# Ced3-han/PepFlowww

Measured on AMD Instinct MI355X. Metric: residues x denoise-steps / s, higher is better.
Workload: dtype f32 (fp32 storage and accumulation; matrix products as 3 x f16 split MFMA, ~22-bit operands); 1 GPU; cfg4/GPU: B=64 x 128-residue synthetic pockets (112 ctx + 16 gen) per GPU; per_gpu_batch=64, residues=128, global_batch=64, parallelism=batch-shard x1, hipgraph=True, precision=fp32

## Files before the change

include/pepflow_hip.h:

```cpp
#ifndef PEPFLOW_HIP_H
#define PEPFLOW_HIP_H
#include <stdint.h>

#ifdef __cplusplus
extern "C" {
#endif

#define PF_ABI_VERSION 65
#define PF_ATT_VROWS 164
#define PF_ATT_VT_NST(L) (((L) + 31) >> 5)
#define PF_ATT_VT_HEAD(L) ((size_t)11 * PF_ATT_VT_NST(L) * 512)
#define PF_ATT_VT_OFF(c, j, L) ((((size_t)(((c) < 128 ? ((c) & 7) : 8 + (((c) - 128) >> 4)) * PF_ATT_VT_NST(L) + ((j) >> 5)) * 64 + (((j) >> 3) & 3) * 16 + \
                                  ((c) < 128 ? ((c) >> 3) : (((c) - 128) & 15))) * 8) + ((j) & 7))
#define PF_E_BADARG (-1)
#define PF_E_TOOLARGE (-2)

typedef void* pf_stream_t;

#define PF_C_S 128
#define PF_C_Z 64
#define PF_HEADS 8
#define PF_C_HID 128
#define PF_QK_PTS 8
#define PF_V_PTS 12
#define PF_IPA_PROJ 3744
#define PF_IPA_FEATS 1536
#define PF_ET_PRE 512

int pf_abi_version(void);

int pf_selftest_mfma(const float* a, const float* b, float* c, int K, pf_stream_t stream);
int pf_selftest_lanes(const float* in, float* out, pf_stream_t stream);

typedef struct {
    const float* x;  int ldx;
    const float* w;  int ldw;
    const float* bias;
    float* y;        int ldy;
    int M, N, K;
    int relu;
    const float* row_mask;
    int mask_pre, mask_post;
    const float* residual; int ldr;
    const float* ln_gamma; const float* ln_beta; float ln_eps;
    const void* w_f16;
    const float* gate; int ldg;
    const float* pt_rot; const float* pt_trans; float* pt_qp; float* pt_kp; float* pt_vp; int pt_col0;
    int single_pass;
    void* att_qk; void* att_vt; int att_L;
    const int* key_end; int key_L; int active_rows;
    float* k_frag;
} pf_linear_args;
int pf_linear_fwd(const pf_linear_args* a, pf_stream_t stream);
int pf_split_pack_f16(const float* w, int ldw, int N, int K, int transpose, void* out, pf_stream_t stream);
typedef struct { const float* w; int ldw, N, K, transpose; void* out; int first; int pad_; } pf_pack_desc;
int pf_split_pack_f16_batch(const pf_pack_desc* desc_dev, int ndesc, int total_items, int* range_flag, pf_stream_t stream);
int pf_split_pack_f16_checked(const float* w, int ldw, int N, int K, int transpose, void* out, int* range_flag, pf_stream_t stream);

typedef struct {
    const float* node_embed;
    const float* seq_table;
    const int64_t* seqs;
    const float* t;
    const float* time_freq;
    const float* ang_freq;
    const float* angles;
    float* out;
    int B, L;
} pf_embed_args;
int pf_embed_inputs_fwd(const pf_embed_args* a, pf_stream_t stream);
typedef struct {
    const float* node_embed; const float* seq_table; const int64_t* seqs; const float* t; const float* time_freq;
    const float* ang_freq; const float* angles;
    const void* w0_f16; const float* b0; const void* w2_f16; const float* b2;
    const float* mask;
    const float* rot;
    float* quat;
    float* s_out;
    int B, L;
    int single_pass;
} pf_input_mixer_args;
int pf_input_mixer_fwd(const pf_input_mixer_args* a, pf_stream_t stream);

typedef struct {
    const float* proj; int ldp;
    const float* rot;
    const float* trans;
    float* qp;
    float* kp;
    float* vp;
    int rows;
} pf_ipa_points_args;
int pf_ipa_points_fwd(const pf_ipa_points_args* a, pf_stream_t stream);

typedef struct {
    const float* proj; int ldp;
    const float* qp; const float* kp; const float* vp;
    const float* z;
    const float* rot; const float* trans;
    const float* mask;
    const float* w_b; const float* b_b;
    const float* w_dz; const float* b_dz;
    const float* head_w;
    float* feats;
    int B, L;
    const float* bias;
    float* p_out;
    int variant;
    const void* att_qk; const void* att_vt; int att_mode;
    int head_group;
    const int* key_end;
    int z_f16;
    const float* dz;
    int dz_f16;
    int fused_pair;
    const float* s_in; const void* proj_w_f16; const float* proj_bias;
    const float* k_frag;
    int k_from_s;
} pf_ipa_attn_args;
int pf_ipa_attn_fwd(const pf_ipa_attn_args* a, pf_stream_t stream);
int pf_ipa_proj_inside_ok(int L, int f16_mode);
int pf_pair_bias_fwd(const float* z, const float* w_b, const float* b_b, float* bias, int B, int L, pf_stream_t stream);

typedef struct {
    const float* qkv;
    const float* mask;
    float* out;
    int B, L;
} pf_seq_attn_args;
int pf_seq_attn_fwd(const pf_seq_attn_args* a, pf_stream_t stream);

typedef struct {
    const float* feats;
    const float* s_in;
    const float* mask;
    const void* w_out_f16; const float* b_out;
    const float* ln_g; const float* ln_b;
    const void* w_in_f16; const float* b_in;
    float* s_ipa;
    float* qkv;
    int rows;
    int single_pass;
    const int* key_end; int key_L;
    float* dump_a0;
    int o_premul;
} pf_node_head_args;
int pf_node_head_fwd(const pf_node_head_args* a, pf_stream_t stream);

typedef struct {
    const float* qkv;
    const float* resid;
    const float* mask;
    const void* w_o_f16; const float* b_o; const float* n1_g; const float* n1_b;
    const void* w_1_f16; const float* b_1; const void* w_2_f16; const float* b_2; const float* n2_g; const float* n2_b;
    const void* w_in_next_f16; const float* b_in_next; float* qkv_out; float* v_out;
    int last;
    const float* s_ipa;
    const void* w_post_f16; const float* b_post;
    const void* w_t1_f16; const float* b_t1; const void* w_t2_f16; const float* b_t2; const void* w_t3_f16; const float* b_t3;
    const float* nt_g; const float* nt_b;
    const void* w_bb_f16; const float* b_bb;
    float* s_out;
    const float* quat_in; const float* rot_in; const float* trans_in;
    float* quat_out; float* rot_out; float* trans_out;
    int has_et;
    const void* w_init_f16; const float* b_init; const void* w_pre_f16; const float* b_pre; float* pre;
    int B, L;
    const void* h_w[2][3]; const float* h_b[2][3];
    float* logits_out;
    float* ang_out;
    int single_pass;
    const int* key_end;
    float* dump[11];
    const int* row_on;
} pf_node_tfmr_args;
int pf_node_tfmr_fwd(const pf_node_tfmr_args* a, pf_stream_t stream);

int pf_rot_to_quat(const float* rot, float* quat, int n, pf_stream_t stream);

typedef struct {
    const float* quat_in;
    const float* rot_in;
    const float* trans_in;
    const float* upd; int ldu;
    const float* mask;
    float* quat_out; float* rot_out; float* trans_out;
    int n;
} pf_rigid_update_args;
int pf_rigid_update_fwd(const pf_rigid_update_args* a, pf_stream_t stream);

typedef struct {
    const float* z_in;
    float* z_out;
    const float* pre;
    const void* w1z_f16;
    const void* w2_f16;
    const float* b2;
    const void* wf_f16;
    const float* ln_g; const float* ln_b;
    const float* mask;
    int B, L;
    const void* w_stream;
    float* bias_out; const void* wb_frags; const float* bb;
    float* dump_h1; float* dump_h2; float* dump_y;
    int single_pass;
    const int* tile_list; const int* n_tiles;
    int z_in_f16, z_out_f16;
    float* dz_out;
    int dz_out_f16;
    const void* w_stream32; const void* wb_frags32;
    unsigned char* dump_m1; unsigned char* dump_m2;
    int z_in_frag, z_out_frag;
    const void* w_stream64;
} pf_edge_transition_args;
int pf_edge_transition_fwd(const pf_edge_transition_args* a, pf_stream_t stream);
int pf_edge_transition_tile_rows(int single_pass);
int pf_edge_transition_v4_tile_rows(void);

typedef struct {
    const int64_t* aa; const int64_t* res_nb; const int64_t* chain_nb;
    const float* pos;
    const float* mask_atoms;
    const float* gen_mask;
    const float* aa_table;
    const float* freq3;
    float* feat;
    float* rot1; float* trans1;
    float* mres; float* ctx;
    int B, L;
    int sample_structure, sample_sequence;
    int L0;
} pf_node_feat_args;
int pf_node_features_fwd(const pf_node_feat_args* a, pf_stream_t stream);

typedef struct {
    const int64_t* aa; const int64_t* res_nb; const int64_t* chain_nb;
    const float* pos; const float* mask_atoms;
    const float* ctx; const float* mres;
    const float* aapair_table;
    const float* relpos_table;
    const float* distcoef;
    const float* freq3;
    const float* w_d0; const float* b_d0; const float* w_d2; const float* b_d2;
    const float* w_o0; const float* b_o0; const float* w_o2; const float* b_o2; const float* w_o4; const float* b_o4;
    float* out;
    int B, L;
    int sample_structure, sample_sequence;
    float* dump_g; float* dump_d2; float* dump_h1; float* dump_cat; float* dump_o1; float* dump_o2;
    float* softplus_ws;
} pf_edge_feat_args;
int pf_edge_features_fwd(const pf_edge_feat_args* a, pf_stream_t stream);

typedef struct {
    const float* rot1; const float* trans1; const float* ang1; const int64_t* seq1;
    const float* gen_mask;
    const float* res_mask;
    float* rot_t; float* trans_t; float* ang_t; int64_t* seq_t; float* simplex_t;
    float* trans0; float* simplex0;
    const float* pred_rot; const float* pred_trans; const float* pred_ang_raw; const float* pred_logits;
    float* traj_rot; float* traj_trans; float* traj_ang; int64_t* traj_seq; float* traj_simplex;
    const float* ts; int num_steps;
    int* step;
    float* t_out;
    const float* expo; uint64_t seed; int64_t first_sample;
    int B, L;
    int sample_bb, sample_ang, sample_seq;
    const uint64_t* seed_dev;
    const int64_t* sample_ids;
} pf_sampler_args;
int pf_sampler_init(const pf_sampler_args* a, const float* rot0, const float* trans0_raw,
                    const float* ang0, const float* simplex0_raw, pf_stream_t stream);
int pf_sampler_step(const pf_sampler_args* a, pf_stream_t stream);
typedef struct {
    int partial;
    const float* start_rot;
    const float* start_trans;
    const float* start_ang;
    const int64_t* start_seq;
    const uint8_t* res_flags;
    const uint32_t* aa_allowed;
} pf_sampler_cond_args;
int pf_sampler_init_cond(const pf_sampler_args* a, const pf_sampler_cond_args* c, const float* rot0, const float* trans0_raw,
                         const float* ang0, const float* simplex0_raw, pf_stream_t stream);
int pf_sampler_step_cond(const pf_sampler_args* a, const pf_sampler_cond_args* c, pf_stream_t stream);

#define PF_GUIDE_MAX_PAIRS 64
#define PF_GUIDE_MAX_L 1024
#define PF_GUIDE_NPARAMS 16
#define PF_GUIDE_NTERMS 5
typedef struct {
    const float* pred_trans;
    const float* trans1;
    const float* gen_mask;
    const float* res_mask;
    const uint8_t* res_flags;
    const uint8_t* hotspots;
    const int* pair_idx;
    const float* pair_par;
    const float* params;
    const float* ts;
    const int* step;
    const float* t;
    float* guided_trans;
    float* energy;
    float* shift_max;
    float* grad;
    int* error;
    int B, L, num_steps, sample_bb;
} pf_guidance_args;
int pf_guidance_fwd(const pf_guidance_args* a, pf_stream_t stream);

int pf_so3_geodesic(const float* base, const float* target, const float* t, float* out, int n, pf_stream_t stream);
int pf_so3_log(const float* rot, float* rotvec, int n, pf_stream_t stream);
int pf_so3_exp(const float* rotvec, float* rot, int n, pf_stream_t stream);
int pf_torus_geodesic(const float* base, const float* target, const float* t, float* out, int n, pf_stream_t stream);

typedef struct {
    const float* rot1; const float* trans1; const float* ang1; const int64_t* seq1;
    const float* gen_mask; const float* res_mask;
    const float* t_raw; const float* rot0; const float* trans0_raw; const float* ang0; const float* simplex0_raw;
    const float* expo; uint64_t seed; int64_t first_sample;
    float* t; float* rot_t; float* trans_t; float* ang_t; int64_t* seq_t;
    const float* pred_rot; const float* pred_trans; const float* pred_ang_raw; const float* pred_logits;
    int64_t* pred_seq;
    float* per_sample;
    float* losses;
    int B, L;
// ... 479 lines not shown
```

pepflowww_amd/_capi.py:

```python
import ctypes as C
import os

import torch

_HERE = os.path.dirname(os.path.abspath(__file__))
LIB_PATH = os.environ.get("PF_LIB_PATH") or os.path.join(_HERE, "lib", "libpepflow_hip.so")
ABI_VERSION = 65

_fp = C.c_void_p
_i = C.c_int
GUIDE_MAX_PAIRS, GUIDE_MAX_L, GUIDE_NPARAMS, GUIDE_NTERMS = 64, 1024, 16, 5


class LinearArgs(C.Structure):
    _fields_ = [("x", _fp), ("ldx", _i), ("w", _fp), ("ldw", _i), ("bias", _fp), ("y", _fp), ("ldy", _i),
                ("M", _i), ("N", _i), ("K", _i), ("relu", _i), ("row_mask", _fp), ("mask_pre", _i),
                ("mask_post", _i), ("residual", _fp), ("ldr", _i), ("ln_gamma", _fp), ("ln_beta", _fp),
                ("ln_eps", C.c_float), ("w_f16", _fp), ("gate", _fp), ("ldg", _i),
                ("pt_rot", _fp), ("pt_trans", _fp), ("pt_qp", _fp), ("pt_kp", _fp), ("pt_vp", _fp), ("pt_col0", _i),
                ("single_pass", _i), ("att_qk", _fp), ("att_vt", _fp), ("att_L", _i), ("key_end", _fp), ("key_L", _i), ("active_rows", _i),
                ("k_frag", _fp)]


class EmbedArgs(C.Structure):
    _fields_ = [("node_embed", _fp), ("seq_table", _fp), ("seqs", _fp), ("t", _fp), ("time_freq", _fp),
                ("ang_freq", _fp), ("angles", _fp), ("out", _fp), ("B", _i), ("L", _i)]


class IpaPointsArgs(C.Structure):
    _fields_ = [("proj", _fp), ("ldp", _i), ("rot", _fp), ("trans", _fp), ("qp", _fp), ("kp", _fp), ("vp", _fp),
                ("rows", _i)]


class IpaAttnArgs(C.Structure):
    _fields_ = [("proj", _fp), ("ldp", _i), ("qp", _fp), ("kp", _fp), ("vp", _fp), ("z", _fp), ("rot", _fp),
                ("trans", _fp), ("mask", _fp), ("w_b", _fp), ("b_b", _fp), ("w_dz", _fp), ("b_dz", _fp),
                ("head_w", _fp), ("feats", _fp), ("B", _i), ("L", _i), ("bias", _fp), ("p_out", _fp),
                ("variant", _i), ("att_qk", _fp), ("att_vt", _fp), ("att_mode", _i), ("head_group", _i), ("key_end", _fp), ("z_f16", _i), ("dz", _fp), ("dz_f16", _i), ("fused_pair", _i),
                ("s_in", _fp), ("proj_w_f16", _fp), ("proj_bias", _fp), ("k_frag", _fp), ("k_from_s", _i)]


class InputMixerArgs(C.Structure):
    _fields_ = [("node_embed", _fp), ("seq_table", _fp), ("seqs", _fp), ("t", _fp), ("time_freq", _fp), ("ang_freq", _fp),
                ("angles", _fp), ("w0_f16", _fp), ("b0", _fp), ("w2_f16", _fp), ("b2", _fp), ("mask", _fp), ("rot", _fp),
                ("quat", _fp), ("s_out", _fp), ("B", _i), ("L", _i), ("single_pass", _i)]


class SeqAttnArgs(C.Structure):
    _fields_ = [("qkv", _fp), ("mask", _fp), ("out", _fp), ("B", _i), ("L", _i)]


class RigidUpdateArgs(C.Structure):
    _fields_ = [("quat_in", _fp), ("rot_in", _fp), ("trans_in", _fp), ("upd", _fp), ("ldu", _i), ("mask", _fp),
                ("quat_out", _fp), ("rot_out", _fp), ("trans_out", _fp), ("n", _i)]


class EdgeTransitionArgs(C.Structure):
    _fields_ = [("z_in", _fp), ("z_out", _fp), ("pre", _fp), ("w1z_f16", _fp), ("w2_f16", _fp), ("b2", _fp), ("wf_f16", _fp),
                ("ln_g", _fp), ("ln_b", _fp), ("mask", _fp), ("B", _i), ("L", _i), ("w_stream", _fp),
                ("bias_out", _fp), ("wb_frags", _fp), ("bb", _fp), ("dump_h1", _fp), ("dump_h2", _fp), ("dump_y", _fp),
                ("single_pass", _i), ("tile_list", _fp), ("n_tiles", _fp), ("z_in_f16", _i), ("z_out_f16", _i), ("dz_out", _fp), ("dz_out_f16", _i),
                ("w_stream32", _fp), ("wb_frags32", _fp), ("dump_m1", _fp), ("dump_m2", _fp), ("z_in_frag", _i), ("z_out_frag", _i), ("w_stream64", _fp)]


class SamplerArgs(C.Structure):
    _fields_ = [("rot1", _fp), ("trans1", _fp), ("ang1", _fp), ("seq1", _fp), ("gen_mask", _fp), ("res_mask", _fp),
                ("rot_t", _fp), ("trans_t", _fp), ("ang_t", _fp), ("seq_t", _fp), ("simplex_t", _fp),
                ("trans0", _fp), ("simplex0", _fp),
                ("pred_rot", _fp), ("pred_trans", _fp), ("pred_ang_raw", _fp), ("pred_logits", _fp),
                ("traj_rot", _fp), ("traj_trans", _fp), ("traj_ang", _fp), ("traj_seq", _fp), ("traj_simplex", _fp),
                ("ts", _fp), ("num_steps", _i), ("step", _fp), ("t_out", _fp),
                ("expo", _fp), ("seed", C.c_uint64), ("first_sample", C.c_int64),
                ("B", _i), ("L", _i), ("sample_bb", _i), ("sample_ang", _i), ("sample_seq", _i), ("seed_dev", _fp), ("sample_ids", _fp)]


class SamplerCondArgs(C.Structure):
    _fields_ = [("partial", _i), ("start_rot", _fp), ("start_trans", _fp), ("start_ang", _fp), ("start_seq", _fp),
                ("res_flags", _fp), ("aa_allowed", _fp)]


class GuidanceArgs(C.Structure):
    _fields_ = [("pred_trans", _fp), ("trans1", _fp), ("gen_mask", _fp), ("res_mask", _fp), ("res_flags", _fp), ("hotspots", _fp),
                ("pair_idx", _fp), ("pair_par", _fp), ("params", _fp), ("ts", _fp), ("step", _fp), ("t", _fp),
                ("guided_trans", _fp), ("energy", _fp), ("shift_max", _fp), ("grad", _fp), ("error", _fp),
                ("B", _i), ("L", _i), ("num_steps", _i), ("sample_bb", _i)]


class TrainArgs(C.Structure):
    _fields_ = [("rot1", _fp), ("trans1", _fp), ("ang1", _fp), ("seq1", _fp), ("gen_mask", _fp), ("res_mask", _fp),
                ("t_raw", _fp), ("rot0", _fp), ("trans0_raw", _fp), ("ang0", _fp), ("simplex0_raw", _fp),
                ("expo", _fp), ("seed", C.c_uint64), ("first_sample", C.c_int64),
                ("t", _fp), ("rot_t", _fp), ("trans_t", _fp), ("ang_t", _fp), ("seq_t", _fp),
                ("pred_rot", _fp), ("pred_trans", _fp), ("pred_ang_raw", _fp), ("pred_logits", _fp),
                ("pred_seq", _fp), ("per_sample", _fp), ("losses", _fp),
                ("B", _i), ("L", _i), ("sample_structure", _i), ("sample_sequence", _i), ("seed_dev", _fp)]


class TrainBwdArgs(C.Structure):
    _fields_ = [("w", C.c_float * 6), ("d_rot", _fp), ("d_trans", _fp), ("d_ang", _fp), ("d_logits", _fp), ("w_dev", _fp)]


class GemmArgs(C.Structure):
    _fields_ = [("A", _fp), ("sam", C.c_longlong), ("sak", C.c_longlong), ("B", _fp), ("sbk", C.c_longlong), ("sbn", C.c_longlong),
                ("C", _fp), ("ldc", _i), ("M", _i), ("N", _i), ("K", _i), ("accumulate", _i),
                ("bias", _fp), ("relu", _i), ("residual", _fp), ("alpha", C.c_float), ("batch1", _i), ("batch2", _i),
                ("bsA1", C.c_longlong), ("bsA2", C.c_longlong), ("bsB1", C.c_longlong), ("bsB2", C.c_longlong),
                ("bsC1", C.c_longlong), ("bsC2", C.c_longlong), ("ksplit", _i), ("rowsum_a", _fp), ("gate", _fp)]


class LayerNormBwdArgs(C.Structure):
    _fields_ = [("x", _fp), ("dy", _fp), ("gamma", _fp), ("dx", _fp), ("dgamma_rows", _fp), ("M", _i), ("N", _i),
                ("dgamma", _fp), ("dbeta", _fp), ("workspace", _fp), ("workspace_elems", C.c_longlong), ("row_scale", _fp)]


class RigidUpdateBwdArgs(C.Structure):
    _fields_ = [("quat_in", _fp), ("rot_in", _fp), ("upd", _fp), ("ldu", _i), ("mask", _fp),
                ("g_rot_out", _fp), ("g_quat_out", _fp), ("g_trans_out", _fp),
                ("g_upd", _fp), ("g_quat_in", _fp), ("g_trans_in", _fp), ("g_rot_in", _fp), ("rot_is_from_quat", _i), ("n", _i)]


class IpaBwdArgs(C.Structure):
    _fields_ = [("proj", _fp), ("ldp", _i), ("qp", _fp), ("kp", _fp), ("vp", _fp), ("z", _fp), ("rot", _fp), ("trans", _fp), ("mask", _fp),
                ("w_b", _fp), ("b_b", _fp), ("w_dz", _fp), ("b_dz", _fp), ("head_w", _fp), ("g_feats", _fp),
                ("P", _fp), ("gA", _fp), ("g_opt", _fp), ("g_frame_rows", _fp), ("g_gamma_rows", _fp),
                ("g_bias", _fp), ("g_pz", _fp), ("g_z", _fp), ("accumulate_gz", _i),
                ("g_qp", _fp), ("g_kp", _fp), ("g_vp", _fp), ("g_proj", _fp), ("B", _i), ("L", _i), ("g_bp", _fp)]


class FullAtomArgs(C.Structure):
    _fields_ = [("rot", _fp), ("trans", _fp), ("angles", _fp), ("aa", _fp), ("tab_rot", _fp), ("tab_trans", _fp), ("tab_group", _fp),
                ("tab_pos", _fp), ("tab_mask", _fp), ("frame_group", _i * 5), ("pos14", _fp), ("frames_rot", _fp), ("frames_trans", _fp),
                ("gen_mask", _fp), ("ctx_pos15", _fp), ("pos15_merged", _fp), ("mask15", _fp), ("rows", _i)]


class BackboneAtomsArgs(C.Structure):
    _fields_ = [("rot", _fp), ("trans", _fp), ("aa", _fp), ("chain_nb", _fp), ("res_nb", _fp), ("mask", _fp), ("tab_bb", _fp),
                ("tab_o", _fp), ("pos4", _fp), ("gen_mask", _fp), ("ctx_pos15", _fp), ("ctx_mask15", _fp), ("pos15_merged", _fp),
                ("mask15", _fp), ("B", _i), ("L", _i)]


class NodeFeatArgs(C.Structure):
    _fields_ = [("aa", _fp), ("res_nb", _fp), ("chain_nb", _fp), ("pos", _fp), ("mask_atoms", _fp), ("gen_mask", _fp),
                ("aa_table", _fp), ("freq3", _fp), ("feat", _fp), ("rot1", _fp), ("trans1", _fp), ("mres", _fp),
                ("ctx", _fp), ("B", _i), ("L", _i), ("sample_structure", _i), ("sample_sequence", _i), ("L0", _i)]


class EdgeFeatArgs(C.Structure):
    _fields_ = [("aa", _fp), ("res_nb", _fp), ("chain_nb", _fp), ("pos", _fp), ("mask_atoms", _fp), ("ctx", _fp),
                ("mres", _fp), ("aapair_table", _fp), ("relpos_table", _fp), ("distcoef", _fp), ("freq3", _fp),
                ("w_d0", _fp), ("b_d0", _fp), ("w_d2", _fp), ("b_d2", _fp), ("w_o0", _fp), ("b_o0", _fp),
                ("w_o2", _fp), ("b_o2", _fp), ("w_o4", _fp), ("b_o4", _fp), ("out", _fp), ("B", _i), ("L", _i),
                ("sample_structure", _i), ("sample_sequence", _i),
                ("dump_g", _fp), ("dump_d2", _fp), ("dump_h1", _fp), ("dump_cat", _fp), ("dump_o1", _fp), ("dump_o2", _fp),
                ("softplus_ws", _fp)]


class NodeHeadArgs(C.Structure):
    _fields_ = [("feats", _fp), ("s_in", _fp), ("mask", _fp), ("w_out_f16", _fp), ("b_out", _fp), ("ln_g", _fp),
                ("ln_b", _fp), ("w_in_f16", _fp), ("b_in", _fp), ("s_ipa", _fp), ("qkv", _fp), ("rows", _i), ("single_pass", _i), ("key_end", _fp), ("key_L", _i), ("dump_a0", _fp), ("o_premul", _i)]


class NodeTfmrArgs(C.Structure):
    _fields_ = [("qkv", _fp), ("resid", _fp), ("mask", _fp),
                ("w_o_f16", _fp), ("b_o", _fp), ("n1_g", _fp), ("n1_b", _fp), ("w_1_f16", _fp), ("b_1", _fp),
                ("w_2_f16", _fp), ("b_2", _fp), ("n2_g", _fp), ("n2_b", _fp),
                ("w_in_next_f16", _fp), ("b_in_next", _fp), ("qkv_out", _fp), ("v_out", _fp), ("last", _i),
                ("s_ipa", _fp), ("w_post_f16", _fp), ("b_post", _fp), ("w_t1_f16", _fp), ("b_t1", _fp), ("w_t2_f16", _fp),
                ("b_t2", _fp), ("w_t3_f16", _fp), ("b_t3", _fp), ("nt_g", _fp), ("nt_b", _fp), ("w_bb_f16", _fp),
                ("b_bb", _fp), ("s_out", _fp), ("quat_in", _fp), ("rot_in", _fp), ("trans_in", _fp),
                ("quat_out", _fp), ("rot_out", _fp), ("trans_out", _fp), ("has_et", _i),
                ("w_init_f16", _fp), ("b_init", _fp), ("w_pre_f16", _fp), ("b_pre", _fp), ("pre", _fp), ("B", _i), ("L", _i),
                ("h_w", (_fp * 3) * 2), ("h_b", (_fp * 3) * 2), ("logits_out", _fp), ("ang_out", _fp), ("single_pass", _i), ("key_end", _fp), ("dump", _fp * 11), ("row_on", _fp)]


class SuperposeArgs(C.Structure):
    _fields_ = [("x", _fp), ("y", _fp), ("mx", _fp), ("my", _fp), ("aa_x", _fp), ("aa_y", _fp), ("pairs", _fp),
                ("rmsd_plain", _fp), ("rmsd", _fp), ("count", _fp), ("ident", _fp), ("rot", _fp), ("trans", _fp), ("aligned", _fp),
                ("degenerate", _fp), ("Bx", _i), ("By", _i), ("N", _i), ("P", _i), ("allow_reflection", _i)]


class BindingSiteArgs(C.Structure):
    _fields_ = [("ctx_pos", _fp), ("ctx_atom_mask", _fp), ("n_atoms", _i), ("ca_atom", _i), ("res_mask", _fp), ("gen_mask", _fp),
                ("pep_sample", _fp), ("pep_native", _fp), ("cutoff", C.c_float), ("site_sample", _fp), ("site_native", _fp),
                ("bsr", _fp), ("B", _i), ("L", _i)]


class TmScoreArgs(C.Structure):
    _fields_ = [("x", _fp), ("y", _fp), ("mx", _fp), ("my", _fp), ("pairs", _fp), ("tm", _fp), ("count", _fp), ("lnorm", _fp),
                ("rot", _fp), ("trans", _fp), ("aligned", _fp), ("work", _fp), ("Bx", _i), ("By", _i), ("N", _i), ("P", _i)]


class DsspArgs(C.Structure):
    _fields_ = [("pos", _fp), ("mask", _fp), ("chain", _fp), ("aa", _fp), ("ss", _fp), ("hb_acc", _fp), ("hb_energy", _fp),
                ("B", _i), ("N", _i), ("n_atoms", _i), ("pro", _i)]


class TmAlignArgs(C.Structure):
    _fields_ = [("x", _fp), ("y", _fp), ("mx", _fp), ("my", _fp), ("pairs", _fp), ("tm", _fp), ("tm_x", _fp), ("rmsd", _fp),
                ("n_aligned", _fp), ("len_x", _fp), ("len_y", _fp), ("rot", _fp), ("trans", _fp), ("y2x", _fp), ("kept", _fp),
                ("aligned", _fp), ("Bx", _i), ("By", _i), ("N", _i), ("P", _i), ("max_len", _i)]


class ViolationsArgs(C.Structure):
    _fields_ = [("pos", _fp), ("atom_mask", _fp), ("aa", _fp), ("residue_index", _fp), ("query", _fp), ("group", _fp), ("radius", _fp),
                ("clash_atom_loss", _fp), ("clash_atom", _fp), ("clash_atom_pairs", _fp), ("clash_atom_loss_cross", _fp),
                ("clash_atom_cross", _fp), ("clash_mean_loss", _fp), ("bond_c_n_loss_mean", _fp), ("angle_ca_c_n_loss_mean", _fp),
                ("angle_c_n_ca_loss_mean", _fp), ("connection_loss", _fp), ("connection_violation", _fp), ("ca_ca_break", _fp),
                ("ca_ca_extreme", _fp), ("B", _i), ("N", _i), ("n_atoms", _i), ("pro", _i),
                ("violation_tolerance_factor", C.c_float), ("clash_overlap_tolerance", C.c_float)]


class SasaArgs(C.Structure):
    _fields_ = [("pos", _fp), ("atom_mask", _fp), ("aa", _fp), ("query", _fp), ("group", _fp), ("radius", _fp), ("points", _fp),
                ("work", _fp), ("count", _fp), ("sasa_atom", _fp), ("sasa_residue", _fp), ("sasa_total", _fp), ("count_own", _fp),
                ("sasa_atom_own", _fp), ("sasa_residue_own", _fp), ("sasa_total_own", _fp), ("B", _i), ("N", _i), ("n_atoms", _i),
                ("n_points", _i), ("probe_radius", C.c_float)]


class CavityArgs(C.Structure):
    _fields_ = [("pos", _fp), ("atom_mask", _fp), ("aa", _fp), ("radius", _fp), ("origin", _fp), ("work", _fp), ("occupied", _fp),
                ("buried", _fp), ("label", _fp), ("n_found", _fp), ("size", _fp), ("center", _fp), ("mean_buried", _fp),
                ("lining", _fp), ("status", _fp), ("B", _i), ("N", _i), ("n_atoms", _i), ("nx", _i), ("ny", _i), ("nz", _i),
                ("n_axis", _i), ("n_diag", _i), ("min_buried", _i), ("connectivity", _i), ("min_points", _i), ("max_cavities", _i),
                ("h", C.c_float), ("probe", C.c_float), ("r_lining", C.c_float)]


class TorsionsArgs(C.Structure):
    _fields_ = [("pos", _fp), ("atom_mask", _fp), ("aa", _fp), ("residue_index", _fp), ("chi_atoms", _fp), ("angles", _fp),
                ("defined", _fp), ("B", _i), ("N", _i), ("n_atoms", _i)]


class SidechainCompareArgs(C.Structure):
    _fields_ = [("pos_x", _fp), ("pos_y", _fp), ("mask_x", _fp), ("mask_y", _fp), ("aa_x", _fp), ("aa_y", _fp), ("angles_x", _fp),
                ("angles_y", _fp), ("defined_x", _fp), ("defined_y", _fp), ("pairs", _fp), ("periodic", _fp), ("swap", _fp),
                ("err_sum", _fp), ("err_count", _fp), ("within", _fp), ("res_with_chi", _fp), ("res_correct", _fp), ("sc_sq_sum", _fp),
                ("sc_atoms", _fp), ("sc_rmsd", _fp), ("err", _fp), ("sc_sq", _fp), ("sc_n", _fp), ("swapped", _fp),
                ("Bx", _i), ("By", _i), ("N", _i), ("P", _i), ("n_atoms_x", _i), ("n_atoms_y", _i), ("correct_tol", C.c_float)]


class LddtArgs(C.Structure):
    _fields_ = [("pos_x", _fp), ("pos_y", _fp), ("mask_x", _fp), ("mask_y", _fp), ("aa_x", _fp), ("aa_y", _fp), ("pairs", _fp),
                ("group", _fp), ("query", _fp), ("scored", _fp), ("kept", _fp), ("scored_cross", _fp), ("kept_cross", _fp),
                ("scored_atom", _fp), ("kept_atom", _fp), ("scored_atom_cross", _fp), ("kept_atom_cross", _fp),
                ("Bx", _i), ("By", _i), ("N", _i), ("P", _i), ("n_atoms_x", _i), ("n_atoms_y", _i), ("slot_mask", _i),
                ("exclude_same_residue", _i), ("cutoff", C.c_float)]


class ContactsArgs(C.Structure):
    _fields_ = [("pos_x", _fp), ("pos_y", _fp), ("mask_x", _fp), ("mask_y", _fp), ("pairs", _fp), ("group", _fp),
                ("contacts_x", _fp), ("contacts_y", _fp), ("contacts_shared", _fp), ("interface_x", _fp), ("interface_y", _fp),
                ("min_dist_x", _fp), ("min_dist_y", _fp), ("Bx", _i), ("By", _i), ("N", _i), ("P", _i), ("n_atoms_x", _i),
                ("n_atoms_y", _i), ("slot_mask", _i), ("contact_cutoff", C.c_float), ("interface_cutoff", C.c_float)]


class ClusterArgs(C.Structure):
    _fields_ = [("dist", _fp), ("index", _fp), ("offsets", _fp), ("score", _fp), ("work", _fp), ("label", _fp), ("cluster_size", _fp),
                ("representative", _fp), ("best", _fp), ("n_neighbours", _fp), ("n_clusters", _fp), ("B", _i), ("G", _i), ("n_max", _i),
                ("method", _i), ("cutoff", C.c_float)]


class PackArgs(C.Structure):
    _fields_ = [("pos", _fp), ("atom_mask", _fp), ("aa", _fp), ("residue_index", _fp), ("movable", _fp), ("radius", _fp), ("types", _fp),
                ("own_mask", _fp), ("tab_rot", _fp), ("tab_trans", _fp), ("tab_group", _fp), ("tab_pos", _fp), ("tab_mask", _fp),
                ("rot_chi", _fp), ("rot_count", _fp), ("rot_energy", _fp), ("work", _fp), ("pos_out", _fp), ("mask_out", _fp),
                ("packed", _fp), ("rotamer", _fp), ("chi", _fp), ("n_rotamers", _fp), ("energy_self_best", _fp), ("energy_residue", _fp),
                ("energy_trace", _fp), ("sweeps_run", _fp), ("changed", _fp), ("choice_trace", _fp),
                ("B", _i), ("N", _i), ("n_atoms", _i), ("max_rot", _i), ("sweeps", _i), ("pro", _i), ("cys", _i),
                ("cutoff", C.c_float), ("w_gauss1", C.c_float), ("w_gauss2", C.c_float), ("w_repulsion", C.c_float),
                ("w_hydrophobic", C.c_float), ("w_hbond", C.c_float)]


class InterfaceEnergyArgs(C.Structure):
    _fields_ = [("pos", _fp), ("atom_mask", _fp), ("aa", _fp), ("group", _fp), ("query", _fp), ("radius", _fp), ("types", _fp),
                ("work", _fp), ("terms_atom", _fp), ("terms_residue", _fp), ("energy_residue", _fp), ("pairs_atom", _fp),
                ("hbond_pairs_atom", _fp), ("hydrophobic_pairs_atom", _fp), ("B", _i), ("N", _i), ("n_atoms", _i),
                ("cutoff", C.c_float), ("w_gauss1", C.c_float), ("w_gauss2", C.c_float), ("w_repulsion", C.c_float),
                ("w_hydrophobic", C.c_float), ("w_hbond", C.c_float)]


class RelaxArgs(C.Structure):
    _fields_ = [("pos", _fp), ("ref_pos", _fp), ("atom_mask", _fp), ("aa", _fp), ("residue_index", _fp), ("movable", _fp),
                ("radius", _fp), ("pair_mask", _fp), ("work", _fp), ("gradient", _fp), ("terms_atom", _fp), ("energy_atom", _fp),
                ("terms", _fp), ("energy", _fp), ("x", _fp), ("g", _fp), ("y", _fp), ("alpha", _fp), ("frozen", _fp),
                ("terms_initial", _fp), ("energy_trace", _fp), ("accepted", _fp), ("step_size", _fp), ("grad_max", _fp),
                ("iterations", _fp), ("B", _i), ("N", _i), ("n_atoms", _i), ("pro", _i), ("steps", _i),
                ("k_rest", C.c_float), ("k_intra", C.c_float), ("k_bond", C.c_float), ("k_angle", C.c_float), ("k_clash", C.c_float),
                ("clash_overlap_tolerance", C.c_float), ("clash_margin", C.c_float), ("step0", C.c_float), ("gtol", C.c_float)]


class EtBwdArgs(C.Structure):
    _fields_ = [("g_y", _fp), ("h1", _fp), ("h2", _fp), ("wfT_f16", _fp), ("w2T_f16", _fp), ("w1T_f16", _fp),
                ("g_h2", _fp), ("g_h1", _fp), ("g_x", _fp), ("npairs", C.c_longlong), ("m1", _fp), ("m2", _fp)]


class OptimArgs(C.Structure):
    _fields_ = [("tensors", _fp), ("hyper", _fp), ("chunks", _fp), ("exp_avg", _fp), ("exp_avg_sq", _fp), ("steps", _fp), ("work", _fp),
                ("result", _fp), ("n_tensors", _i), ("n_groups", _i), ("n_chunks", _i)]


_SIGNATURES = {
    "pf_et_bwd_chain": ([C.POINTER(EtBwdArgs), _fp], _i),
    "pf_gemm_tn_cat": ([_fp, _i, _i, _fp, _fp, _fp, _i, _i, _fp, _i, _i, _fp, _i, _fp, C.c_longlong, _fp], _i),
    "pf_gemm_tn_sum2": ([_fp, _i, _i, _fp, _fp, _i, _i, _fp, _i, C.c_longlong, _i, _fp, _i, _fp, C.c_longlong, _fp], _i),
    "pf_et_pack_train": ([_fp, _fp, _fp, _fp, _fp, _fp, _fp, C.c_float, _fp, _fp, _fp], _i),
    "pf_abi_version": ([], _i),
    "pf_selftest_mfma": ([_fp, _fp, _fp, _i, _fp], _i),
    "pf_selftest_lanes": ([_fp, _fp, _fp], _i),
    "pf_linear_fwd": ([C.POINTER(LinearArgs), _fp], _i),
    "pf_embed_inputs_fwd": ([C.POINTER(EmbedArgs), _fp], _i),
    "pf_input_mixer_fwd": ([C.POINTER(InputMixerArgs), _fp], _i),
    "pf_ipa_points_fwd": ([C.POINTER(IpaPointsArgs), _fp], _i),
    "pf_ipa_attn_fwd": ([C.POINTER(IpaAttnArgs), _fp], _i),
    "pf_ipa_proj_inside_ok": ([_i, _i], _i),
    "pf_pair_bias_fwd": ([_fp, _fp, _fp, _fp, _i, _i, _fp], _i),
    "pf_seq_attn_fwd": ([C.POINTER(SeqAttnArgs), _fp], _i),
    "pf_node_head_fwd": ([C.POINTER(NodeHeadArgs), _fp], _i),
    "pf_node_tfmr_fwd": ([C.POINTER(NodeTfmrArgs), _fp], _i),
    "pf_rot_to_quat": ([_fp, _fp, _i, _fp], _i),
    "pf_rigid_update_fwd": ([C.POINTER(RigidUpdateArgs), _fp], _i),
    "pf_edge_transition_fwd": ([C.POINTER(EdgeTransitionArgs), _fp], _i),
    "pf_edge_transition_tile_rows": ([_i], _i),
    "pf_edge_transition_v4_tile_rows": ([], _i),
    "pf_node_features_fwd": ([C.POINTER(NodeFeatArgs), _fp], _i),
    "pf_edge_features_fwd": ([C.POINTER(EdgeFeatArgs), _fp], _i),
    "pf_sampler_init": ([C.POINTER(SamplerArgs), _fp, _fp, _fp, _fp, _fp], _i),
# ... 141 lines not shown
```

pepflowww_amd/csrc/common.h:

```cpp
#pragma once
#include <hip/hip_runtime.h>

static inline int pf_cu_count() {
    static int cache[64] = {0};
    int dev = 0, c = 256;
    if (hipGetDevice(&dev) != hipSuccess) return 256;
    if (dev >= 0 && dev < 64 && cache[dev] > 0) return cache[dev];
    if (hipDeviceGetAttribute(&c, hipDeviceAttributeMultiprocessorCount, dev) != hipSuccess || c <= 0) c = 256;
    if (dev >= 0 && dev < 64) cache[dev] = c;
    return c;
}
#include <stdint.h>

#define PF_WAVE 64

typedef float f32x4 __attribute__((ext_vector_type(4)));

__device__ __forceinline__ f32x4 mfma16(float a, float b, f32x4 c) {
    return __builtin_amdgcn_mfma_f32_16x16x4f32(a, b, c, 0, 0, 0);
}

__device__ __forceinline__ void lds_barrier() {
    asm volatile("s_waitcnt lgkmcnt(0)" ::: "memory");
    __builtin_amdgcn_s_barrier();
// ... 14 lines not shown
template <int OFF> __device__ __forceinline__ float lane_xor(float v) {
    if constexpr (OFF == 1) return lane_xor1(v);
    else if constexpr (OFF == 2) return lane_xor2(v);
    else if constexpr (OFF == 4) return lane_xor4(v);
    else return lane_xor8(v);
}
__device__ __forceinline__ float sum_xor16(float v) {
    auto r = __builtin_amdgcn_permlane16_swap(__float_as_uint(v), __float_as_uint(v), false, false);
    return __uint_as_float(r[0]) + __uint_as_float(r[1]);
}
__device__ __forceinline__ float sum_xor32(float v) {
    auto r = __builtin_amdgcn_permlane32_swap(__float_as_uint(v), __float_as_uint(v), false, false);
    return __uint_as_float(r[0]) + __uint_as_float(r[1]);
}
__device__ __forceinline__ float max_xor16(float v) {
    auto r = __builtin_amdgcn_permlane16_swap(__float_as_uint(v), __float_as_uint(v), false, false);
    return fmaxf(__uint_as_float(r[0]), __uint_as_float(r[1]));
}
__device__ __forceinline__ float max_xor32(float v) {
    auto r = __builtin_amdgcn_permlane32_swap(__float_as_uint(v), __float_as_uint(v), false, false);
    return fmaxf(__uint_as_float(r[0]), __uint_as_float(r[1]));
}
__device__ __forceinline__ bool pf_rows_all_masked(const int* __restrict__ key_end, int L, int m0, int n, int M) {
    if (!key_end) return false;
    const int mend = m0 + n < M ? m0 + n : M;
    int m = m0;
    while (m < mend) {
        const int b = m / L, i = m - b * L;
        if (i < key_end[b]) return false;
        m = (b + 1) * L;
    }
    return true;
}
__device__ __forceinline__ float row16_sum(float v) {
    v += lane_xor8(v); v += lane_xor4(v); v += lane_xor2(v); v += lane_xor1(v);
    return v;
}
__device__ __forceinline__ float row16_max(float v) {
    v = fmaxf(v, lane_xor8(v)); v = fmaxf(v, lane_xor4(v)); v = fmaxf(v, lane_xor2(v)); v = fmaxf(v, lane_xor1(v));
    return v;
}
__device__ __forceinline__ float wave_sum(float v) { return sum_xor32(sum_xor16(row16_sum(v))); }
__device__ __forceinline__ float wave_max(float v) { return max_xor32(max_xor16(row16_max(v))); }

__device__ __forceinline__ float keep_if(bool ok, float v) { return __uint_as_float(__float_as_uint(v) & (ok ? 0xffffffffu : 0u)); }
__device__ __forceinline__ float4 keep_if(bool ok, const float4& v) {
    const unsigned m = ok ? 0xffffffffu : 0u;
    return make_float4(__uint_as_float(__float_as_uint(v.x) & m), __uint_as_float(__float_as_uint(v.y) & m),
                       __uint_as_float(__float_as_uint(v.z) & m), __uint_as_float(__float_as_uint(v.w) & m));
}

template <int MT, int NT>
__device__ __forceinline__ void mfma_slice(const float4 (&a)[MT], const float4 (&b)[NT], f32x4 (&acc)[MT][NT]) {
#pragma unroll
    for (int mt = 0; mt < MT; ++mt)
#pragma unroll
        for (int nt = 0; nt < NT; ++nt) {
            acc[mt][nt] = mfma16(a[mt].x, b[nt].x, acc[mt][nt]);
            acc[mt][nt] = mfma16(a[mt].y, b[nt].y, acc[mt][nt]);
            acc[mt][nt] = mfma16(a[mt].z, b[nt].z, acc[mt][nt]);
            acc[mt][nt] = mfma16(a[mt].w, b[nt].w, acc[mt][nt]);
        }
}

template <int NT, int PF_DEPTH = 4>
struct BStream {
    const float* wrow[NT];
    bool wok[NT];
    float4 ring[PF_DEPTH][NT];
    int nslices;

    __device__ __forceinline__ void init(const float* __restrict__ W, int ldw, int n0, int n_valid, int K) {
        const int lane = threadIdx.x & 63;
        const int r = lane & 15, g = lane >> 4;
        nslices = K >> 4;
#pragma unroll
        for (int nt = 0; nt < NT; ++nt) {
            const int n = n0 + 16 * nt + r;
            wok[nt] = n < n_valid;
            wrow[nt] = W + (size_t)(wok[nt] ? n : 0) * ldw + 4 * g;
        }
    }
    __device__ __forceinline__ void load(int slot_static, int slice, float4 (&dst)[NT]) {
        (void)slot_static;
#pragma unroll
        for (int nt = 0; nt < NT; ++nt)
            dst[nt] = *reinterpret_cast<const float4*>(wrow[nt] + 16 * slice);
    }
    __device__ __forceinline__ void prefetch() {
#pragma unroll
        for (int d = 0; d < PF_DEPTH; ++d)
            if (d < nslices) load(d, d, ring[d]);
    }
};

template <int MT, int NT, int PF_DEPTH>
__device__ __forceinline__ void gemm_ldsA_stream(const float* __restrict__ A_lds, int lda, BStream<NT, PF_DEPTH>& bs,
                                                 f32x4 (&acc)[MT][NT], int slice0, int count) {
    const int lane = threadIdx.x & 63;
    const float* arow = A_lds + (lane & 15) * lda + 4 * (lane >> 4);
    const int ns = bs.nslices;
    for (int base = 0; base < count; base += PF_DEPTH) {
#pragma unroll
        for (int u = 0; u < PF_DEPTH; ++u) {
            if (base + u < count) {
                const int sl = slice0 + base + u;
                float4 a[MT];
#pragma unroll
                for (int mt = 0; mt < MT; ++mt)
                    a[mt] = *reinterpret_cast<const float4*>(arow + mt * 16 * lda + 16 * (base + u));
                mfma_slice<MT, NT>(a, bs.ring[u], acc);
                if (sl + PF_DEPTH < ns) bs.load(u, sl + PF_DEPTH, bs.ring[u]);
            }
        }
    }
}

template <int MT, int NT>
__device__ __forceinline__ void gemm_ldsA_glbB(const float* __restrict__ A_lds, int lda,
                                               const float* __restrict__ W, int ldw, int n0, int n_valid,
                                               int K, f32x4 (&acc)[MT][NT]) {
    BStream<NT> bs;
    bs.init(W, ldw, n0, n_valid, K);
    bs.prefetch();
    gemm_ldsA_stream<MT, NT, 4>(A_lds, lda, bs, acc, 0, bs.nslices);
}

typedef _Float16 half8 __attribute__((ext_vector_type(8)));
typedef _Float16 half4 __attribute__((ext_vector_type(4)));
__device__ __forceinline__ float exp_softmax(float x) { return __builtin_amdgcn_exp2f(x * 1.4426950408889634f); }
constexpr float PF_LO_SCALE = 2048.f, PF_LO_INV = 1.f / 2048.f;

__device__ __forceinline__ f32x4 mfma_h(half8 a, half8 b, f32x4 c) {
    return __builtin_amdgcn_mfma_f32_16x16x32_f16(a, b, c, 0, 0, 0);
}
constexpr float PF_F16_MAX = 65504.f;
#ifndef PF_SPLIT_SATURATE
#define PF_SPLIT_SATURATE 1
#endif
__device__ __forceinline__ void split4(const float (&v)[4], half4& hi, half4& lo) {
#pragma unroll
    for (int e = 0; e < 4; ++e) {
#if PF_SPLIT_SATURATE
        const float vc = fminf(fmaxf(v[e], -PF_F16_MAX), PF_F16_MAX) + v[e] * 0.f;
#else
        const float vc = v[e];
#endif
        const _Float16 h = (_Float16)vc;
        hi[e] = h;
        lo[e] = (_Float16)__builtin_fmaf((float)h, -PF_LO_SCALE, vc * PF_LO_SCALE);
    }
}
__device__ __forceinline__ float join(f32x4 m, f32x4 c, int e) { return m[e] + c[e] * PF_LO_INV; }

template <int WT, int D, bool SP = false>
struct WSplit {
    const _Float16* wh[WT];
    const _Float16* wl[WT];
    half8 rh[D][WT], rl[D][WT];
    int nsteps;
    __device__ __forceinline__ void init(const void* planes, int Npad, int K, int n0) {
        const int lane = threadIdx.x & 63;
        const _Float16* hi = reinterpret_cast<const _Float16*>(planes);
        const _Float16* lo = hi + (size_t)Npad * K;
        nsteps = K >> 5;
#pragma unroll
        for (int wt = 0; wt < WT; ++wt) {
            const size_t off = ((size_t)((n0 >> 4) + wt) * nsteps * 64 + lane) * 8;
            wh[wt] = hi + off;
            wl[wt] = lo + off;
        }
    }
    __device__ __forceinline__ void load(int step, half8 (&dh)[WT], half8 (&dl)[WT]) {
#pragma unroll
        for (int wt = 0; wt < WT; ++wt) {
            dh[wt] = *reinterpret_cast<const half8*>(wh[wt] + (size_t)step * 512);
            if constexpr (!SP) dl[wt] = *reinterpret_cast<const half8*>(wl[wt] + (size_t)step * 512);
        }
    }
    __device__ __forceinline__ void prefetch() {
#pragma unroll
        for (int d = 0; d < D; ++d)
            if (d < nsteps) load(d, rh[d], rl[d]);
    }
};

template <int WT, int D, bool SP>
__device__ __forceinline__ void gemm_split16(WSplit<WT, D, SP>& ws, const _Float16* Xh, const _Float16* Xl, int ldx,
                                             f32x4 (&am)[WT], f32x4 (&ac)[WT], int step0, int count) {
    const int lane = threadIdx.x & 63;
    const int off = (lane & 15) * ldx + 8 * (lane >> 4);
    for (int base = 0; base < count; base += D) {
#pragma unroll
        for (int u = 0; u < D; ++u) {
            if (base + u < count) {
                const int st = step0 + base + u;
                const half8 xh = *reinterpret_cast<const half8*>(Xh + off + 32 * (base + u));
                half8 xl;
                if constexpr (!SP) xl = *reinterpret_cast<const half8*>(Xl + off + 32 * (base + u));
#pragma unroll
                for (int wt = 0; wt < WT; ++wt) {
                    am[wt] = mfma_h(ws.rh[u][wt], xh, am[wt]);
                    if constexpr (!SP) {
                        ac[wt] = mfma_h(ws.rh[u][wt], xl, ac[wt]);
                        ac[wt] = mfma_h(ws.rl[u][wt], xh, ac[wt]);
                    }
                }
                if (st + D < ws.nsteps) ws.load(st + D, ws.rh[u], ws.rl[u]);
            }
        }
    }
}
template <int WT, int D, bool SP, int RT>
__device__ __forceinline__ void gemm_split16r(WSplit<WT, D, SP>& ws, const _Float16* Xh, const _Float16* Xl, int ldx,
                                              f32x4 (&am)[RT][WT], f32x4 (&ac)[RT][WT], int step0, int count) {
    const int lane = threadIdx.x & 63;
    const int off = (lane & 15) * ldx + 8 * (lane >> 4);
    for (int base = 0; base < count; base += D) {
#pragma unroll
        for (int u = 0; u < D; ++u) {
            if (base + u < count) {
                const int st = step0 + base + u;
#pragma unroll
                for (int rt = 0; rt < RT; ++rt) {
                    const half8 xh = *reinterpret_cast<const half8*>(Xh + rt * 16 * ldx + off + 32 * (base + u));
                    half8 xl;
                    if constexpr (!SP) xl = *reinterpret_cast<const half8*>(Xl + rt * 16 * ldx + off + 32 * (base + u));
#pragma unroll
                    for (int wt = 0; wt < WT; ++wt) {
                        am[rt][wt] = mfma_h(ws.rh[u][wt], xh, am[rt][wt]);
                        if constexpr (!SP) {
                            ac[rt][wt] = mfma_h(ws.rh[u][wt], xl, ac[rt][wt]);
                            ac[rt][wt] = mfma_h(ws.rl[u][wt], xh, ac[rt][wt]);
                        }
                    }
                }
                if (st + D < ws.nsteps) ws.load(st + D, ws.rh[u], ws.rl[u]);
            }
        }
    }
}
template <int WT> __device__ __forceinline__ void acc_zero1(f32x4 (&a)[WT], f32x4 (&b)[WT]) {
#pragma unroll
    for (int wt = 0; wt < WT; ++wt) { a[wt] = (f32x4){0.f, 0.f, 0.f, 0.f}; b[wt] = (f32x4){0.f, 0.f, 0.f, 0.f}; }
}

template <int WT>
struct WPre {
    half8 h[WT], l[WT];
    __device__ __forceinline__ void load(const void* planes, int N, int Kw, int n0) {
        const int lane = threadIdx.x & 63;
        const int wsteps = Kw >> 5;
        const _Float16* wh = reinterpret_cast<const _Float16*>(planes) + ((size_t)(n0 >> 4) * wsteps * 64 + lane) * 8;
        const _Float16* wl = wh + (size_t)N * Kw;
        const size_t tstride = (size_t)wsteps * 512;
#pragma unroll
        for (int wt = 0; wt < WT; ++wt) {
            h[wt] = *reinterpret_cast<const half8*>(wh + wt * tstride);
            l[wt] = *reinterpret_cast<const half8*>(wl + wt * tstride);
        }
    }
};

template <int WT, int PT, bool SP = false>
__device__ __forceinline__ void gemm_split_lowreg(const void* planes, int N, int Kw, int n0, int K,
                                                  const _Float16* Xh, const _Float16* Xl, int ldx,
                                                  f32x4 (&am)[WT][PT], f32x4 (&ac)[WT][PT]) {
    static_assert(PT % 2 == 0, "row tiles are fed in pairs");
    const int lane = threadIdx.x & 63, r = lane & 15, g = lane >> 4;
    const int wsteps = Kw >> 5, nst = K >> 5;
    const _Float16* wh = reinterpret_cast<const _Float16*>(planes) + ((size_t)(n0 >> 4) * wsteps * 64 + lane) * 8;
    const _Float16* wl = wh + (size_t)N * Kw;
    const size_t tstride = (size_t)wsteps * 512;
    const _Float16* xh = Xh + r * ldx + 8 * g;
    const _Float16* xl = Xl + r * ldx + 8 * g;
    for (int st = 0; st < nst; ++st) {
        half8 bh[WT], bl[WT];
#pragma unroll
        for (int wt = 0; wt < WT; ++wt) {
            bh[wt] = *reinterpret_cast<const half8*>(wh + wt * tstride + (size_t)st * 512);
            if constexpr (!SP) bl[wt] = *reinterpret_cast<const half8*>(wl + wt * tstride + (size_t)st * 512);
        }
#pragma unroll
        for (int p0 = 0; p0 < PT; p0 += 2) {
            half8 ah[2], al[2];
#pragma unroll
            for (int q = 0; q < 2; ++q) {
                ah[q] = *reinterpret_cast<const half8*>(xh + (p0 + q) * 16 * ldx + 32 * st);
                if constexpr (!SP) al[q] = *reinterpret_cast<const half8*>(xl + (p0 + q) * 16 * ldx + 32 * st);
            }
#pragma unroll
            for (int wt = 0; wt < WT; ++wt)
#pragma unroll
                for (int q = 0; q < 2; ++q) am[wt][p0 + q] = mfma_h(bh[wt], ah[q], am[wt][p0 + q]);
            if constexpr (!SP) {
#pragma unroll
                for (int wt = 0; wt < WT; ++wt)
#pragma unroll
                    for (int q = 0; q < 2; ++q) ac[wt][p0 + q] = mfma_h(bh[wt], al[q], ac[wt][p0 + q]);
#pragma unroll
                for (int wt = 0; wt < WT; ++wt)
#pragma unroll
                    for (int q = 0; q < 2; ++q) ac[wt][p0 + q] = mfma_h(bl[wt], ah[q], ac[wt][p0 + q]);
            }
        }
    }
// ... 88 lines not shown
```

pepflowww_amd/csrc/ipa_split.hip:

```cpp
#include <cstdlib>
#include <type_traits>
#include "common.h"
#include "../../include/pepflow_hip.h"

#ifdef PF_PROFILE
__device__ long long g_prof_ipas[64];
#define PROFS(i) do { if (blockIdx.x == gridDim.x / 2 + 3 && threadIdx.x == 64) g_prof_ipas[i] = clock64(); } while (0)
extern "C" int pf_debug_prof_ipas(long long* out, int n) {
    return (int)hipMemcpyFromSymbol(out, HIP_SYMBOL(g_prof_ipas), sizeof(long long) * n, 0, hipMemcpyDeviceToHost);
}
#else
#define PROFS(i)
#endif

namespace {

typedef float f32x2 __attribute__((ext_vector_type(2)));
constexpr int H = PF_HEADS, C = PF_C_HID, PQ = PF_QK_PTS, PV = PF_V_PTS;
constexpr int OFF_KV = 1024;
#ifndef PF_IPA_WMAX
#define PF_IPA_WMAX 8
#endif
constexpr int WMAX = PF_IPA_WMAX;
constexpr int KPS = 28;
constexpr int VPS = 36;

__device__ __forceinline__ float softplusf2(float x) { return x > 20.f ? x : log1pf(expf(x)); }

template <bool D16> struct DzVec { typedef float4 type; };
template <> struct DzVec<true> { typedef half4 type; };

template <int NB4, bool D16>
__device__ __forceinline__ void pair_dz_rows(const void* __restrict__ dzp, size_t rowb, int L, int i0, int Le, int kt,
                                             const float* __restrict__ Pw, int SLD, int ks, int cq, f32x2 (&acc)[32]) {
    typedef typename DzVec<D16>::type V4;
    typedef typename std::conditional<D16, _Float16, float>::type DT;
    constexpr int NT = 4 * NB4;
    const DT* base = reinterpret_cast<const DT*>(dzp) + rowb * (size_t)L * 16 + 4 * cq;
    int koff[NT];
    float on[NT];
#pragma unroll
    for (int u = 0; u < NT; ++u) {
        const int uu = min(u, kt - 1);
        koff[u] = min(16 * uu + ks, L - 1) * 16;
        on[u] = u < kt ? 1.f : 0.f;
    }
    auto load_row = [&](int qi, V4 (&buf)[NT]) {
        const DT* row = base + (size_t)min(i0 + qi, Le - 1) * L * 16;
#pragma unroll
        for (int u = 0; u < NT; ++u) buf[u] = *reinterpret_cast<const V4*>(row + koff[u]);
    };
    auto mac_row = [&](int qi, const V4 (&buf)[NT]) {
        const float* pr = Pw + qi * SLD;
#pragma unroll
        for (int u = 0; u < NT; ++u) {
            float pv;
            if (u <= 4 * (NB4 - 1)) pv = pr[16 * u];
            else pv = pr[16 * min(u, kt - 1)] * on[u];
            const f32x2 p2 = {pv, pv};
            f32x2 d0, d1;
            if constexpr (D16) { d0 = (f32x2){(float)buf[u][0], (float)buf[u][1]}; d1 = (f32x2){(float)buf[u][2], (float)buf[u][3]}; }
            else { d0 = (f32x2){buf[u].x, buf[u].y}; d1 = (f32x2){buf[u].z, buf[u].w}; }
            acc[2 * qi] = __builtin_elementwise_fma(d0, p2, acc[2 * qi]);
            acc[2 * qi + 1] = __builtin_elementwise_fma(d1, p2, acc[2 * qi + 1]);
        }
    };
    constexpr int D = NB4 == 1 ? 8 : NB4 == 2 ? 4 : 2;
    V4 buf[D][NT];
#pragma unroll
    for (int d = 0; d < D - 1; ++d) load_row(d, buf[d]);
#pragma unroll
    for (int qi = 0; qi < 16; ++qi) {
        load_row(min(qi + D - 1, 15), buf[(qi + D - 1) % D]);
        __builtin_amdgcn_sched_barrier(0);
        mac_row(qi, buf[qi % D]);
        __builtin_amdgcn_sched_barrier(0);
    }
}

template <bool D16>
__device__ __forceinline__ void pair_dz_phase(const pf_ipa_attn_args& a, size_t rowb, int h, int i0, int Le, int kt, const float* Pwave,
                                              int SLD, float inv, int lane) {
    const int ks = (lane & 3) | ((lane >> 4) << 2), cq = (lane >> 2) & 3;
    f32x2 acc[32];
#pragma unroll
    for (int k = 0; k < 32; ++k) acc[k] = (f32x2){0.f, 0.f};
    const float* Pw = Pwave + ks;
    const int nb4 = (kt + 3) >> 2;
    if (nb4 <= 1) pair_dz_rows<1, D16>(a.dz, rowb, a.L, i0, Le, kt, Pw, SLD, ks, cq, acc);
    else if (nb4 == 2) pair_dz_rows<2, D16>(a.dz, rowb, a.L, i0, Le, kt, Pw, SLD, ks, cq, acc);
    else if (nb4 == 3) pair_dz_rows<3, D16>(a.dz, rowb, a.L, i0, Le, kt, Pw, SLD, ks, cq, acc);
    else pair_dz_rows<4, D16>(a.dz, rowb, a.L, i0, Le, kt, Pw, SLD, ks, cq, acc);
    float v[64];
#pragma unroll
    for (int k = 0; k < 32; ++k) { v[2 * k] = acc[k][0]; v[2 * k + 1] = acc[k][1]; }
    float w[32], x[16], y[8], z4[4];
#pragma unroll
    for (int k = 0; k < 32; ++k) {
        auto rr = __builtin_amdgcn_permlane32_swap(__float_as_uint(v[k]), __float_as_uint(v[k + 32]), false, false);
        w[k] = __uint_as_float(rr[0]) + __uint_as_float(rr[1]);
    }
#pragma unroll
    for (int k = 0; k < 16; ++k) {
        auto rr = __builtin_amdgcn_permlane16_swap(__float_as_uint(w[k]), __float_as_uint(w[k + 16]), false, false);
        x[k] = __uint_as_float(rr[0]) + __uint_as_float(rr[1]);
    }
    {
        const bool hi = lane & 2;
#pragma unroll
        for (int k = 0; k < 8; ++k) {
            const float send = hi ? x[k] : x[k + 8], keep = hi ? x[k + 8] : x[k];
            y[k] = keep + lane_xor2(send);
        }
    }
    {
        const bool hi = lane & 1;
#pragma unroll
        for (int k = 0; k < 4; ++k) {
            const float send = hi ? y[k] : y[k + 4], keep = hi ? y[k + 4] : y[k];
            z4[k] = keep + lane_xor1(send);
        }
    }
    const int qi = ((lane >> 5) & 1) * 8 + ((lane >> 4) & 1) * 4 + (lane & 3);
    const float invq = __shfl(inv, qi);
    const float4 bd = *reinterpret_cast<const float4*>(a.b_dz + 4 * cq);
    const int i = min(i0 + qi, Le - 1);
    *reinterpret_cast<float4*>(a.feats + (rowb + i) * PF_IPA_FEATS + 1408 + h * 16 + 4 * cq) =
        make_float4(z4[0] * invq + bd.x, z4[1] * invq + bd.y, z4[2] * invq + bd.z, z4[3] * invq + bd.w);
}

template <int I, int N, class F> __device__ __forceinline__ void cfor_p(F&& f) {
    if constexpr (I < N) {
        f(std::integral_constant<int, I>{});
        cfor_p<I + 1, N>(f);
    }
}
constexpr int PJ_TILES = 31;
constexpr int PJ_NPAD = 3968;
constexpr int PJ_CT = 3;
constexpr int PJ_NCH = (PJ_TILES + PJ_CT - 1) / PJ_CT;
constexpr int PJ_CHUNK_B = PJ_CT * 8 * 1024;
constexpr int PJ_NB = 4;
constexpr int PJ_STAGE_B = PJ_NB * PJ_CHUNK_B;
__device__ __forceinline__ constexpr int pj_tile(int idx, int h) {
    return idx < 8 ? 8 * h + idx : idx < 24 ? 64 + 16 * h + (idx - 8) : idx < 26 ? 192 + 2 * h + (idx - 24) : 208 + 5 * h + (idx - 26);
}
__device__ __forceinline__ void pj_glds16(const void* sbase, unsigned voff, unsigned lds_addr) {
    const unsigned long long v = (unsigned long long)sbase;
    const unsigned lo = __builtin_amdgcn_readfirstlane((unsigned)v), hi = __builtin_amdgcn_readfirstlane((unsigned)(v >> 32));
    const void* sb = (const void*)(((unsigned long long)hi << 32) | lo);
    lds_addr = __builtin_amdgcn_readfirstlane(lds_addr);
    asm volatile("s_mov_b32 m0, %2\n\ts_nop 4\n\tglobal_load_lds_dwordx4 %0, %1" : : "v"(voff), "s"(sb), "s"(lds_addr) : "memory", "m0");
}
template <class V> __device__ __forceinline__ void pf_pin(V& v) { asm("" : "+v"(v)); }
template <int N> __device__ __forceinline__ void pj_wait_vm() { asm volatile("s_waitcnt vmcnt(%0)" : : "n"(N) : "memory"); }
__device__ __forceinline__ void pj_wait_vm_dyn(int n) {
    n = __builtin_amdgcn_readfirstlane(n);
    switch (n > 40 ? 40 : n) {
#define PJ_W(k) case k: pj_wait_vm<k>(); break;
        PJ_W(0) PJ_W(1) PJ_W(2) PJ_W(3) PJ_W(4) PJ_W(5) PJ_W(6) PJ_W(7) PJ_W(8) PJ_W(9) PJ_W(10) PJ_W(11) PJ_W(12) PJ_W(13) PJ_W(14)
        PJ_W(15) PJ_W(16) PJ_W(17) PJ_W(18) PJ_W(19) PJ_W(20) PJ_W(21) PJ_W(22) PJ_W(23) PJ_W(24) PJ_W(25) PJ_W(26) PJ_W(27) PJ_W(28)
        PJ_W(29) PJ_W(30) PJ_W(31) PJ_W(32) PJ_W(33) PJ_W(34) PJ_W(35) PJ_W(36) PJ_W(37) PJ_W(38) PJ_W(39) PJ_W(40)
#undef PJ_W
    }
}
__device__ __forceinline__ constexpr int pj_vt_row(int f) { return f < 64 ? 16 * (f & 3) + (f >> 2) : 64 + 16 * ((f - 64) & 3) + ((f - 64) >> 2); }
__device__ __forceinline__ int pj_vt_pos(int j) { return (j & ~31) + 8 * ((j >> 2) & 3) + 4 * ((j >> 4) & 1) + (j & 3); }
__host__ __device__ __forceinline__ constexpr int pj_vtl(int LP) { return ((LP + 31) & ~31) + 8; }
__host__ __device__ __forceinline__ constexpr int pj_vp_floats(int LP) {
    return LP * VPS > 48 * pj_vtl(LP) ? LP * VPS : 48 * pj_vtl(LP);
}
struct PjW { half8 h[4], l[4]; };
template <bool KF> __device__ __forceinline__ constexpr int pj_ntiles() { return KF ? PJ_TILES - 8 : PJ_TILES; }
template <bool KF> __device__ __forceinline__ constexpr int pj_nch() { return (pj_ntiles<KF>() + PJ_CT - 1) / PJ_CT; }
template <bool KF> __device__ __forceinline__ constexpr int pj_orig(int j) { return KF && j >= 8 ? j + 8 : j; }
__device__ __forceinline__ constexpr bool pj_q_tile(int idx) { return idx < 8 || idx == 24 || idx == 25; }
template <bool KS, bool KF = false>
__device__ __forceinline__ void proj_head(const pf_ipa_attn_args& a, size_t rowb, int iq, int h, int jrow, int LPe, bool wave_on, int role, int tile, float* KP,
                                          _Float16* VPT , int VTL, _Float16* VTH , int VTG,
                                          unsigned char* WS , float* QPW ,
                                          float* PB ,
                                          float4 (&qf)[8], float4 (&qp4)[6], int lane, int wave, int nw) {
    const int r = lane & 15, g = lane >> 4;
    PROFS(8);
    const unsigned char* whp = reinterpret_cast<const unsigned char*>(a.proj_w_f16);
    const unsigned char* wlp = whp + (size_t)PJ_NPAD * 128 * 2;
    const unsigned ws0 = (unsigned)(size_t)(__attribute__((address_space(3))) void*)WS;
    const unsigned l16 = lane * 16;
    const int ppw = (PJ_CT * 8 + nw - 1) / nw;
    constexpr int NT = pj_ntiles<KF>(), NCH = pj_nch<KF>();
    auto issue = [&](int c) __attribute__((always_inline)) {
        const int npc = min(PJ_CT, NT - PJ_CT * c) * 8;
        for (int k = 0; k < ppw; ++k) {
            const int pc = min(wave + k * nw, npc - 1);
            const int tl = pc >> 3, ks = (pc >> 1) & 3, pl = pc & 1;
            const int T16 = pj_tile(pj_orig<KF>(PJ_CT * c + tl), h);
            pj_glds16((pl ? wlp : whp) + (size_t)(T16 * 4 + ks) * 1024, l16, ws0 + (c % PJ_NB) * PJ_CHUNK_B + pc * 1024);
        }
    };
    for (int i = wave * 64 + lane; i < PJ_TILES * 16; i += nw * 64) PB[i] = a.proj_bias[16 * pj_tile(i >> 4, h) + (i & 15)];
    for (int i = wave * 64 + lane; i < 24 * VTL; i += nw * 64) reinterpret_cast<float2*>(VPT)[i] = make_float2(0.f, 0.f);
    PROFS(30);
    half8 xh[4], xl[4];
    float R[9], T[3];
    {
        const float* xrow = a.s_in + (rowb + iq) * 128 + 8 * g;
        float4 t[8];
#pragma unroll
        for (int ks = 0; ks < 4; ++ks) { t[2 * ks] = *reinterpret_cast<const float4*>(xrow + 32 * ks); t[2 * ks + 1] = *reinterpret_cast<const float4*>(xrow + 32 * ks + 4); }
        const float* Rg = a.rot + (rowb + iq) * 9;
        const float* Tg = a.trans + (rowb + iq) * 3;
#pragma unroll
        for (int k = 0; k < 9; ++k) R[k] = Rg[k];
#pragma unroll
        for (int k = 0; k < 3; ++k) T[k] = Tg[k];
#pragma unroll
        for (int ks = 0; ks < 4; ++ks) {
            const float v0[4] = {t[2 * ks].x, t[2 * ks].y, t[2 * ks].z, t[2 * ks].w}, v1[4] = {t[2 * ks + 1].x, t[2 * ks + 1].y, t[2 * ks + 1].z, t[2 * ks + 1].w};
            half4 h0, l0, h1, l1;
            split4(v0, h0, l0);
            split4(v1, h1, l1);
#pragma unroll
            for (int e = 0; e < 4; ++e) { xh[ks][e] = h0[e]; xh[ks][4 + e] = h1[e]; xl[ks][e] = l0[e]; xl[ks][4 + e] = l1[e]; }
        }
    }
    PROFS(31);
    if constexpr (KF) {
        _Float16* kfrag = VTH + (size_t)8 * (VTG >> 5) * 1024 + (size_t)tile * 4096 + lane * 8;
        if (wave_on && role != 1) {
            const float* krow = a.s_in + (rowb + iq) * 128 + 4 * g;
#pragma unroll
            for (int hb = 0; hb < 2; ++hb) {
                float4 kt[4];
#pragma unroll
                for (int u = 0; u < 4; ++u) kt[u] = *reinterpret_cast<const float4*>(krow + 16 * (4 * hb + u));
#pragma unroll
                for (int u = 0; u < 4; ++u) {
                    const int t8 = 4 * hb + u;
                    const float v[4] = {kt[u].x, kt[u].y, kt[u].z, kt[u].w};
                    if constexpr (KS) {
                        half4 hi, lo;
#pragma unroll
                        for (int e = 0; e < 4; ++e) hi[e] = (_Float16)v[e];
                        pf_pin(hi);
#pragma unroll
                        for (int e = 0; e < 4; ++e) lo[e] = (_Float16)(v[e] - (float)hi[e]);
                        _Float16* d = kfrag + (t8 >> 1) * 1024 + (t8 & 1) * 4;
                        *reinterpret_cast<half4*>(d) = hi;
                        *reinterpret_cast<half4*>(d + 512) = lo;
                    } else {
                        *reinterpret_cast<float4*>(reinterpret_cast<float*>(kfrag - lane * 8) + t8 * 256 + lane * 4) = kt[u];
                    }
                }
            }
        }
    }
    PROFS(32);
    asm volatile("" ::: "memory");
#pragma unroll
    for (int c = 0; c < PJ_NB - 1; ++c)
        if (c < NCH) issue(c);
    PROFS(33);
    _Float16* kfrag = VTH + (size_t)8 * (VTG >> 5) * 1024 + (size_t)tile * 4096 + lane * 8;
    float qpr[2][3] = {{0.f, 0.f, 0.f}, {0.f, 0.f, 0.f}};
    auto ldfrag = [&](int c, int tl, PjW& w) __attribute__((always_inline)) {
        const unsigned char* b = WS + (c % PJ_NB) * PJ_CHUNK_B + tl * 8192 + lane * 16;
#pragma unroll
        for (int ks = 0; ks < 4; ++ks) {
            w.h[ks] = *reinterpret_cast<const half8*>(b + ks * 2048);
            w.l[ks] = *reinterpret_cast<const half8*>(b + ks * 2048 + 1024);
        }
    };
    cfor_p<0, NCH>([&](auto ic) __attribute__((always_inline)) {
        constexpr int c = decltype(ic)::value;
        constexpr int NDY = (c + 1 < NCH) + (PJ_NB > 3 && c + 2 < NCH) + (PJ_NB > 4 && c + 3 < NCH);
        static_assert(PJ_NB == 2 || PJ_NB == 4, "wait accounting written for 2 or 4 staging buffers");
        PROFS(9 + 2 * c);
        pj_wait_vm_dyn(PJ_NB == 2 ? 0 : NDY * ppw);
        if constexpr (c == 0) asm volatile("s_waitcnt lgkmcnt(0)" ::: "memory");
        __builtin_amdgcn_s_barrier();
        PROFS(10 + 2 * c);
        asm volatile("" ::: "memory");
        if constexpr (c + PJ_NB - 1 < NCH) issue(c + PJ_NB - 1);
        if (wave_on) {
            PjW wa, wb;
            if (role == 0) ldfrag(c, 0, wa);
            cfor_p<0, PJ_CT>([&](auto it) __attribute__((always_inline)) {
                constexpr int tl = decltype(it)::value, jt = PJ_CT * c + tl, idx = pj_orig<KF>(jt);
                if constexpr (jt < NT) {
                  if (role == 0 || (role == 1) == pj_q_tile(idx)) {
                    PjW& w = (tl & 1) ? wb : wa;
                    if (role != 0) ldfrag(c, tl, w);
                    else if constexpr (tl + 1 < PJ_CT && jt + 1 < NT) ldfrag(c, tl + 1, (tl & 1) ? wa : wb);
                    constexpr bool VTILE = idx >= 16 && idx < 24;
                    f32x4 am = {0.f, 0.f, 0.f, 0.f}, ac = {0.f, 0.f, 0.f, 0.f};
#pragma unroll
                    for (int ks = 0; ks < 4; ++ks) {
                        if constexpr (VTILE) {
                            am = mfma_h(xh[ks], w.h[ks], am);
                            ac = mfma_h(xl[ks], w.h[ks], ac);
                            ac = mfma_h(xh[ks], w.l[ks], ac);
                        } else {
                            am = mfma_h(w.h[ks], xh[ks], am);
                            ac = mfma_h(w.h[ks], xl[ks], ac);
                            ac = mfma_h(w.l[ks], xh[ks], ac);
                        }
                    }
                    float v[4];
                    if constexpr (VTILE) {
                        const float b1 = PB[16 * idx + r];
#pragma unroll
                        for (int e = 0; e < 4; ++e) v[e] = (am[e] + ac[e] * PF_LO_INV) + b1;
                    } else {
                        const float4 b4 = *reinterpret_cast<const float4*>(PB + 16 * idx + 4 * g);
                        v[0] = (am[0] + ac[0] * PF_LO_INV) + b4.x; v[1] = (am[1] + ac[1] * PF_LO_INV) + b4.y;
                        v[2] = (am[2] + ac[2] * PF_LO_INV) + b4.z; v[3] = (am[3] + ac[3] * PF_LO_INV) + b4.w;
                    }
                    if constexpr (idx < 8) {
                        qf[idx] = make_float4(v[0], v[1], v[2], v[3]);
                    } else if constexpr (idx < 16) {
                        if constexpr (KS) {
                            half4 hi, lo;
#pragma unroll
                            for (int e = 0; e < 4; ++e) hi[e] = (_Float16)v[e];
                            pf_pin(hi);
#pragma unroll
                            for (int e = 0; e < 4; ++e) lo[e] = (_Float16)(v[e] - (float)hi[e]);
                            _Float16* d = kfrag + ((idx - 8) >> 1) * 1024 + ((idx - 8) & 1) * 4;
                            *reinterpret_cast<half4*>(d) = hi;
                            *reinterpret_cast<half4*>(d + 512) = lo;
                        } else {
                            *reinterpret_cast<float4*>(reinterpret_cast<float*>(kfrag - lane * 8) + (idx - 8) * 256 + lane * 4) = make_float4(v[0], v[1], v[2], v[3]);
                        }
                    } else if constexpr (VTILE) {
                        half4 hi, lo;
#pragma unroll
                        for (int e = 0; e < 4; ++e) hi[e] = (_Float16)v[e];
                        pf_pin(hi);
#pragma unroll
                        for (int e = 0; e < 4; ++e) lo[e] = (_Float16)(v[e] - (float)hi[e]);
                        const int f = 16 * (idx - 16) + r;
                        const int row = pj_vt_row(f), nst = VTG >> 5;
                        _Float16* d = VTH + ((size_t)((row >> 4) * nst + (tile >> 1)) * 2 * 64 + 16 * g + (row & 15)) * 8 + 4 * (tile & 1);
                        *reinterpret_cast<half4*>(d) = hi;
                        *reinterpret_cast<half4*>(d + 512) = lo;
                    } else {
                        const float ox = R[0] * v[0] + R[1] * v[1] + R[2] * v[2] + T[0];
                        const float oy = R[3] * v[0] + R[4] * v[1] + R[5] * v[2] + T[1];
                        const float oz = R[6] * v[0] + R[7] * v[1] + R[8] * v[2] + T[2];
                        if constexpr (idx < 26) {
                            qpr[idx - 24][0] = ox; qpr[idx - 24][1] = oy; qpr[idx - 24][2] = oz;
                        } else {
                            const int pp = 4 * (idx - 26) + g;
                            if (jrow < LPe) {
                                if (pp < 8) {
                                    float* o = KP + jrow * KPS + 3 * pp;
                                    o[0] = ox; o[1] = oy; o[2] = oz;
                                } else {
                                    _Float16* o = VPT + 3 * (pp - 8) * VTL + pj_vt_pos(jrow);
                                    const float c3[3] = {ox, oy, oz};
#pragma unroll
                                    for (int m = 0; m < 3; ++m) {
                                        const _Float16 hi = (_Float16)c3[m];
                                        o[m * VTL] = hi;
                                        o[(48 + m) * VTL] = (_Float16)(c3[m] - (float)hi);
                                    }
                                }
                            }
                        }
                    }
                  }
                }
            });
        }
    });
    if (wave_on) {
        asm volatile("s_waitcnt vmcnt(0) lgkmcnt(0)" ::: "memory");
        __builtin_amdgcn_wave_barrier();
        if (role == 2) return;
        float qv[24];
#pragma unroll
        for (int t2 = 0; t2 < 2; ++t2)
#pragma unroll
            for (int gs = 0; gs < 4; ++gs)
#pragma unroll
                for (int cc = 0; cc < 3; ++cc) qv[3 * (4 * t2 + gs) + cc] = __shfl(qpr[t2][cc], r + 16 * gs, 64);
#pragma unroll
        for (int q = 0; q < 6; ++q) qp4[q] = make_float4(qv[4 * q], qv[4 * q + 1], qv[4 * q + 2], qv[4 * q + 3]);
        (void)QPW;
    }
}

constexpr int KLS = 128 + 8;
constexpr int PJ16_CHUNK_B = PJ_CT * 4 * 1024;
constexpr int PJ16_STAGE_B = PJ_NB * PJ16_CHUNK_B;
template <bool KF = false>
__device__ __forceinline__ void proj_head16(const pf_ipa_attn_args& a, size_t rowb, int iq, int h, int jrow, bool wave_on, float* KP,
                                            _Float16* KL, _Float16* VT, int VTS, unsigned char* WS ,
                                            float* QPW , float* PB,
                                            half8 (&qh)[4], float4 (&qp4)[6], int lane, int wave, int nw) {
    const int r = lane & 15, g = lane >> 4;
    const unsigned char* whp = reinterpret_cast<const unsigned char*>(a.proj_w_f16);
    const unsigned ws0 = (unsigned)(size_t)(__attribute__((address_space(3))) void*)WS;
    const unsigned l16 = lane * 16;
    const int ppw = (PJ_CT * 4 + nw - 1) / nw;
    constexpr int NT = pj_ntiles<KF>(), NCH = pj_nch<KF>();
    auto issue = [&](int c) __attribute__((always_inline)) {
        const int npc = min(PJ_CT, NT - PJ_CT * c) * 4;
        for (int k = 0; k < ppw; ++k) {
            const int pc = min(wave + k * nw, npc - 1);
            const int T16 = pj_tile(pj_orig<KF>(PJ_CT * c + (pc >> 2)), h);
            pj_glds16(whp + (size_t)(T16 * 4 + (pc & 3)) * 1024, l16, ws0 + (c % PJ_NB) * PJ16_CHUNK_B + pc * 1024);
        }
    };
    for (int i = wave * 64 + lane; i < PJ_TILES * 16; i += nw * 64) PB[i] = a.proj_bias[16 * pj_tile(i >> 4, h) + (i & 15)];
    half8 xh[4];
    float R[9], T[3];
    {
        const float* xrow = a.s_in + (rowb + iq) * 128 + 8 * g;
        float4 t[8];
#pragma unroll
        for (int ks = 0; ks < 4; ++ks) { t[2 * ks] = *reinterpret_cast<const float4*>(xrow + 32 * ks); t[2 * ks + 1] = *reinterpret_cast<const float4*>(xrow + 32 * ks + 4); }
        const float* Rg = a.rot + (rowb + iq) * 9;
        const float* Tg = a.trans + (rowb + iq) * 3;
#pragma unroll
        for (int k = 0; k < 9; ++k) R[k] = Rg[k];
#pragma unroll
        for (int k = 0; k < 3; ++k) T[k] = Tg[k];
#pragma unroll
        for (int ks = 0; ks < 4; ++ks) {
            xh[ks][0] = (_Float16)t[2 * ks].x; xh[ks][1] = (_Float16)t[2 * ks].y; xh[ks][2] = (_Float16)t[2 * ks].z; xh[ks][3] = (_Float16)t[2 * ks].w;
            xh[ks][4] = (_Float16)t[2 * ks + 1].x; xh[ks][5] = (_Float16)t[2 * ks + 1].y; xh[ks][6] = (_Float16)t[2 * ks + 1].z; xh[ks][7] = (_Float16)t[2 * ks + 1].w;
        }
    }
    if constexpr (KF) {
        if (wave_on) {
#pragma unroll
            for (int ks = 0; ks < 4; ++ks) *reinterpret_cast<half8*>(KL + jrow * KLS + 32 * ks + 8 * g) = xh[ks];
        }
    }
    asm volatile("" ::: "memory");
#pragma unroll
    for (int c = 0; c < PJ_NB - 1; ++c)
        if (c < NCH) issue(c);
    _Float16* QL = reinterpret_cast<_Float16*>(QPW);
    float qpr[2][3] = {{0.f, 0.f, 0.f}, {0.f, 0.f, 0.f}};
    auto ldfrag = [&](int c, int tl, half8 (&w)[4]) __attribute__((always_inline)) {
        const unsigned char* b = WS + (c % PJ_NB) * PJ16_CHUNK_B + tl * 4096 + lane * 16;
#pragma unroll
        for (int ks = 0; ks < 4; ++ks) w[ks] = *reinterpret_cast<const half8*>(b + ks * 1024);
    };
    cfor_p<0, NCH>([&](auto ic) __attribute__((always_inline)) {
        constexpr int c = decltype(ic)::value;
        constexpr int NDY = (c + 1 < NCH) + (PJ_NB > 3 && c + 2 < NCH);
        static_assert(PJ_NB == 4, "wait accounting written for 4 staging buffers");
        pj_wait_vm_dyn(NDY * ppw);
        if constexpr (c == 0) asm volatile("s_waitcnt lgkmcnt(0)" ::: "memory");
        __builtin_amdgcn_s_barrier();
        asm volatile("" ::: "memory");
        if constexpr (c + PJ_NB - 1 < NCH) issue(c + PJ_NB - 1);
        if (wave_on) {
            half8 wa[4], wb[4];
            ldfrag(c, 0, wa);
            cfor_p<0, PJ_CT>([&](auto it) __attribute__((always_inline)) {
                constexpr int tl = decltype(it)::value, jt = PJ_CT * c + tl, idx = pj_orig<KF>(jt);
                if constexpr (jt < NT) {
                    half8 (&w)[4] = (tl & 1) ? wb : wa;
                    if constexpr (tl + 1 < PJ_CT && jt + 1 < NT) ldfrag(c, tl + 1, (tl & 1) ? wa : wb);
                    f32x4 am = {0.f, 0.f, 0.f, 0.f};
                    if constexpr (idx >= 16 && idx < 24) {
#pragma unroll
                        for (int ks = 0; ks < 4; ++ks) am = mfma_h(xh[ks], w[ks], am);
                        const float bn = PB[16 * idx + r];
                        half4 hv;
                        hv[0] = (_Float16)(am[0] + bn); hv[1] = (_Float16)(am[1] + bn); hv[2] = (_Float16)(am[2] + bn); hv[3] = (_Float16)(am[3] + bn);
                        *reinterpret_cast<half4*>(VT + (16 * (idx - 16) + r) * VTS + (jrow - r) + 4 * g) = hv;
                    } else {
#pragma unroll
                        for (int ks = 0; ks < 4; ++ks) am = mfma_h(w[ks], xh[ks], am);
                        const float4 b4 = *reinterpret_cast<const float4*>(PB + 16 * idx + 4 * g);
                        float v[4];
                        v[0] = am[0] + b4.x; v[1] = am[1] + b4.y; v[2] = am[2] + b4.z; v[3] = am[3] + b4.w;
                        if constexpr (idx < 16) {
                            half4 hv;
                            hv[0] = (_Float16)v[0]; hv[1] = (_Float16)v[1]; hv[2] = (_Float16)v[2]; hv[3] = (_Float16)v[3];
                            if constexpr (idx < 8) {
                                *reinterpret_cast<half4*>(QL + r * 40 + 16 * (idx & 1) + 4 * g) = hv;
                                if constexpr (idx & 1) {
                                    asm volatile("s_waitcnt lgkmcnt(0)" ::: "memory");
                                    __builtin_amdgcn_wave_barrier();
                                    qh[idx >> 1] = *reinterpret_cast<const half8*>(QL + r * 40 + 8 * g);
                                    asm volatile("s_waitcnt lgkmcnt(0)" ::: "memory");
                                    __builtin_amdgcn_wave_barrier();
                                }
                            } else {
                                *reinterpret_cast<half4*>(KL + jrow * KLS + 16 * (idx - 8) + 4 * g) = hv;
                            }
                        } else {
                            const float ox = R[0] * v[0] + R[1] * v[1] + R[2] * v[2] + T[0];
                            const float oy = R[3] * v[0] + R[4] * v[1] + R[5] * v[2] + T[1];
                            const float oz = R[6] * v[0] + R[7] * v[1] + R[8] * v[2] + T[2];
                            if constexpr (idx < 26) {
                                qpr[idx - 24][0] = ox; qpr[idx - 24][1] = oy; qpr[idx - 24][2] = oz;
                            } else {
                                const int pp = 4 * (idx - 26) + g;
                                if (pp < 8) {
                                    float* o = KP + jrow * KPS + 3 * pp;
                                    o[0] = ox; o[1] = oy; o[2] = oz;
                                } else {
                                    _Float16* o = VT + (128 + 3 * (pp - 8)) * VTS + jrow;
                                    o[0] = (_Float16)ox; o[VTS] = (_Float16)oy; o[2 * VTS] = (_Float16)oz;
                                }
                            }
                        }
                    }
                }
            });
        }
    });
    if (wave_on) {
        asm volatile("s_waitcnt lgkmcnt(0)" ::: "memory");
        __builtin_amdgcn_wave_barrier();
        float qv[24];
#pragma unroll
        for (int t2 = 0; t2 < 2; ++t2)
#pragma unroll
            for (int gs = 0; gs < 4; ++gs)
#pragma unroll
                for (int cc = 0; cc < 3; ++cc) qv[3 * (4 * t2 + gs) + cc] = __shfl(qpr[t2][cc], r + 16 * gs, 64);
#pragma unroll
        for (int q = 0; q < 6; ++q) qp4[q] = make_float4(qv[4 * q], qv[4 * q + 1], qv[4 * q + 2], qv[4 * q + 3]);
    }
}

template <bool VEC4, bool FUSE = false, bool PROJ = false, bool KFRAG = false, bool KF = false, bool HELP = true>
__global__ __launch_bounds__(512) void ipa_scores_kernel(pf_ipa_attn_args a, int nrb, int rows_per_block, int LP, int SLD) {
    extern __shared__ __attribute__((aligned(16))) float smem[];
    constexpr bool KSPLIT = PROJ && !FUSE;
    const int L = a.L;
    float* KP = smem;
    float* MJ = KP + LP * KPS;
    float* VP = MJ + LP;
    float* SW = VP + (PROJ ? pj_vp_floats(LP) : LP * VPS);

    const int tid = threadIdx.x, wave = tid >> 6, lane = tid & 63;
    const int r = lane & 15, g = lane >> 4;
    const int lid = xcd_remap(blockIdx.x, gridDim.x);
    const int rb = lid % nrb;
    const int h = (lid / nrb) % H;
    const int b = lid / (nrb * H);
    const size_t rowb = (size_t)b * L;
    const int ntq = rows_per_block >> 4;
    const bool helper = PROJ && HELP && wave >= ntq;
    const int i0 = rb * rows_per_block + (helper ? wave - ntq : wave) * 16;
    const int Le = a.key_end ? min(__builtin_amdgcn_readfirstlane(a.key_end[b]), L) : L;
    const int kt = (Le + 15) >> 4, ktf = Le >> 4;
    const bool wave_on = i0 < Le;
    if (rb * rows_per_block >= Le) return;
    const int LPe = 16 * kt;
    PROFS(0);

    const int iq = max(min(i0 + r, Le - 1), 0);
    float4 qf[8];
    float4 qp4[6];
    if constexpr (!PROJ) {
        const float* qrow = a.proj + (rowb + iq) * a.ldp + h * C + 4 * g;
#pragma unroll
        for (int s = 0; s < 8; ++s) qf[s] = *reinterpret_cast<const float4*>(qrow + 16 * s);
#pragma unroll
        for (int q = 0; q < 6; ++q) qp4[q] = *reinterpret_cast<const float4*>(a.qp + (rowb + iq) * 192 + h * 24 + 4 * q);
    }
    const float mi = a.mask[rowb + iq];
    const float gamma = softplusf2(a.head_w[h]) * 0.09622504486493763f;
    const float* kbase = a.proj + rowb * a.ldp + OFF_KV + h * 2 * C + 4 * g;
    const char* kfr_u = nullptr;
    if constexpr (PROJ) {
        const int VTG = (L + 31) & ~31;
        kfr_u = reinterpret_cast<const char*>(a.att_vt) + (((size_t)b * H + h) * 512 * VTG + (size_t)8 * (VTG >> 5) * 1024) * sizeof(_Float16);
    }
    auto loadk = [&](int t, float4 (&kf)[8]) {
        if constexpr (KSPLIT) {
            const char* kt_u = kfr_u + (size_t)t * 8192;
#pragma unroll
            for (int s = 0; s < 4; ++s) {
                kf[s] = *reinterpret_cast<const float4*>(kt_u + s * 2048 + (unsigned)lane * 16u);
                kf[4 + s] = *reinterpret_cast<const float4*>(kt_u + s * 2048 + 1024 + (unsigned)lane * 16u);
            }
        } else if constexpr (PROJ) {
            const char* kt_u = kfr_u + (size_t)t * 8192;
#pragma unroll
            for (int s = 0; s < 8; ++s) kf[s] = *reinterpret_cast<const float4*>(kt_u + s * 1024 + (unsigned)lane * 16u);
        } else if constexpr (KFRAG) {
            const float* kt_f = a.k_frag + ((((size_t)b * H + h) * (L >> 4) + t) * 8) * 256 + lane * 4;
#pragma unroll
            for (int s = 0; s < 8; ++s) kf[s] = *reinterpret_cast<const float4*>(kt_f + s * 256);
        } else {
            const float* krow = kbase + (size_t)min(16 * t + r, Le - 1) * a.ldp;
#pragma unroll
            for (int s = 0; s < 8; ++s) kf[s] = *reinterpret_cast<const float4*>(krow + 16 * s);
        }
    };
    float4 kf[8], kn[8];
    half8 qh[4], ql[4];
    if constexpr (!PROJ) { if (wave_on) loadk(0, kf); }

    if constexpr (PROJ) {
        for (int j = tid; j < LPe; j += blockDim.x) MJ[j] = j < L ? a.mask[rowb + min(j, L - 1)] : 0.f;
        unsigned char* WS = reinterpret_cast<unsigned char*>(SW);
        float* QPW = reinterpret_cast<float*>(WS + PJ_STAGE_B) + (helper ? 0 : wave) * 16 * 24;
        float* PB = reinterpret_cast<float*>(WS + PJ_STAGE_B) + ntq * 16 * 24;
        const int role = HELP ? ((int)(blockDim.x >> 6) > ntq ? (helper ? 2 : 1) : 0) : 0;
        const int VTG = (L + 31) & ~31;
        _Float16* VTH = reinterpret_cast<_Float16*>(const_cast<void*>(a.att_vt)) + ((size_t)b * H + h) * 512 * VTG;
        proj_head<KSPLIT, KF>(a, rowb, iq, h, i0 + r, LPe, wave_on, role, helper ? wave - ntq : wave, KP, reinterpret_cast<_Float16*>(VP), pj_vtl(LP), VTH, VTG, WS, QPW,
                  PB, qf, qp4, lane, wave, (int)(blockDim.x >> 6));
        __syncthreads();
        if (!wave_on || helper) return;
        loadk(0, kf);
#pragma unroll
        for (int s = 0; KSPLIT && s < 4; ++s) {
            const float v[8] = {qf[2 * s].x, qf[2 * s].y, qf[2 * s].z, qf[2 * s].w, qf[2 * s + 1].x, qf[2 * s + 1].y, qf[2 * s + 1].z, qf[2 * s + 1].w};
#pragma unroll
            for (int j = 0; j < 8; ++j) qh[s][j] = (_Float16)v[j];
            pf_pin(qh[s]);
#pragma unroll
            for (int j = 0; j < 8; ++j) ql[s][j] = (_Float16)(v[j] - (float)qh[s][j]);
        }
    } else {
    {
        const int nth = blockDim.x;
        constexpr int KB = 2, VB = 3;
        float4 k4[KB], v4[VB];
        float mj0 = 0.f;
#pragma unroll
        for (int u = 0; u < KB; ++u) {
            const int idx = min(tid + u * nth, LPe * 6 - 1), j = idx / 6, q = idx - j * 6;
            k4[u] = *reinterpret_cast<const float4*>(a.kp + (rowb + min(j, L - 1)) * 192 + h * 24 + 4 * q);
        }
        mj0 = a.mask[rowb + min(tid, L - 1)];
        mj0 = tid < L ? mj0 : 0.f;
#pragma unroll
        for (int u = 0; u < VB; ++u) {
            const int idx = min(tid + u * nth, LPe * 9 - 1), j = idx / 9, q = idx - j * 9;
            v4[u] = *reinterpret_cast<const float4*>(a.vp + (rowb + min(j, L - 1)) * 288 + h * 36 + 4 * q);
        }
        asm volatile("" : "+v"(k4[0].x), "+v"(k4[0].y), "+v"(k4[0].z), "+v"(k4[0].w), "+v"(k4[1].x), "+v"(k4[1].y), "+v"(k4[1].z), "+v"(k4[1].w), "+v"(mj0));
        asm volatile("" : "+v"(v4[0].x), "+v"(v4[0].y), "+v"(v4[0].z), "+v"(v4[0].w), "+v"(v4[1].x), "+v"(v4[1].y), "+v"(v4[1].z), "+v"(v4[1].w),
                          "+v"(v4[2].x), "+v"(v4[2].y), "+v"(v4[2].z), "+v"(v4[2].w));
#pragma unroll
        for (int u = 0; u < KB; ++u) {
            const int idx = tid + u * nth, j = idx / 6, q = idx - j * 6;
            if (idx < LPe * 6) *reinterpret_cast<float4*>(KP + j * KPS + 4 * q) = k4[u];
        }
        if (tid < LPe) MJ[tid] = mj0;
#pragma unroll
        for (int u = 0; u < VB; ++u) {
            const int idx = tid + u * nth, j = idx / 9, q = idx - j * 9;
            if (idx < LPe * 9) *reinterpret_cast<float4*>(VP + j * VPS + 4 * q) = v4[u];
        }
        for (int idx = tid + KB * nth; idx < LPe * 6; idx += nth) {
            const int j = idx / 6, q = idx - j * 6;
            const float4 v = *reinterpret_cast<const float4*>(a.kp + (rowb + min(j, L - 1)) * 192 + h * 24 + 4 * q);
            *reinterpret_cast<float4*>(KP + j * KPS + 4 * q) = v;
        }
        for (int j = tid + nth; j < LPe; j += nth) MJ[j] = j < L ? a.mask[rowb + j] : 0.f;
        for (int idx = tid + VB * nth; idx < LPe * 9; idx += nth) {
            const int j = idx / 9, q = idx - j * 9;
            *reinterpret_cast<float4*>(VP + j * VPS + 4 * q) = *reinterpret_cast<const float4*>(a.vp + (rowb + min(j, L - 1)) * 288 + h * 36 + 4 * q);
        }
    }
    __syncthreads();
    if (!wave_on) return;
    }
    PROFS(1);

    const float scale_qk = 0.051031036307982884f;
    const float* brow = a.bias + (((size_t)b * H + h) * L + iq) * L;
    float* srow = SW + (size_t)wave * 16 * SLD + r * SLD + 4 * g;
    float mx = -3.0e38f;
    auto qk_tile = [&](int t, const float4 (&kf)[8], auto tail) {
        constexpr bool TAIL = decltype(tail)::value;
        const int jb = 16 * t + 4 * g;
        float bj[4];
        if constexpr (VEC4 && !TAIL) {
            const float4 bv = *reinterpret_cast<const float4*>(brow + jb);
            bj[0] = bv.x; bj[1] = bv.y; bj[2] = bv.z; bj[3] = bv.w;
        } else {
#pragma unroll
            for (int e = 0; e < 4; ++e) bj[e] = brow[TAIL ? min(jb + e, L - 1) : jb + e];
        }
        f32x4 acc = {0.f, 0.f, 0.f, 0.f}, acc2 = {0.f, 0.f, 0.f, 0.f};
        if constexpr (KSPLIT) {
#pragma unroll
            for (int s = 0; s < 4; ++s) {
                const half8 kh = __builtin_bit_cast(half8, kf[s]), kl = __builtin_bit_cast(half8, kf[4 + s]);
                acc = mfma_h(kh, qh[s], acc);
                acc2 = mfma_h(kh, ql[s], acc2);
                acc2 = mfma_h(kl, qh[s], acc2);
            }
        } else {
#pragma unroll
            for (int s = 0; s < 8; s += 2) {
                acc = mfma16(kf[s].x, qf[s].x, acc);   acc2 = mfma16(kf[s + 1].x, qf[s + 1].x, acc2);
                acc = mfma16(kf[s].y, qf[s].y, acc);   acc2 = mfma16(kf[s + 1].y, qf[s + 1].y, acc2);
                acc = mfma16(kf[s].z, qf[s].z, acc);   acc2 = mfma16(kf[s + 1].z, qf[s + 1].z, acc2);
                acc = mfma16(kf[s].w, qf[s].w, acc);   acc2 = mfma16(kf[s + 1].w, qf[s + 1].w, acc2);
            }
        }
        acc += acc2;
        float sv[4];
#pragma unroll
        for (int e = 0; e < 4; ++e) {
            const int j = jb + e;
            const float* kp = KP + j * KPS;
            f32x2 d2 = {0.f, 0.f};
#pragma unroll
            for (int q = 0; q < 6; ++q) {
                const float4 kq = *reinterpret_cast<const float4*>(kp + 4 * q);
                const f32x2 da = (f32x2){qp4[q].x, qp4[q].y} - (f32x2){kq.x, kq.y};
                const f32x2 db = (f32x2){qp4[q].z, qp4[q].w} - (f32x2){kq.z, kq.w};
                d2 = __builtin_elementwise_fma(da, da, d2);
                d2 = __builtin_elementwise_fma(db, db, d2);
            }
            float v = acc[e] * scale_qk + bj[e];
            v = v + (-0.5f) * (gamma * (d2[0] + d2[1]));
            v = v + 1e5f * (mi * MJ[j] - 1.f);
            if constexpr (TAIL) v = j < Le ? v : -3.0e38f;
            sv[e] = v;
            mx = fmaxf(mx, v);
// ... 599 lines not shown
#pragma unroll
        for (int k = 0; k < NP; ++k) {
            const int idx = lane + 64 * k, hh = idx / (LPU / 4), j = 4 * (idx % (LPU / 4));
            if (2 * LPU % 64 == 0 || idx < 2 * LPU) {
                const float4 v = pv[k];
                float* d = PL + hh * LDP + ((j >> 2) & 3);
                const int u = j >> 4;
                d[pdz_slot(u, 0)] = j < Le ? v.x : 0.f;
                d[pdz_slot(u, 1)] = j + 1 < Le ? v.y : 0.f;
                d[pdz_slot(u, 2)] = j + 2 < Le ? v.z : 0.f;
                d[pdz_slot(u, 3)] = j + 3 < Le ? v.w : 0.f;
            }
        }
    } else {
        for (int idx = lane; idx < LPU * 8; idx += 64) {
            const int hh = idx / LPU, j = idx - hh * LPU;
            PL[hh * LDP + pdz_slot(j >> 4, j & 3) + ((j >> 2) & 3)] = j < Le ? ld_boff<float>(prow, 4u * (unsigned)(hh * L * L + j)) : 0.f;
        }
    }
    asm volatile("s_waitcnt lgkmcnt(0)" ::: "memory");
    __builtin_amdgcn_wave_barrier();
    f32x4 acc[4];
#pragma unroll
    for (int t = 0; t < 4; ++t) acc[t] = (f32x4){0.f, 0.f, 0.f, 0.f};
    const float* pl = PL + (r & 7) * LDP;
#pragma unroll
    for (int u = 0; u < NU; ++u) {
        const float4 pa = *reinterpret_cast<const float4*>(pl + pdz_slot(u, g));
        if constexpr (D16) {
#pragma unroll
            for (int t = 0; t < 4; ++t) bv[u][t] = (float)bv16[u][t];
        }
        acc[0] = mfma16(pa.x, bv[u][0], acc[0]);
        acc[1] = mfma16(pa.y, bv[u][1], acc[1]);
        acc[2] = mfma16(pa.z, bv[u][2], acc[2]);
        acc[3] = mfma16(pa.w, bv[u][3], acc[3]);
    }
    if (g < 2) {
        float* f = a.feats + (size_t)row * PF_IPA_FEATS + 1408;
#pragma unroll
        for (int e = 0; e < 4; ++e) f[(unsigned)((4 * g + e) * 16 + r)] = ((acc[0][e] + acc[1][e]) + (acc[2][e] + acc[3][e])) + bdz;
    }
}

template <int NG, int NU, bool D16, bool V4>
__device__ __forceinline__ void pair_dz_pick(const pf_ipa_attn_args& a, float* PL, long row, long b, long i, int Le, int nge, int lane) {
    if constexpr (NU <= 2) pair_dz_row<NG, NU, D16, V4>(a, PL, row, b, i, Le, lane);
    else {
        if (nge > NU - 2) pair_dz_row<NG, NU, D16, V4>(a, PL, row, b, i, Le, lane);
        else pair_dz_pick<NG, NU - 2, D16, V4>(a, PL, row, b, i, Le, nge, lane);
    }
}

template <int NG, bool D16 = false>
__global__ __launch_bounds__(256, NG <= 8 ? 8 : NG <= 11 ? 5 : 4) void ipa_pair_dz_kernel(pf_ipa_attn_args a) {
    extern __shared__ __attribute__((aligned(16))) float smem[];
    const int tid = threadIdx.x, wave = __builtin_amdgcn_readfirstlane(tid >> 6), lane = tid & 63;
    const int L = a.L;
    const long row = (long)blockIdx.x * 4 + wave;
    if (row >= (long)a.B * L) return;
    const long b = (unsigned)row / (unsigned)L, i = row - b * L;
    const int Le = a.key_end ? min(__builtin_amdgcn_readfirstlane(a.key_end[b]), L) : L;
    if (i >= Le) return;
    float* PL = smem + wave * 8 * (16 * NG + 8);
    if ((L & 3) == 0) pair_dz_pick<NG, NG, D16, true>(a, PL, row, b, i, Le, (Le + 15) >> 4, lane);
    else pair_dz_pick<NG, NG, D16, false>(a, PL, row, b, i, Le, (Le + 15) >> 4, lane);
}

template <int NG>
__global__ __launch_bounds__(256) void ipa_pair_dz16_kernel(pf_ipa_attn_args a) {
    constexpr int LPZ = 16 * NG;
    extern __shared__ __attribute__((aligned(16))) float smem[];
    const int tid = threadIdx.x, wave = tid >> 6, lane = tid & 63;
    const int ks = (lane & 3) | ((lane >> 4) << 2), q = (lane >> 2) & 3;
    const int L = a.L;
    const long row = (long)blockIdx.x * 4 + wave;
    if (row >= (long)a.B * L) return;
    const long b = row / L, i = row - b * L;
    const int Le = a.key_end ? min(__builtin_amdgcn_readfirstlane(a.key_end[b]), L) : L;
    if (i >= Le) return;
    const int nge = (Le + 15) >> 4;
    float* PL = smem + wave * 8 * LPZ;
    const _Float16* drow = reinterpret_cast<const _Float16*>(a.dz) + (size_t)row * L * 16 + 4 * q;
    half4 d[NG];
#pragma unroll
    for (int u = 0; u < NG; ++u)
        if (u < nge) d[u] = *reinterpret_cast<const half4*>(drow + (size_t)min(16 * u + ks, L - 1) * 16);
    if ((L & 3) == 0) {
        for (int idx = lane; idx < LPZ * 2; idx += 64) {
            const int hh = idx / (LPZ / 4), j = 4 * (idx - hh * (LPZ / 4));
            float4 v = make_float4(0.f, 0.f, 0.f, 0.f);
            if (j < Le) {
                v = *reinterpret_cast<const float4*>(a.p_out + ((b * H + hh) * L + i) * L + j);
                if (j + 1 >= Le) v.y = 0.f;
                if (j + 2 >= Le) v.z = 0.f;
                if (j + 3 >= Le) v.w = 0.f;
            }
            *reinterpret_cast<float4*>(PL + hh * LPZ + j) = v;
        }
    } else {
        for (int idx = lane; idx < LPZ * 8; idx += 64) {
            const int hh = idx / LPZ, j = idx - hh * LPZ;
            PL[idx] = j < Le ? a.p_out[((b * H + hh) * L + i) * L + j] : 0.f;
        }
    }
    asm volatile("s_waitcnt lgkmcnt(0)" ::: "memory");
    __builtin_amdgcn_wave_barrier();
    float v[32];
#pragma unroll
    for (int k = 0; k < 32; ++k) v[k] = 0.f;
#pragma unroll
    for (int u = 0; u < NG; ++u) {
        if (u < nge) {
            const float d0 = (float)d[u][0], d1 = (float)d[u][1], d2 = (float)d[u][2], d3 = (float)d[u][3];
#pragma unroll
            for (int h = 0; h < 8; ++h) {
                const float ph = PL[h * LPZ + 16 * u + ks];
                v[4 * h] += ph * d0; v[4 * h + 1] += ph * d1; v[4 * h + 2] += ph * d2; v[4 * h + 3] += ph * d3;
            }
        }
    }
    float w[16], x[8], y[4], z2[2];
    {
        const bool hi = lane & 1;
#pragma unroll
        for (int k = 0; k < 16; ++k) {
            const float send = hi ? v[k] : v[k + 16], keep = hi ? v[k + 16] : v[k];
            w[k] = keep + lane_xor1(send);
        }
    }
    {
        const bool hi = lane & 2;
#pragma unroll
        for (int k = 0; k < 8; ++k) {
            const float send = hi ? w[k] : w[k + 8], keep = hi ? w[k + 8] : w[k];
            x[k] = keep + lane_xor2(send);
        }
    }
#pragma unroll
    for (int k = 0; k < 4; ++k) {
        auto rr = __builtin_amdgcn_permlane16_swap(__float_as_uint(x[k]), __float_as_uint(x[k + 4]), false, false);
        y[k] = __uint_as_float(rr[0]) + __uint_as_float(rr[1]);
    }
#pragma unroll
    for (int k = 0; k < 2; ++k) {
        auto rr = __builtin_amdgcn_permlane32_swap(__float_as_uint(y[k]), __float_as_uint(y[k + 2]), false, false);
        z2[k] = __uint_as_float(rr[0]) + __uint_as_float(rr[1]);
    }
    const int h = ((lane & 1) << 2) | (lane & 2) | ((lane >> 4) & 1), c = 4 * q + 2 * (lane >> 5);
    const float2 bd = *reinterpret_cast<const float2*>(a.b_dz + c);
    *reinterpret_cast<float2*>(a.feats + (size_t)row * PF_IPA_FEATS + 1408 + h * 16 + c) = make_float2(z2[0] + bd.x, z2[1] + bd.y);
}

}

extern "C" int pf_ipa_proj_inside_ok(int L, int f16_mode) {
    if (L < 1) return 0;
    const int LP = (L + 15) & ~15, SLD = LP + 4 < 36 ? 36 : LP + 4, tiles = LP >> 4;
    if (f16_mode) {
        if ((L & 15) != 0 || tiles > WMAX) return 0;
        const int L32 = (L + 31) & ~31, SLD16 = L32 + 4 < 36 ? 36 : L32 + 4;
        const size_t fixed16 = ((size_t)L * KPS + L) * sizeof(float);
        const size_t swb = (size_t)tiles * 16 * SLD16 * sizeof(float), stg = (size_t)PJ16_STAGE_B + (size_t)tiles * 1536 + (size_t)PJ_TILES * 64;
        const size_t lds16 = fixed16 + (swb > stg ? swb : stg) + ((size_t)L * KLS + (size_t)PF_ATT_VROWS * (L32 + 8)) * sizeof(_Float16);
        return lds16 <= 160 * 1024;
    }
    if ((L & 3) != 0) return 0;
    const size_t fixed = ((size_t)LP * KPS + LP + (size_t)pj_vp_floats(LP)) * sizeof(float), per_wave = (size_t)16 * SLD * sizeof(float);
    if (fixed + per_wave > 160 * 1024) return 0;
    int wmax = (int)((160 * 1024 - fixed) / per_wave);
    wmax = wmax > WMAX ? WMAX : wmax;
    if (tiles > WMAX && tiles % WMAX != 0 && wmax > 4) wmax = 4;
    if (wmax < 1) return 0;
    const int nrb = (tiles + wmax - 1) / wmax, wpb = (tiles + nrb - 1) / nrb;
    if (nrb != 1) return 0;
    const size_t lds = fixed + wpb * per_wave;
    const size_t need = fixed + (size_t)PJ_STAGE_B + (size_t)wpb * 16 * 24 * sizeof(float) + (size_t)PJ_TILES * 16 * sizeof(float);
    return (lds > need ? lds : need) <= 160 * 1024;
}

int pf_ipa_split_launch(const pf_ipa_attn_args* a, hipStream_t s) {
    const int L = a->L;
    int rc = 0;
    const bool pj16 = a->s_in && a->att_mode == 2 && (L & 15) == 0;
    if (a->k_from_s && !a->s_in) return PF_E_BADARG;
    if (a->att_mode == 1) return PF_E_BADARG;
    const bool planes = ((a->att_qk && a->att_vt) || pj16) && a->att_mode == 2 && (L & 15) == 0;
    const bool fuse = a->fused_pair && a->dz && (planes ? a->dz_f16 != 0 : a->dz_f16 == 0);
    if (!fuse && !a->p_out) return PF_E_BADARG;
    {
        const int LP = (L + 15) & ~15, SLD = LP + 4 < 36 ? 36 : LP + 4;
        const int tiles = LP >> 4;
        const bool pj = a->s_in != nullptr && !pj16;
        const size_t fixed = ((size_t)LP * KPS + LP + (size_t)(pj ? pj_vp_floats(LP) : LP * VPS)) * sizeof(float), per_wave = (size_t)16 * SLD * sizeof(float);
        int wmax = (int)((160 * 1024 - fixed) / per_wave);
        wmax = wmax > WMAX ? WMAX : wmax;
        if (tiles > WMAX && tiles % WMAX != 0 && wmax > 4) wmax = 4;
        if (wmax < 1) return PF_E_TOOLARGE;
        const int nrb = (tiles + wmax - 1) / wmax;
        const int wpb = (tiles + nrb - 1) / nrb;
        const size_t lds = fixed + wpb * per_wave;
        static PfOncePerDevice attr_set;
        if (attr_set.first()) {
            (void)hipFuncSetAttribute((const void*)ipa_scores_kernel<true>, hipFuncAttributeMaxDynamicSharedMemorySize, 160 * 1024);
            (void)hipFuncSetAttribute((const void*)ipa_scores_kernel<false>, hipFuncAttributeMaxDynamicSharedMemorySize, 160 * 1024);
            (void)hipFuncSetAttribute((const void*)ipa_scores_kernel<true, true>, hipFuncAttributeMaxDynamicSharedMemorySize, 160 * 1024);
            (void)hipFuncSetAttribute((const void*)ipa_scores_kernel<false, true>, hipFuncAttributeMaxDynamicSharedMemorySize, 160 * 1024);
            (void)hipFuncSetAttribute((const void*)ipa_scores_kernel<true, false, false, true>, hipFuncAttributeMaxDynamicSharedMemorySize, 160 * 1024);
            (void)hipFuncSetAttribute((const void*)ipa_scores_kernel<true, true, false, true>, hipFuncAttributeMaxDynamicSharedMemorySize, 160 * 1024);
        }
        if (pj16) {
            if (tiles > WMAX || !a->proj_w_f16 || !a->proj_bias || !fuse) return PF_E_BADARG;
            const int L32 = (L + 31) & ~31, SLD16 = L32 + 4 < 36 ? 36 : L32 + 4;
            const size_t fixed16 = ((size_t)L * KPS + L) * sizeof(float);
            const size_t swb = (size_t)tiles * 16 * SLD16 * sizeof(float), stg = (size_t)PJ16_STAGE_B + (size_t)tiles * 1536 + (size_t)PJ_TILES * 64;
            const size_t lds16 = fixed16 + (swb > stg ? swb : stg) + ((size_t)L * KLS + (size_t)PF_ATT_VROWS * (L32 + 8)) * sizeof(_Float16);
            if (lds16 > 160 * 1024) return PF_E_TOOLARGE;
            static PfOncePerDevice attr_pj16;
            if (attr_pj16.first()) {
                (void)hipFuncSetAttribute((const void*)ipa_scores16_kernel<true, true>, hipFuncAttributeMaxDynamicSharedMemorySize, 160 * 1024);
                (void)hipFuncSetAttribute((const void*)ipa_scores16_kernel<true, true, true>, hipFuncAttributeMaxDynamicSharedMemorySize, 160 * 1024);
            }
            if (a->k_from_s) hipLaunchKernelGGL((ipa_scores16_kernel<true, true, true>), dim3((unsigned)(a->B * H)), dim3(64 * tiles), lds16, s, *a, 1, 16 * tiles, SLD16);
            else hipLaunchKernelGGL((ipa_scores16_kernel<true, true>), dim3((unsigned)(a->B * H)), dim3(64 * tiles), lds16, s, *a, 1, 16 * tiles, SLD16);
            PF_CHECK_LAUNCH();
            return 0;
        }
        if (a->k_frag && (a->s_in || planes || (L & 15) != 0)) return PF_E_BADARG;
        if (pj && (planes || nrb != 1 || (L & 3) != 0 || !a->proj_w_f16 || !a->proj_bias || !a->proj || !a->att_vt || a->ldp < OFF_KV + 2 * H * C)) return PF_E_BADARG;
        if (pj) {
            static PfOncePerDevice attr_pj;
            if (attr_pj.first()) {
                (void)hipFuncSetAttribute((const void*)ipa_scores_kernel<true, false, true, false, false, true>, hipFuncAttributeMaxDynamicSharedMemorySize, 160 * 1024);
                (void)hipFuncSetAttribute((const void*)ipa_scores_kernel<true, true, true, false, false, true>, hipFuncAttributeMaxDynamicSharedMemorySize, 160 * 1024);
                (void)hipFuncSetAttribute((const void*)ipa_scores_kernel<true, false, true, false, true, true>, hipFuncAttributeMaxDynamicSharedMemorySize, 160 * 1024);
                (void)hipFuncSetAttribute((const void*)ipa_scores_kernel<true, true, true, false, true, true>, hipFuncAttributeMaxDynamicSharedMemorySize, 160 * 1024);
                (void)hipFuncSetAttribute((const void*)ipa_scores_kernel<true, false, true, false, false, false>, hipFuncAttributeMaxDynamicSharedMemorySize, 160 * 1024);
                (void)hipFuncSetAttribute((const void*)ipa_scores_kernel<true, true, true, false, false, false>, hipFuncAttributeMaxDynamicSharedMemorySize, 160 * 1024);
                (void)hipFuncSetAttribute((const void*)ipa_scores_kernel<true, false, true, false, true, false>, hipFuncAttributeMaxDynamicSharedMemorySize, 160 * 1024);
                (void)hipFuncSetAttribute((const void*)ipa_scores_kernel<true, true, true, false, true, false>, hipFuncAttributeMaxDynamicSharedMemorySize, 160 * 1024);
            }
            const size_t need = fixed + (size_t)PJ_STAGE_B + (size_t)wpb * 16 * 24 * sizeof(float) + (size_t)PJ_TILES * 16 * sizeof(float);
            const size_t ldsp = lds > need ? lds : need;
            if (ldsp > 160 * 1024) return PF_E_TOOLARGE;
            const int nwv = wpb <= 4 ? 2 * wpb : wpb;
#define PF_SCORES_PJ(FUSEv, KFv) do { \
                if (nwv != wpb) hipLaunchKernelGGL((ipa_scores_kernel<true, FUSEv, true, false, KFv, true>), dim3((unsigned)(a->B * H * nrb)), dim3(64 * nwv), ldsp, s, *a, nrb, 16 * wpb, LP, SLD); \
                else hipLaunchKernelGGL((ipa_scores_kernel<true, FUSEv, true, false, KFv, false>), dim3((unsigned)(a->B * H * nrb)), dim3(64 * nwv), ldsp, s, *a, nrb, 16 * wpb, LP, SLD); } while (0)
            if (a->k_from_s) {
                if (fuse) PF_SCORES_PJ(true, true);
                else PF_SCORES_PJ(false, true);
            } else if (fuse) PF_SCORES_PJ(true, false);
            else PF_SCORES_PJ(false, false);
#undef PF_SCORES_PJ
        } else if (planes) {
            const int L32 = (L + 31) & ~31, SLD16 = L32 + 4 < 36 ? 36 : L32 + 4;
            const size_t fixed16 = ((size_t)L * KPS + L) * sizeof(float), pw16 = (size_t)16 * SLD16 * sizeof(float);
            int wm = (int)((160 * 1024 - fixed16) / pw16);
            wm = wm > WMAX ? WMAX : wm;
            if (tiles > WMAX && tiles % WMAX != 0 && wm > 4) wm = 4;
            if (tiles <= 4 && wm > 2) wm = 2;
            if (wm < 1) return PF_E_TOOLARGE;
            const int nrb16 = (tiles + wm - 1) / wm, wpb16 = (tiles + nrb16 - 1) / nrb16;
            const size_t lds16 = fixed16 + wpb16 * pw16;
            static PfOncePerDevice attr16;
            if (attr16.first()) {
                (void)hipFuncSetAttribute((const void*)ipa_scores16_kernel<false>, hipFuncAttributeMaxDynamicSharedMemorySize, 160 * 1024);
                (void)hipFuncSetAttribute((const void*)ipa_scores16_kernel<true>, hipFuncAttributeMaxDynamicSharedMemorySize, 160 * 1024);
            }
            const dim3 g16((unsigned)(a->B * H * nrb16)), b16(64 * wpb16);
            if (fuse) hipLaunchKernelGGL((ipa_scores16_kernel<true>), g16, b16, lds16, s, *a, nrb16, 16 * wpb16, SLD16);
            else hipLaunchKernelGGL(ipa_scores16_kernel<false>, g16, b16, lds16, s, *a, nrb16, 16 * wpb16, SLD16);
        } else if (a->k_frag) {
            if (fuse) hipLaunchKernelGGL((ipa_scores_kernel<true, true, false, true>), dim3((unsigned)(a->B * H * nrb)), dim3(64 * wpb), lds, s, *a, nrb, 16 * wpb, LP, SLD);
            else hipLaunchKernelGGL((ipa_scores_kernel<true, false, false, true>), dim3((unsigned)(a->B * H * nrb)), dim3(64 * wpb), lds, s, *a, nrb, 16 * wpb, LP, SLD);
        } else if (fuse) {
            if ((L & 3) == 0) hipLaunchKernelGGL((ipa_scores_kernel<true, true>), dim3((unsigned)(a->B * H * nrb)), dim3(64 * wpb), lds, s, *a, nrb, 16 * wpb, LP, SLD);
            else hipLaunchKernelGGL((ipa_scores_kernel<false, true>), dim3((unsigned)(a->B * H * nrb)), dim3(64 * wpb), lds, s, *a, nrb, 16 * wpb, LP, SLD);
        } else if ((L & 3) == 0)
            hipLaunchKernelGGL(ipa_scores_kernel<true>, dim3((unsigned)(a->B * H * nrb)), dim3(64 * wpb), lds, s, *a, nrb, 16 * wpb, LP, SLD);
        else
            hipLaunchKernelGGL(ipa_scores_kernel<false>, dim3((unsigned)(a->B * H * nrb)), dim3(64 * wpb), lds, s, *a, nrb, 16 * wpb, LP, SLD);
        PF_CHECK_LAUNCH();
    }
    if (rc) return rc;
    if (fuse) return 0;
    const int ng = (L + 15) / 16;
    const size_t lds = ((size_t)8 * 16 * ng + ZW * 8 * 64 + 4 * 64 * 4) * sizeof(float);
    const long rows = (long)a->B * L;
    if (ng > 16 || rows > 0x7fffffffL) return PF_E_TOOLARGE;
    if (a->dz) {
        const dim3 gridd((unsigned)((rows + 3) / 4));
        const size_t ldsd = (size_t)4 * 8 * (a->dz_f16 ? 16 * ng : 16 * ng + 8) * sizeof(float);
        switch (ng) {
#define PF_PAIRDZ_CASE(N) case N: if (a->dz_f16) hipLaunchKernelGGL(ipa_pair_dz16_kernel<N>, gridd, dim3(256), ldsd, s, *a); else hipLaunchKernelGGL((ipa_pair_dz_kernel<N, false>), gridd, dim3(256), ldsd, s, *a); break;
            PF_PAIRDZ_CASE(1) PF_PAIRDZ_CASE(2) PF_PAIRDZ_CASE(3) PF_PAIRDZ_CASE(4) PF_PAIRDZ_CASE(5) PF_PAIRDZ_CASE(6) PF_PAIRDZ_CASE(7)
            PF_PAIRDZ_CASE(8) PF_PAIRDZ_CASE(9) PF_PAIRDZ_CASE(10) PF_PAIRDZ_CASE(11) PF_PAIRDZ_CASE(12) PF_PAIRDZ_CASE(13)
            PF_PAIRDZ_CASE(14) PF_PAIRDZ_CASE(15) PF_PAIRDZ_CASE(16)
#undef PF_PAIRDZ_CASE
        }
        PF_CHECK_LAUNCH();
        return 0;
    }
    const dim3 grid((unsigned)rows), blk(64 * ZW);
    switch (ng) {
#define PF_PAIR_CASE(N) case N: if (a->z_f16) hipLaunchKernelGGL((ipa_pair_kernel<N, true>), grid, blk, lds, s, *a); else hipLaunchKernelGGL(ipa_pair_kernel<N>, grid, blk, lds, s, *a); break;
        PF_PAIR_CASE(1) PF_PAIR_CASE(2) PF_PAIR_CASE(3) PF_PAIR_CASE(4) PF_PAIR_CASE(5) PF_PAIR_CASE(6) PF_PAIR_CASE(7) PF_PAIR_CASE(8)
        PF_PAIR_CASE(9) PF_PAIR_CASE(10) PF_PAIR_CASE(11) PF_PAIR_CASE(12) PF_PAIR_CASE(13) PF_PAIR_CASE(14) PF_PAIR_CASE(15) PF_PAIR_CASE(16)
#undef PF_PAIR_CASE
    }
    PF_CHECK_LAUNCH();
    return 0;
}
```

pepflowww_amd/csrc/node_track.hip:

```cpp
#include "common.h"
#include "rigid_dev.h"
#include "../../include/pepflow_hip.h"

#ifdef PF_PROFILE
__device__ long long g_prof[64];
#ifndef PF_PROF_LAST
#define PF_PROF_LAST 1
#endif
#define PROF(i) do { if (LAST == (PF_PROF_LAST != 0) && blockIdx.x == 0 && threadIdx.x == 0) g_prof[i] = clock64(); } while (0)
extern "C" int pf_debug_prof(long long* out, int n) {
    return (int)hipMemcpyFromSymbol(out, HIP_SYMBOL(g_prof), sizeof(long long) * n, 0, hipMemcpyDeviceToHost);
}
#else
#define PROF(i)
#endif

namespace {

constexpr int TR = 16;
constexpr int LDX = 132;
constexpr int LDP = 136;
constexpr int NTHR = 512;
#ifndef PF_NT_MINW
#define PF_NT_MINW 2
#endif

struct Planes { _Float16* h; _Float16* l; };

struct LnParams { float g[8], b[8]; };
__device__ __forceinline__ void ln_load(LnParams& p, const float* __restrict__ g, const float* __restrict__ b) {
    const int sub = threadIdx.x & 15;
    const float4 g0 = *reinterpret_cast<const float4*>(g + 8 * sub), g1 = *reinterpret_cast<const float4*>(g + 8 * sub + 4);
    const float4 b0 = *reinterpret_cast<const float4*>(b + 8 * sub), b1 = *reinterpret_cast<const float4*>(b + 8 * sub + 4);
    p.g[0] = g0.x; p.g[1] = g0.y; p.g[2] = g0.z; p.g[3] = g0.w; p.g[4] = g1.x; p.g[5] = g1.y; p.g[6] = g1.z; p.g[7] = g1.w;
    p.b[0] = b0.x; p.b[1] = b0.y; p.b[2] = b0.z; p.b[3] = b0.w; p.b[4] = b1.x; p.b[5] = b1.y; p.b[6] = b1.z; p.b[7] = b1.w;
}
template <int ROWS = 16>
__device__ __forceinline__ void ln_tile(float* T, const LnParams& p, float mk, Planes out, int m0, int M, float* gout) {
    const int tid = threadIdx.x;
    if (tid < 16 * ROWS) {
        const int row = tid >> 4, sub = tid & 15, m = m0 + row;
        float v[8];
        {
            const float4 a = *reinterpret_cast<const float4*>(T + row * LDX + 8 * sub);
            const float4 b = *reinterpret_cast<const float4*>(T + row * LDX + 8 * sub + 4);
            v[0] = a.x; v[1] = a.y; v[2] = a.z; v[3] = a.w; v[4] = b.x; v[5] = b.y; v[6] = b.z; v[7] = b.w;
        }
        float s = ((v[0] + v[1]) + (v[2] + v[3])) + ((v[4] + v[5]) + (v[6] + v[7]));
        s = row16_sum(s);
        const float mean = s / 128.f;
        float q = 0.f;
#pragma unroll
        for (int c = 0; c < 8; ++c) { const float d = v[c] - mean; q += d * d; }
        q = row16_sum(q);
        const float rstd = rsqrtf(q / 128.f + 1e-5f);
        float y[8];
#pragma unroll
        for (int c = 0; c < 8; ++c) y[c] = ((v[c] - mean) * rstd * p.g[c] + p.b[c]) * mk;
        *reinterpret_cast<float4*>(T + row * LDX + 8 * sub) = make_float4(y[0], y[1], y[2], y[3]);
        *reinterpret_cast<float4*>(T + row * LDX + 8 * sub + 4) = make_float4(y[4], y[5], y[6], y[7]);
        half4 h0, l0, h1, l1;
        const float y0[4] = {y[0], y[1], y[2], y[3]}, y1[4] = {y[4], y[5], y[6], y[7]};
        split4(y0, h0, l0);
        split4(y1, h1, l1);
        *reinterpret_cast<half4*>(out.h + row * LDP + 8 * sub) = h0;
        *reinterpret_cast<half4*>(out.h + row * LDP + 8 * sub + 4) = h1;
        *reinterpret_cast<half4*>(out.l + row * LDP + 8 * sub) = l0;
        *reinterpret_cast<half4*>(out.l + row * LDP + 8 * sub + 4) = l1;
        if (gout && m < M) {
            *reinterpret_cast<float4*>(gout + (size_t)m * 128 + 8 * sub) = make_float4(y[0], y[1], y[2], y[3]);
            *reinterpret_cast<float4*>(gout + (size_t)m * 128 + 8 * sub + 4) = make_float4(y[4], y[5], y[6], y[7]);
        }
    }
}

__device__ __forceinline__ float4 sel4(bool ok, const float4& v) {
    const float f = ok ? 1.f : 0.f;
    return make_float4(v.x * f, v.y * f, v.z * f, v.w * f);
}

__device__ __forceinline__ void put_planes(Planes p, int r, int n, const float (&v)[4]) {
    half4 hi, lo;
    split4(v, hi, lo);
    *reinterpret_cast<half4*>(p.h + r * LDP + n) = hi;
    *reinterpret_cast<half4*>(p.l + r * LDP + n) = lo;
}

template <bool SP, bool DUMP = false, bool PM = false>
__global__ __launch_bounds__(NTHR, PF_NT_MINW) void node_head_kernel(pf_node_head_args a) {
    extern __shared__ __attribute__((aligned(16))) unsigned char smem_raw[];
    constexpr int CK = 256, LDC = CK + 8;
    _Float16* Ch = reinterpret_cast<_Float16*>(smem_raw);
    float* X = reinterpret_cast<float*>(smem_raw + 2 * 2 * TR * LDC * sizeof(_Float16));
    Planes Xa = {reinterpret_cast<_Float16*>(X + TR * LDX), reinterpret_cast<_Float16*>(X + TR * LDX) + TR * LDP};
    const int tid = threadIdx.x, wave = tid >> 6, lane = tid & 63;
    const int r = lane & 15, g = lane >> 4;
    const int m0 = blockIdx.x * TR, M = a.rows;
    if (pf_rows_all_masked(a.key_end, a.key_L, m0, TR, M)) return;
    const int n = wave * 16 + 4 * g;

    constexpr int C0 = PM ? 4 : 0;
    WSplit<1, 8, SP> ws;
    ws.init(a.w_out_f16, 128, PF_IPA_FEATS - C0 * 256, wave * 16);
    ws.prefetch();
    LnParams lnp;
    ln_load(lnp, a.ln_g, a.ln_b);
    const float4 bias_out = *reinterpret_cast<const float4*>(a.b_out + n);
    float4 bias_in[3];
#pragma unroll
    for (int wt = 0; wt < 3; ++wt) bias_in[wt] = *reinterpret_cast<const float4*>(a.b_in + wave * 48 + wt * 16 + 4 * g);
    const int mr = m0 + r;
    const int mrc = mr < M ? mr : M - 1;
    const float rmask_ld = a.mask[mrc];
    const float4 rres_ld = *reinterpret_cast<const float4*>(a.s_in + (size_t)mrc * 128 + n);
    const int srow = tid >> 5, sc4 = tid & 31;
    const bool sok = m0 + srow < M;
    const float* src = a.feats + (size_t)(sok ? m0 + srow : 0) * PF_IPA_FEATS + 4 * sc4;
    constexpr int NCH = PF_IPA_FEATS / CK;
    float4 st[NCH][2];
#pragma unroll
    for (int c = 0; c < NCH; ++c)
#pragma unroll
        for (int hlf = 0; hlf < 2; ++hlf)
            st[c][hlf] = *reinterpret_cast<const float4*>(src + c * CK + hlf * 128);
    auto commit = [&](int c) {
        _Float16* bh = Ch + (c & 1) * 2 * TR * LDC;
        _Float16* bl = bh + TR * LDC;
#pragma unroll
        for (int hlf = 0; hlf < 2; ++hlf) {
            const float4 sv = sel4(sok, st[c][hlf]);
            const float v[4] = {sv.x, sv.y, sv.z, sv.w};
            half4 hi, lo;
            split4(v, hi, lo);
            *reinterpret_cast<half4*>(bh + srow * LDC + hlf * 128 + 4 * sc4) = hi;
            *reinterpret_cast<half4*>(bl + srow * LDC + hlf * 128 + 4 * sc4) = lo;
        }
    };
    if constexpr (PM) {
        auto add4 = [](const float4& p, const float4& q) { return make_float4(p.x + q.x, p.y + q.y, p.z + q.z, p.w + q.w); };
        float4 ev = sel4(sok, st[0][0]), od = sel4(sok, st[0][1]);
#pragma unroll
        for (int c = 1; c < 4; ++c) { ev = add4(ev, sel4(sok, st[c][0])); od = add4(od, sel4(sok, st[c][1])); }
        *reinterpret_cast<float4*>(X + srow * LDX + 4 * sc4) = add4(ev, od);
    }
    commit(C0);
    __syncthreads();
    f32x4 am[1], ac[1];
    acc_zero1<1>(am, ac);
#pragma unroll
    for (int c = C0; c < NCH; ++c) {
        const _Float16* bh = Ch + (c & 1) * 2 * TR * LDC;
        gemm_split16(ws, bh, bh + TR * LDC, LDC, am, ac, (c - C0) * 8, 8);
        if (c + 1 < NCH) commit(c + 1);
        __syncthreads();
    }
    WSplit<3, 4, SP> wq;
    wq.init(a.w_in_f16, 384, 128, wave * 48);
    wq.prefetch();
    {
        const float rmask = rmask_ld * (mr < M ? 1.f : 0.f);
        const float4 rres = sel4(mr < M, rres_ld);
        float4 hs = make_float4(0.f, 0.f, 0.f, 0.f);
        if constexpr (PM) hs = *reinterpret_cast<const float4*>(X + r * LDX + n);
        auto lin = [&](int e, float h) { const float j = join(am[0], ac[0], e); if constexpr (PM) return j + h; else return j; };
        float4 y;
        y.x = (lin(0, hs.x) + bias_out.x) * rmask + rres.x;
        y.y = (lin(1, hs.y) + bias_out.y) * rmask + rres.y;
        y.z = (lin(2, hs.z) + bias_out.z) * rmask + rres.z;
        y.w = (lin(3, hs.w) + bias_out.w) * rmask + rres.w;
        *reinterpret_cast<float4*>(X + r * LDX + n) = y;
        if constexpr (DUMP) { if (mr < M) *reinterpret_cast<float4*>(a.dump_a0 + (size_t)mr * 128 + n) = y; }
    }
    __syncthreads();
    ln_tile(X, lnp, 1.f, Xa, m0, M, a.s_ipa);
    __syncthreads();
    f32x4 qm[3], qc[3];
    acc_zero1<3>(qm, qc);
    gemm_split16(wq, Xa.h, Xa.l, LDP, qm, qc, 0, 4);
    if (mr < M) {
#pragma unroll
        for (int wt = 0; wt < 3; ++wt) {
            float4 y;
            y.x = join(qm[wt], qc[wt], 0) + bias_in[wt].x; y.y = join(qm[wt], qc[wt], 1) + bias_in[wt].y;
            y.z = join(qm[wt], qc[wt], 2) + bias_in[wt].z; y.w = join(qm[wt], qc[wt], 3) + bias_in[wt].w;
            *reinterpret_cast<float4*>(a.qkv + (size_t)mr * 384 + wave * 48 + wt * 16 + 4 * g) = y;
        }
    }
}

constexpr int TR2 = 32;
template <bool SP, bool PM = false>
__global__ __launch_bounds__(NTHR, PF_NT_MINW) void node_head32_kernel(pf_node_head_args a) {
    extern __shared__ __attribute__((aligned(16))) unsigned char smem_raw[];
    constexpr int CK = 256, LDC = CK + 8;
    _Float16* Ch = reinterpret_cast<_Float16*>(smem_raw);
    float* X = reinterpret_cast<float*>(smem_raw + 2 * 2 * TR2 * LDC * sizeof(_Float16));
    Planes Xa = {reinterpret_cast<_Float16*>(X + TR2 * LDX), reinterpret_cast<_Float16*>(X + TR2 * LDX) + TR2 * LDP};
    const int tid = threadIdx.x, wave = tid >> 6, lane = tid & 63;
    const int r = lane & 15, g = lane >> 4;
    int m0 = blockIdx.x * TR2, M = a.rows;
    if (a.key_end) {
        const int tps = (a.key_L + TR2 - 1) / TR2, b = blockIdx.x / tps, i0 = (blockIdx.x - b * tps) * TR2;
        if (i0 >= a.key_end[b]) return;
        m0 = b * a.key_L + i0;
        M = (b + 1) * a.key_L;
    }
    const int n = wave * 16 + 4 * g;

    constexpr int C0 = PM ? 4 : 0;
    WSplit<1, 8, SP> ws;
    ws.init(a.w_out_f16, 128, PF_IPA_FEATS - C0 * 256, wave * 16);
    ws.prefetch();
    LnParams lnp;
    ln_load(lnp, a.ln_g, a.ln_b);
    const float4 bias_out = *reinterpret_cast<const float4*>(a.b_out + n);
    float4 bias_in[3];
#pragma unroll
    for (int wt = 0; wt < 3; ++wt) bias_in[wt] = *reinterpret_cast<const float4*>(a.b_in + wave * 48 + wt * 16 + 4 * g);
    float rmask_ld[2];
    float4 rres_ld[2];
#pragma unroll
    for (int rt = 0; rt < 2; ++rt) {
        const int mr = m0 + rt * 16 + r;
        const int mrc = mr < M ? mr : M - 1;
// ... 342 lines not shown
    auto joined = [&](int rt, const float4& bias, float (&v)[4]) {
        v[0] = join(am[rt][0], ac[rt][0], 0) + bias.x; v[1] = join(am[rt][0], ac[rt][0], 1) + bias.y;
        v[2] = join(am[rt][0], ac[rt][0], 2) + bias.z; v[3] = join(am[rt][0], ac[rt][0], 3) + bias.w;
    };
    auto relu4 = [](float (&v)[4]) {
#pragma unroll
        for (int e = 0; e < 4; ++e) v[e] = fmaxf(v[e], 0.f);
    };
    zero();
    gemm_split16r<1, 4, SP, RT>(ws, Xa.h, Xa.l, LDP, am, ac, 0, 4);
    ws.init(a.w_1_f16, 128, 128, wave * 16);
    ws.prefetch();
#pragma unroll
    for (int rt = 0; rt < RT; ++rt) {
        const float4 rres = sel4(mr[rt] < M, rres_ld[rt]);
        float v[4];
        joined(rt, bias_o, v);
        *reinterpret_cast<float4*>(T1 + (16 * rt + r) * LDX + n) = make_float4(v[0] + rres.x, v[1] + rres.y, v[2] + rres.z, v[3] + rres.w);
        dump4(a.dump[1], rt, v[0] + rres.x, v[1] + rres.y, v[2] + rres.z, v[3] + rres.w);
    }
    __syncthreads();
    ln_tile<TR>(T1, ln1, 1.f, Xb, m0, M, DUMP ? a.dump[2] : nullptr);
    __syncthreads();
    PROF(5);
    zero();
    gemm_split16r<1, 4, SP, RT>(ws, Xb.h, Xb.l, LDP, am, ac, 0, 4);
    ws.init(a.w_2_f16, 128, 128, wave * 16);
    ws.prefetch();
#pragma unroll
    for (int rt = 0; rt < RT; ++rt) {
        float v[4];
        joined(rt, bias_1, v);
        relu4(v);
        put_planes(Xa, 16 * rt + r, n, v);
        dump4(a.dump[3], rt, v[0], v[1], v[2], v[3]);
    }
    __syncthreads();
    PROF(6);
    zero();
    gemm_split16r<1, 4, SP, RT>(ws, Xa.h, Xa.l, LDP, am, ac, 0, 4);
    auto lin2_to_t0 = [&]() {
#pragma unroll
        for (int rt = 0; rt < RT; ++rt) {
            const float4 u = *reinterpret_cast<const float4*>(T1 + (16 * rt + r) * LDX + n);
            float v[4];
            joined(rt, bias_2, v);
            *reinterpret_cast<float4*>(T0 + (16 * rt + r) * LDX + n) = make_float4(v[0] + u.x, v[1] + u.y, v[2] + u.z, v[3] + u.w);
            dump4(a.dump[4], rt, v[0] + u.x, v[1] + u.y, v[2] + u.z, v[3] + u.w);
        }
    };
    if constexpr (!LAST) {
        WSplit<3, 4, SP> wq;
        wq.init(a.w_in_next_f16, 384, 128, wave * 48);
        wq.prefetch();
        lin2_to_t0();
        __syncthreads();
        ln_tile<TR>(T0, ln2, 1.f, Xb, m0, M, a.v_out);
        __syncthreads();
        PROF(7);
        f32x4 qm[RT][3], qc[RT][3];
#pragma unroll
        for (int rt = 0; rt < RT; ++rt) acc_zero1<3>(qm[rt], qc[rt]);
        gemm_split16r<3, 4, SP, RT>(wq, Xb.h, Xb.l, LDP, qm, qc, 0, 4);
#pragma unroll
        for (int rt = 0; rt < RT; ++rt) {
            if (mr[rt] < M) {
#pragma unroll
                for (int wt = 0; wt < 3; ++wt) {
                    float4 y;
                    y.x = join(qm[rt][wt], qc[rt][wt], 0) + bias_in[wt].x; y.y = join(qm[rt][wt], qc[rt][wt], 1) + bias_in[wt].y;
                    y.z = join(qm[rt][wt], qc[rt][wt], 2) + bias_in[wt].z; y.w = join(qm[rt][wt], qc[rt][wt], 3) + bias_in[wt].w;
                    *reinterpret_cast<float4*>(a.qkv_out + (size_t)mr[rt] * 384 + wave * 48 + wt * 16 + 4 * g) = y;
                }
            }
        }
        PROF(8);
    } else {
        ws.init(a.w_post_f16, 128, 128, wave * 16);
        ws.prefetch();
        lin2_to_t0();
        float4 fq = make_float4(1.f, 0.f, 0.f, 0.f);
        float fR[9], fx[3], fmask = 0.f;
        if (tid < TR && m0 + tid < M) {
            const int m = m0 + tid;
            fq = *reinterpret_cast<const float4*>(a.quat_in + (size_t)m * 4);
#pragma unroll
            for (int k = 0; k < 9; ++k) fR[k] = a.rot_in[(size_t)m * 9 + k];
#pragma unroll
            for (int k = 0; k < 3; ++k) fx[k] = a.trans_in[(size_t)m * 3 + k];
            fmask = a.mask[m];
        }
        __syncthreads();
        ln_tile<TR>(T0, ln2, 1.f, Xb, m0, M, DUMP ? a.dump[5] : nullptr);
        __syncthreads();
        PROF(7);
        zero();
        gemm_split16r<1, 4, SP, RT>(ws, Xb.h, Xb.l, LDP, am, ac, 0, 4);
        ws.init(a.w_t1_f16, 128, 128, wave * 16);
        ws.prefetch();
#pragma unroll
        for (int rt = 0; rt < RT; ++rt) {
            const float4 rsipa = sel4(mr[rt] < M, rsipa_ld[rt]);
            float v[4];
            joined(rt, bias_post, v);
            v[0] += rsipa.x; v[1] += rsipa.y; v[2] += rsipa.z; v[3] += rsipa.w;
            *reinterpret_cast<float4*>(T1 + (16 * rt + r) * LDX + n) = make_float4(v[0], v[1], v[2], v[3]);
            put_planes(Xa, 16 * rt + r, n, v);
            dump4(a.dump[6], rt, v[0], v[1], v[2], v[3]);
        }
        __syncthreads();
        PROF(8);
        zero();
        gemm_split16r<1, 4, SP, RT>(ws, Xa.h, Xa.l, LDP, am, ac, 0, 4);
        ws.init(a.w_t2_f16, 128, 128, wave * 16);
        ws.prefetch();
#pragma unroll
        for (int rt = 0; rt < RT; ++rt) {
            float v[4];
            joined(rt, bias_t1, v);
            relu4(v);
            put_planes(Xb, 16 * rt + r, n, v);
            dump4(a.dump[7], rt, v[0], v[1], v[2], v[3]);
        }
        __syncthreads();
        zero();
        gemm_split16r<1, 4, SP, RT>(ws, Xb.h, Xb.l, LDP, am, ac, 0, 4);
        ws.init(a.w_t3_f16, 128, 128, wave * 16);
        ws.prefetch();
#pragma unroll
        for (int rt = 0; rt < RT; ++rt) {
            float v[4];
            joined(rt, bias_t2, v);
            relu4(v);
            put_planes(Xa, 16 * rt + r, n, v);
            dump4(a.dump[8], rt, v[0], v[1], v[2], v[3]);
        }
        __syncthreads();
        zero();
        gemm_split16r<1, 4, SP, RT>(ws, Xa.h, Xa.l, LDP, am, ac, 0, 4);
        const bool do_bb = wave == 0, do_init = a.has_et && wave >= 4;
        if (do_bb) { ws.init(a.w_bb_f16, 16, 128, 0); ws.prefetch(); }
        else if (do_init) { ws.init(a.w_init_f16, 64, 128, (wave - 4) * 16); ws.prefetch(); }
        WSplit<4, 2, SP> wp;
        if (a.has_et) { wp.init(a.w_pre_f16, PF_ET_PRE, 64, wave * 64); wp.prefetch(); }
#pragma unroll
        for (int rt = 0; rt < RT; ++rt) {
            const float4 s0 = *reinterpret_cast<const float4*>(T1 + (16 * rt + r) * LDX + n);
            float v[4];
            joined(rt, bias_t3, v);
            *reinterpret_cast<float4*>(T0 + (16 * rt + r) * LDX + n) = make_float4(v[0] + s0.x, v[1] + s0.y, v[2] + s0.z, v[3] + s0.w);
            dump4(a.dump[9], rt, v[0] + s0.x, v[1] + s0.y, v[2] + s0.z, v[3] + s0.w);
        }
        __syncthreads();
        ln_tile<TR>(T0, ln3, lnmask_ld * (lnrow < M ? 1.f : 0.f), Xb, m0, M, a.s_out);
        __syncthreads();
        PROF(9);
        if (do_bb || do_init) {
            zero();
            gemm_split16r<1, 4, SP, RT>(ws, Xb.h, Xb.l, LDP, am, ac, 0, 4);
#pragma unroll
            for (int rt = 0; rt < RT; ++rt) {
                float v[4];
                if (do_bb) {
                    joined(rt, bias_bb, v);
                    if (g < 2) *reinterpret_cast<float4*>(U + (16 * rt + r) * 8 + 4 * g) = make_float4(v[0], v[1], v[2], v[3]);
                    if constexpr (DUMP) { if (g < 2 && mr[rt] < M) *reinterpret_cast<float4*>(a.dump[10] + (size_t)mr[rt] * 8 + 4 * g) = make_float4(v[0], v[1], v[2], v[3]); }
                } else {
                    joined(rt, bias_init, v);
                    put_planes(Xa, 16 * rt + r, (wave - 4) * 16 + 4 * g, v);
                }
            }
        }
        __syncthreads();
        if (tid < TR && m0 + tid < M) {
            const int m = m0 + tid;
            float Ro[9], xo[3];
            float4 qo;
            rigid_update_dev(fq, fR, fx, U + tid * 8, fmask, qo, Ro, xo);
            *reinterpret_cast<float4*>(a.quat_out + (size_t)m * 4) = qo;
#pragma unroll
            for (int k = 0; k < 3; ++k) a.trans_out[(size_t)m * 3 + k] = xo[k];
#pragma unroll
            for (int k = 0; k < 9; ++k) a.rot_out[(size_t)m * 9 + k] = Ro[k];
        }
        PROF(10);
        if (a.has_et) {
            f32x4 pm[RT][4], pc[RT][4];
#pragma unroll
            for (int rt = 0; rt < RT; ++rt) acc_zero1<4>(pm[rt], pc[rt]);
            PROF(12);
            gemm_split16r<4, 2, SP, RT>(wp, Xa.h, Xa.l, LDP, pm, pc, 0, 2);
            PROF(13);
#pragma unroll
            for (int rt = 0; rt < RT; ++rt) {
                if (mr[rt] < M) {
#pragma unroll
                    for (int wt = 0; wt < 4; ++wt) {
                        float4 y;
                        y.x = join(pm[rt][wt], pc[rt][wt], 0) + bias_pre[wt].x; y.y = join(pm[rt][wt], pc[rt][wt], 1) + bias_pre[wt].y;
                        y.z = join(pm[rt][wt], pc[rt][wt], 2) + bias_pre[wt].z; y.w = join(pm[rt][wt], pc[rt][wt], 3) + bias_pre[wt].w;
                        *reinterpret_cast<float4*>(a.pre + (size_t)mr[rt] * PF_ET_PRE + wave * 64 + wt * 16 + 4 * g) = y;
                    }
                }
            }
        } else if (a.logits_out) {
            __syncthreads();
            Planes Xc = {reinterpret_cast<_Float16*>(T0), reinterpret_cast<_Float16*>(T0) + TR * LDP};
#pragma unroll
            for (int net = 0; net < 2; ++net) {
                const int nout = net ? 5 : 20, ntile = net ? 1 : 2;
                ws.init(a.h_w[net][0], 128, 128, wave * 16);
                ws.prefetch();
                const float4 hb0 = *reinterpret_cast<const float4*>(a.h_b[net][0] + n), hb1 = *reinterpret_cast<const float4*>(a.h_b[net][1] + n);
                zero();
                gemm_split16r<1, 4, SP, RT>(ws, Xb.h, Xb.l, LDP, am, ac, 0, 4);
                ws.init(a.h_w[net][1], 128, 128, wave * 16);
                ws.prefetch();
#pragma unroll
                for (int rt = 0; rt < RT; ++rt) {
                    float v[4];
                    joined(rt, hb0, v);
                    relu4(v);
                    put_planes(Xa, 16 * rt + r, n, v);
                }
                __syncthreads();
                zero();
                gemm_split16r<1, 4, SP, RT>(ws, Xa.h, Xa.l, LDP, am, ac, 0, 4);
                if (wave < ntile) { ws.init(a.h_w[net][2], 16 * ntile, 128, wave * 16); ws.prefetch(); }
#pragma unroll
                for (int rt = 0; rt < RT; ++rt) {
                    float v[4];
                    joined(rt, hb1, v);
                    relu4(v);
                    put_planes(Xc, 16 * rt + r, n, v);
                }
                __syncthreads();
                if (wave < ntile) {
                    const float4 hb2 = *reinterpret_cast<const float4*>(a.h_b[net][2] + n);
                    zero();
                    gemm_split16r<1, 4, SP, RT>(ws, Xc.h, Xc.l, LDP, am, ac, 0, 4);
#pragma unroll
                    for (int rt = 0; rt < RT; ++rt) {
                        if (mr[rt] < M) {
                            float* op = (net ? a.ang_out : a.logits_out) + (size_t)mr[rt] * nout;
                            float v[4];
                            joined(rt, hb2, v);
#pragma unroll
                            for (int e = 0; e < 4; ++e)
                                if (n + e < nout) op[n + e] = v[e];
                        }
                    }
                }
                __syncthreads();
            }
        }
        PROF(11);
    }
}

constexpr int LDF = 640 + 8;
template <bool SP>
__global__ __launch_bounds__(NTHR) void input_mixer_kernel(pf_input_mixer_args a) {
    extern __shared__ __attribute__((aligned(16))) unsigned char smem_raw[];
    Planes Xf = {reinterpret_cast<_Float16*>(smem_raw), reinterpret_cast<_Float16*>(smem_raw) + TR * LDF};
    Planes Xa = {Xf.l + TR * LDF, Xf.l + TR * LDF + TR * LDP};
    const int tid = threadIdx.x, wave = tid >> 6, lane = tid & 63;
    const int r = lane & 15, g = lane >> 4;
    const int m0 = blockIdx.x * TR, M = a.B * a.L;
    const int n = wave * 16 + 4 * g;
    WSplit<1, 8, SP> w0;
    w0.init(a.w0_f16, 128, 640, wave * 16);
    w0.prefetch();
    const float4 b0 = *reinterpret_cast<const float4*>(a.b0 + n);
    const float4 b2 = *reinterpret_cast<const float4*>(a.b2 + n);
    const int mr = m0 + r, mrc = mr < M ? mr : M - 1;
    const float rmask = a.mask[mrc] * (mr < M ? 1.f : 0.f);
    __shared__ float TC[2][128];
    const int b_first = m0 / a.L, b_last = min(m0 + TR - 1, M - 1) / a.L;
    const bool tc_shared = b_last - b_first < 2;
    if (tc_shared && tid < 128 * (b_last - b_first + 1)) {
        const int bi = tid >> 7, k = tid & 127;
        const float tt = a.t[b_first + bi] * 2056.f;
        TC[bi][k] = k < 64 ? sinf(tt * a.time_freq[k]) : cosf(tt * a.time_freq[k - 64]);
    }
    __syncthreads();
    for (int idx = tid; idx < TR * 160; idx += NTHR) {
        const int row = idx / 160, c4 = idx - row * 160;
        const int m = min(m0 + row, M - 1);
        const int b = m / a.L;
        float v[4];
        if (c4 < 32) {
            const float4 t = *reinterpret_cast<const float4*>(a.node_embed + (size_t)m * 128 + 4 * c4);
            v[0] = t.x; v[1] = t.y; v[2] = t.z; v[3] = t.w;
        } else if (c4 < 64) {
            long long sq = a.seqs[m];
            sq = sq < 0 ? 0 : (sq > 21 ? 21 : sq);
            const float4 t = *reinterpret_cast<const float4*>(a.seq_table + sq * 128 + 4 * (c4 - 32));
            v[0] = t.x; v[1] = t.y; v[2] = t.z; v[3] = t.w;
        } else {
            const float tt = a.t[b] * 2056.f;
#pragma unroll
            for (int e = 0; e < 4; ++e) {
                const int c = 4 * c4 + e;
                float x;
                if (c < 384 && tc_shared) x = TC[b - b_first][c - 256];
                else if (c < 320) x = sinf(tt * a.time_freq[c - 256]);
                else if (c < 384) x = cosf(tt * a.time_freq[c - 320]);
                else if (c < 629) {
                    const int q = c - 384, d = q / 49, k = q - d * 49;
                    const float ang = a.angles[(size_t)m * 5 + d];
                    if (k == 0) x = ang;
                    else if (k < 25) x = sinf(ang * a.ang_freq[k - 1]);
                    else x = cosf(ang * a.ang_freq[k - 25]);
                } else x = 0.f;
                v[e] = x;
            }
        }
        half4 hi, lo;
        split4(v, hi, lo);
        *reinterpret_cast<half4*>(Xf.h + row * LDF + 4 * c4) = hi;
        *reinterpret_cast<half4*>(Xf.l + row * LDF + 4 * c4) = lo;
    }
    if (tid < TR && m0 + tid < M) {
        float R[9], q[4];
#pragma unroll
        for (int k = 0; k < 9; ++k) R[k] = a.rot[(size_t)(m0 + tid) * 9 + k];
        rot_to_quat_dev(R, q);
        *reinterpret_cast<float4*>(a.quat + (size_t)(m0 + tid) * 4) = make_float4(q[0], q[1], q[2], q[3]);
    }
    __syncthreads();
    f32x4 am[1], ac[1];
    acc_zero1<1>(am, ac);
    gemm_split16(w0, Xf.h, Xf.l, LDF, am, ac, 0, 20);
    WSplit<1, 4, SP> w2;
    w2.init(a.w2_f16, 128, 128, wave * 16);
    w2.prefetch();
    {
        const float v[4] = {fmaxf(join(am[0], ac[0], 0) + b0.x, 0.f), fmaxf(join(am[0], ac[0], 1) + b0.y, 0.f),
                            fmaxf(join(am[0], ac[0], 2) + b0.z, 0.f), fmaxf(join(am[0], ac[0], 3) + b0.w, 0.f)};
        put_planes(Xa, r, n, v);
    }
    __syncthreads();
    acc_zero1<1>(am, ac);
    gemm_split16(w2, Xa.h, Xa.l, LDP, am, ac, 0, 4);
    if (mr < M) {
        float4 y;
        y.x = (join(am[0], ac[0], 0) + b2.x) * rmask; y.y = (join(am[0], ac[0], 1) + b2.y) * rmask;
        y.z = (join(am[0], ac[0], 2) + b2.z) * rmask; y.w = (join(am[0], ac[0], 3) + b2.w) * rmask;
        *reinterpret_cast<float4*>(a.s_out + (size_t)mr * 128 + n) = y;
    }
}

}

extern "C" int pf_input_mixer_fwd(const pf_input_mixer_args* a, pf_stream_t stream) {
    if (!a || !a->node_embed || !a->seq_table || !a->seqs || !a->t || !a->time_freq || !a->ang_freq || !a->angles || !a->w0_f16 ||
        !a->b0 || !a->w2_f16 || !a->b2 || !a->mask || !a->rot || !a->quat || !a->s_out || a->B <= 0 || a->L <= 0)
        return PF_E_BADARG;
    const int rows = a->B * a->L;
    const size_t lds = (size_t)2 * TR * LDF * sizeof(_Float16) + (size_t)2 * TR * LDP * sizeof(_Float16);
    if (a->single_pass) hipLaunchKernelGGL(input_mixer_kernel<true>, dim3((unsigned)((rows + TR - 1) / TR)), dim3(NTHR), lds, (hipStream_t)stream, *a);
    else hipLaunchKernelGGL(input_mixer_kernel<false>, dim3((unsigned)((rows + TR - 1) / TR)), dim3(NTHR), lds, (hipStream_t)stream, *a);
    PF_CHECK_LAUNCH();
    return 0;
}

extern "C" int pf_node_head_fwd(const pf_node_head_args* a, pf_stream_t stream) {
    if (!a || !a->feats || !a->s_in || !a->mask || !a->w_out_f16 || !a->b_out || !a->ln_g || !a->ln_b || !a->w_in_f16 ||
        !a->b_in || !a->s_ipa || !a->qkv || a->rows <= 0)
        return PF_E_BADARG;
    const size_t lds = (size_t)2 * 2 * TR * 264 * sizeof(_Float16) + (size_t)TR * LDX * sizeof(float) +
                       (size_t)2 * TR * LDP * sizeof(_Float16);
    if (a->rows >= pf_cu_count() * TR2 && !a->dump_a0) {
        const size_t lds2 = (size_t)2 * 2 * TR2 * 264 * sizeof(_Float16) + (size_t)TR2 * LDX * sizeof(float) + (size_t)2 * TR2 * LDP * sizeof(_Float16);
        static PfOncePerDevice attr_set;
        if (attr_set.first()) {
            (void)hipFuncSetAttribute((const void*)node_head32_kernel<true>, hipFuncAttributeMaxDynamicSharedMemorySize, 160 * 1024);
            (void)hipFuncSetAttribute((const void*)node_head32_kernel<false>, hipFuncAttributeMaxDynamicSharedMemorySize, 160 * 1024);
            (void)hipFuncSetAttribute((const void*)node_head32_kernel<true, true>, hipFuncAttributeMaxDynamicSharedMemorySize, 160 * 1024);
            (void)hipFuncSetAttribute((const void*)node_head32_kernel<false, true>, hipFuncAttributeMaxDynamicSharedMemorySize, 160 * 1024);
        }
        const bool per_sample = a->key_end && a->key_L > 0 && a->rows % a->key_L == 0;
        pf_node_head_args aa = *a;
        if (!per_sample) aa.key_end = nullptr;
        const dim3 grid(per_sample ? (unsigned)((a->rows / a->key_L) * ((a->key_L + TR2 - 1) / TR2)) : (unsigned)((a->rows + TR2 - 1) / TR2));
        a = &aa;
        if (a->o_premul) {
            if (a->single_pass) hipLaunchKernelGGL((node_head32_kernel<true, true>), grid, dim3(NTHR), lds2, (hipStream_t)stream, *a);
            else hipLaunchKernelGGL((node_head32_kernel<false, true>), grid, dim3(NTHR), lds2, (hipStream_t)stream, *a);
        } else if (a->single_pass) hipLaunchKernelGGL(node_head32_kernel<true>, grid, dim3(NTHR), lds2, (hipStream_t)stream, *a);
        else hipLaunchKernelGGL(node_head32_kernel<false>, grid, dim3(NTHR), lds2, (hipStream_t)stream, *a);
        PF_CHECK_LAUNCH();
        return 0;
    }
    if (a->dump_a0) {
        if (a->single_pass || a->o_premul) return PF_E_BADARG;
        hipLaunchKernelGGL((node_head_kernel<false, true>), dim3((unsigned)((a->rows + TR - 1) / TR)), dim3(NTHR), lds, (hipStream_t)stream, *a);
        PF_CHECK_LAUNCH();
        return 0;
    }
    if (a->o_premul) {
        if (a->single_pass) hipLaunchKernelGGL((node_head_kernel<true, false, true>), dim3((unsigned)((a->rows + TR - 1) / TR)), dim3(NTHR), lds, (hipStream_t)stream, *a);
        else hipLaunchKernelGGL((node_head_kernel<false, false, true>), dim3((unsigned)((a->rows + TR - 1) / TR)), dim3(NTHR), lds, (hipStream_t)stream, *a);
    } else if (a->single_pass) hipLaunchKernelGGL(node_head_kernel<true>, dim3((unsigned)((a->rows + TR - 1) / TR)), dim3(NTHR), lds, (hipStream_t)stream, *a);
    else hipLaunchKernelGGL(node_head_kernel<false>, dim3((unsigned)((a->rows + TR - 1) / TR)), dim3(NTHR), lds, (hipStream_t)stream, *a);
    PF_CHECK_LAUNCH();
    return 0;
}

extern "C" int pf_node_tfmr_fwd(const pf_node_tfmr_args* a, pf_stream_t stream) {
    if (!a || !a->qkv || !a->resid || !a->mask || !a->w_o_f16 || !a->b_o || !a->n1_g || !a->n1_b || !a->w_1_f16 || !a->b_1 ||
        !a->w_2_f16 || !a->b_2 || !a->n2_g || !a->n2_b || a->B <= 0 || a->L <= 0)
        return PF_E_BADARG;
    if (!a->last && (!a->w_in_next_f16 || !a->b_in_next || !a->qkv_out || !a->v_out)) return PF_E_BADARG;
    if (a->last && (!a->s_ipa || !a->w_post_f16 || !a->b_post || !a->w_t1_f16 || !a->b_t1 || !a->w_t2_f16 || !a->b_t2 ||
                    !a->w_t3_f16 || !a->b_t3 || !a->nt_g || !a->nt_b || !a->w_bb_f16 || !a->b_bb || !a->s_out || !a->quat_in ||
                    !a->rot_in || !a->trans_in || !a->quat_out || !a->rot_out || !a->trans_out))
        return PF_E_BADARG;
    if (a->last && a->has_et && (!a->w_init_f16 || !a->b_init || !a->w_pre_f16 || !a->b_pre || !a->pre)) return PF_E_BADARG;
    if (a->last && !a->has_et && a->logits_out) {
        if (!a->ang_out) return PF_E_BADARG;
        for (int net = 0; net < 2; ++net)
            for (int l = 0; l < 3; ++l)
                if (!a->h_w[net][l] || !a->h_b[net][l]) return PF_E_BADARG;
    }
    const int LP = (a->L + 15) / 16 * 16;
    const int LDS_S = LP + 4;
    const int tiles16 = (a->L + 15) / 16;
    auto lds_of = [&](int rt) {
        const int tr = 16 * rt;
        return ((size_t)2 * tr * LDX + tr * 8 + (size_t)tr * 4 * LDS_S) * sizeof(float) + (size_t)4 * tr * LDP * sizeof(_Float16);
    };
    const int RTn = ((long)a->B * tiles16 > pf_cu_count() && a->L > 16 && !a->dump[0] && lds_of(2) <= (size_t)160 * 1024) ? 2 : 1;
    const int TRn = 16 * RTn;
    const size_t lds = lds_of(RTn);
    if (lds > 160 * 1024) return PF_E_TOOLARGE;
    const int tiles = (a->L + TRn - 1) / TRn;
    const dim3 grid((unsigned)(a->B * tiles));
    const int variant = (RTn == 2 ? 4 : 0) + (a->last ? 2 : 0) + (a->single_pass ? 1 : 0);
    static PfOncePerDevice attr_set[8];
#define PF_NT_CASE(V, LASTV, SPV, RTV)                                                                                           \
    case V:                                                                                                                      \
        if (attr_set[V].first()) {                                                                                                      \
            (void)hipFuncSetAttribute((const void*)node_tfmr_kernel<LASTV, SPV, RTV>, hipFuncAttributeMaxDynamicSharedMemorySize, \
                                      160 * 1024);                                                                               \
        }                                                                                                                        \
        hipLaunchKernelGGL((node_tfmr_kernel<LASTV, SPV, RTV>), grid, dim3(NTHR), lds, (hipStream_t)stream, *a, LP, LDS_S);      \
        break;
    if (a->dump[0]) {
        for (int k = 0; k < (a->last ? 11 : 5); ++k)
            if (!a->dump[k]) return PF_E_BADARG;
        if (a->single_pass || RTn != 1) return PF_E_BADARG;
        static PfOncePerDevice dattr[2];
        if (a->last) {
            if (dattr[1].first()) { (void)hipFuncSetAttribute((const void*)node_tfmr_kernel<true, false, 1, true>, hipFuncAttributeMaxDynamicSharedMemorySize, 160 * 1024); }
            hipLaunchKernelGGL((node_tfmr_kernel<true, false, 1, true>), grid, dim3(NTHR), lds, (hipStream_t)stream, *a, LP, LDS_S);
        } else {
            if (dattr[0].first()) { (void)hipFuncSetAttribute((const void*)node_tfmr_kernel<false, false, 1, true>, hipFuncAttributeMaxDynamicSharedMemorySize, 160 * 1024); }
            hipLaunchKernelGGL((node_tfmr_kernel<false, false, 1, true>), grid, dim3(NTHR), lds, (hipStream_t)stream, *a, LP, LDS_S);
        }
        PF_CHECK_LAUNCH();
        return 0;
    }
    switch (variant) {
        PF_NT_CASE(0, false, false, 1) PF_NT_CASE(1, false, true, 1) PF_NT_CASE(2, true, false, 1) PF_NT_CASE(3, true, true, 1)
        PF_NT_CASE(4, false, false, 2) PF_NT_CASE(5, false, true, 2) PF_NT_CASE(6, true, false, 2) PF_NT_CASE(7, true, true, 2)
    }
#undef PF_NT_CASE
    PF_CHECK_LAUNCH();
    return 0;
}
```

pepflowww_amd/engine.py:

```python
import ctypes as C
import math
from collections import OrderedDict

import torch

from . import _capi

N_BLOCKS = 6


def _f32(t):
    return t.detach().to(torch.float32).contiguous()


LO_SCALE = 2048.0


F16_MAX = 65504.0


_DEFERRED = None


def _range_error(name):
# ... 365 lines not shown
        g = lambda k: _f32(sd["ga_encoder." + k]).to(device)
        self.t = {}
        t = self.t
        w0 = g("res_feat_mixer.0.weight")
        t["mix0.w"] = torch.nn.functional.pad(w0, (0, 640 - w0.shape[1])).contiguous()
        t["mix0.b"] = g("res_feat_mixer.0.bias")
        t["mix2.w"], t["mix2.b"] = g("res_feat_mixer.2.weight"), g("res_feat_mixer.2.bias")
        t["mix0.w16"], t["mix2.w16"] = split_f16(t["mix0.w"]), split_f16(t["mix2.w"])
        t["seq_table"] = g("current_seq_embedder.weight")
        t["ang_freq"] = g("angles_embedder.freq_bands")
        half = 64
        freq = torch.exp(torch.arange(half, dtype=torch.float32) * -(math.log(2056) / (half - 1)))
        t["time_freq"] = freq.to(device)
        for net in ("seq_net", "angle_net"):
            for i in (0, 2, 4):
                t[f"{net}.{i}.w"], t[f"{net}.{i}.b"] = g(f"{net}.{i}.weight"), g(f"{net}.{i}.bias")
                t[f"{net}.{i}.w16"] = split_f16(t[f"{net}.{i}.w"])
                if i == 4:
                    t[f"{net}.{i}.b"] = torch.nn.functional.pad(t[f"{net}.{i}.b"], (0, 32 - t[f"{net}.{i}.b"].numel())).contiguous()
        for net in ("seq_net", "angle_net"):
            h = torch.relu(t[f"{net}.0.b"])
            h = torch.relu(t[f"{net}.2.w"] @ h + t[f"{net}.2.b"])
            t[f"{net}.const"] = (t[f"{net}.4.w"] @ h + g(f"{net}.4.bias")).contiguous()
        for b in range(N_BLOCKS):
            p = f"trunk.ipa_{b}."
            t[f"{b}.proj.w"] = torch.cat([g(p + "linear_q.weight"), g(p + "linear_kv.weight"),
                                          g(p + "linear_q_points.weight"), g(p + "linear_kv_points.weight")], 0).contiguous()
            t[f"{b}.proj.b"] = torch.cat([g(p + "linear_q.bias"), g(p + "linear_kv.bias"),
                                          g(p + "linear_q_points.bias"), g(p + "linear_kv_points.bias")], 0).contiguous()
            t[f"{b}.proj.w16"] = split_f16(t[f"{b}.proj.w"])
            t[f"{b}.projp.w16"], t[f"{b}.projp.b"] = pack_ipa_projection(t[f"{b}.proj.w"], t[f"{b}.proj.b"])
            for nm in ("linear_b", "down_z", "linear_out"):
                t[f"{b}.{nm}.w"], t[f"{b}.{nm}.b"] = g(p + nm + ".weight"), g(p + nm + ".bias")
            t[f"{b}.linear_out.w16"] = split_f16(t[f"{b}.linear_out.w"])
            t[f"{b}.projm.w"], t[f"{b}.projm.b"] = fold_linear_out_into_values(t[f"{b}.proj.w"], t[f"{b}.proj.b"], t[f"{b}.linear_out.w"])
            t[f"{b}.projpm.w16"], t[f"{b}.projpm.b"] = pack_ipa_projection(t[f"{b}.projm.w"], t[f"{b}.projm.b"])
            t[f"{b}.linear_out.w16m"] = split_f16(t[f"{b}.linear_out.w"][:, 1024:].contiguous())
            wk_, bk_ = fold_keys_into_queries(t[f"{b}.projm.w"], t[f"{b}.projm.b"])
            t[f"{b}.projpmk.w16"], t[f"{b}.projpmk.b"] = pack_ipa_projection(wk_, bk_)
            wk_, bk_ = fold_keys_into_queries(t[f"{b}.proj.w"], t[f"{b}.proj.b"])
            t[f"{b}.projpk.w16"], t[f"{b}.projpk.b"] = pack_ipa_projection(wk_, bk_)
            t[f"{b}.head_w"] = g(p + "head_weights")
            t[f"{b}.ipa_ln.w"], t[f"{b}.ipa_ln.b"] = g(f"trunk.ipa_ln_{b}.weight"), g(f"trunk.ipa_ln_{b}.bias")
            for l in range(2):
                q = f"trunk.seq_tfmr_{b}.layers.{l}."
                t[f"{b}.{l}.in.w"], t[f"{b}.{l}.in.b"] = g(q + "self_attn.in_proj_weight"), g(q + "self_attn.in_proj_bias")
                t[f"{b}.{l}.out.w"], t[f"{b}.{l}.out.b"] = g(q + "self_attn.out_proj.weight"), g(q + "self_attn.out_proj.bias")
                for nm in ("linear1", "linear2", "norm1", "norm2"):
                    t[f"{b}.{l}.{nm}.w"], t[f"{b}.{l}.{nm}.b"] = g(q + nm + ".weight"), g(q + nm + ".bias")
                for nm in ("in", "out", "linear1", "linear2"):
                    t[f"{b}.{l}.{nm}.w16"] = split_f16(t[f"{b}.{l}.{nm}.w"])
            t[f"{b}.post.w"], t[f"{b}.post.b"] = g(f"trunk.post_tfmr_{b}.weight"), g(f"trunk.post_tfmr_{b}.bias")
            t[f"{b}.post.w16"] = split_f16(t[f"{b}.post.w"])
            q = f"trunk.node_transition_{b}."
            for nm in ("linear_1", "linear_2", "linear_3", "ln"):
                t[f"{b}.nt.{nm}.w"], t[f"{b}.nt.{nm}.b"] = g(q + nm + ".weight"), g(q + nm + ".bias")
            for nm in ("linear_1", "linear_2", "linear_3"):
                t[f"{b}.nt.{nm}.w16"] = split_f16(t[f"{b}.nt.{nm}.w"])
            t[f"{b}.bb.w"], t[f"{b}.bb.b"] = g(f"trunk.bb_update_{b}.linear.weight"), g(f"trunk.bb_update_{b}.linear.bias")
            t[f"{b}.bb.w16"] = split_f16(t[f"{b}.bb.w"])
            t[f"{b}.bb.b8"] = torch.nn.functional.pad(t[f"{b}.bb.b"], (0, 2)).contiguous()
            if b < N_BLOCKS - 1:
                q = f"trunk.edge_transition_{b}."
                t[f"{b}.et.init.w"], t[f"{b}.et.init.b"] = g(q + "initial_embed.weight"), g(q + "initial_embed.bias")
                w1, b1 = g(q + "trunk.0.weight"), g(q + "trunk.0.bias")
                wf, bf = g(q + "final_layer.weight"), g(q + "final_layer.bias")
                t[f"{b}.et.b2"] = g(q + "trunk.2.bias")
                t[f"{b}.et.stream"] = pack_et_stream(w1[:, :64], g(q + "trunk.2.weight"), wf)
                t[f"{b}.et.streamf"] = pack_et_stream(w1[:, :64], g(q + "trunk.2.weight"), wf, z_frag=True)
                t[f"{b}.et.wbfrags"] = pack_bias_frags(g(f"trunk.ipa_{b + 1}.linear_b.weight"), g(f"trunk.ipa_{b + 1}.down_z.weight"))
                t[f"{b}.et.stream32"] = pack_et_stream32(w1[:, :64], g(q + "trunk.2.weight"), wf)
                t[f"{b}.et.stream32f"] = pack_et_stream32(w1[:, :64], g(q + "trunk.2.weight"), wf, z_frag=True)
                t[f"{b}.et.stream64f"] = pack_et_stream64(w1[:, :64], g(q + "trunk.2.weight"), wf)
                t[f"{b}.et.stream64h"] = pack_et_stream64(w1[:, :64], g(q + "trunk.2.weight"), wf, f16=True)
                t[f"{b}.et.wbfrags32"] = pack_bias_frags32(g(f"trunk.ipa_{b + 1}.linear_b.weight"), g(f"trunk.ipa_{b + 1}.down_z.weight"))
                t[f"{b}.et.pre.w"] = torch.cat([w1[:, 64:128], w1[:, 128:192], wf[:, 64:128], wf[:, 128:192]], 0).contiguous()
                t[f"{b}.et.pre.b"] = torch.cat([torch.zeros_like(b1), b1, torch.zeros_like(bf), bf], 0).contiguous()
                t[f"{b}.et.ln.w"], t[f"{b}.et.ln.b"] = g(q + "layer_norm.weight"), g(q + "layer_norm.bias")
                t[f"{b}.et.init.w16"], t[f"{b}.et.pre.w16"] = split_f16(t[f"{b}.et.init.w"]), split_f16(t[f"{b}.et.pre.w"])

    def __getitem__(self, k):
        return self.t[k]


class DenoiseEngine:
    OPTIONS = ("fused_proj", "fused_pair", "et_v4", "et_v5", "et_zfrag", "k_frag", "et_last_store", "o_premul", "k_fold")
    K_FOLD = True
    O_PREMUL = True

    def __init__(self, weights, B, L, device, precision="fp32", owner=None, options=None):
        assert precision in ("fp32", "f16"), precision
        self.precision = precision
        opt = dict(options or {})
        assert set(opt) <= set(self.OPTIONS), sorted(set(opt) - set(self.OPTIONS))
        self.options = opt
        self._owner = owner
        self.lib = _capi.load()
        self.w = weights
        self.B, self.L, self.device = B, L, device
        rows = B * L
        self.rows = rows
        e = lambda *s, dt=torch.float32: torch.zeros(*s, dtype=dt, device=device)
        self.t = e(B)
        self.rot_t, self.trans_t, self.ang_t = e(rows, 9), e(rows, 3), e(rows, 5)
        self.seq_t = e(rows, dt=torch.int64)
        self.node_embed = e(rows, 128)
        self.edge_embed = None
        self.mask = e(rows)
        self.feat = e(rows, 640)
        self.s, self.u, self.v, self.ta, self.tb = (e(rows, 128) for _ in range(5))
        self.proj = e(rows, 3744)
        self.qp, self.kp, self.vp = e(rows, 192), e(rows, 192), e(rows, 288)
        self.feats = e(rows, 1536)
        self.qkv, self.qkv2 = e(rows, 384), e(rows, 384)
        self.upd = e(rows, 8)
        self.quat, self.rot, self.trans = e(rows, 4), e(rows, 9), e(rows, 3)
        self.n64, self.pre = e(rows, 64), e(rows, 512)
        self.z16 = precision == "f16" and (L % 16 == 0) and (64 <= L <= 256)
        self.zbuf = e(B, L, L, 64, dt=torch.float16 if self.z16 else torch.float32)
        self.edge16 = e(B, L, L, 64, dt=torch.float16) if self.z16 else None
        self.pair_bias = e(B, 8, L, L)
        self.pair_bias0 = e(B, 8, L, L)
        dzt = torch.float16 if self.z16 else torch.float32
        self.pair_dz = e(B, L, L, 16, dt=dzt) if 64 <= L <= 256 else None
        self.pair_dz0 = e(B, L, L, 16, dt=dzt) if 64 <= L <= 256 else None
        self._dz0_f32 = e(B, L, L, 16) if (self.z16 and self.pair_dz0 is not None) else None
        self.fused_pair = self.pair_dz is not None and opt.get("fused_pair", self.z16 or L <= 64)
        self.attn_p = None if self.fused_pair else e(B, 8, L, L)
        self.et_v4 = opt.get("et_v4", precision == "fp32")
        self.et_rows = int(self.lib.pf_edge_transition_v4_tile_rows()) if self.et_v4 else int(self.lib.pf_edge_transition_tile_rows(int(precision == "f16")))
        zf_ok = L % 16 == 0 and self.pair_dz is not None and opt.get("et_zfrag", True)
        self.z_frag = zf_ok and ((self.et_v4 and not self.z16) or (self.z16 and not self.et_v4 and self.et_rows == 16))
        self.et_v5h = bool(self.z_frag and self.z16 and 32 <= L <= 4096 and opt.get("et_v5", True))
        self.edge_frag = e(B, L, L, 64, dt=torch.float16 if self.z16 else torch.float32) if self.z_frag else None
        self.et_v5 = bool(self.et_v4 and self.z_frag and not self.z16 and 32 <= L <= 4096 and opt.get("et_v5", True))
        self.et_nib, self.et_njb = (L + self.et_rows - 1) // self.et_rows, (L + 15) // 16
        self.et_tiles = e(B * self.et_nib * self.et_njb, dt=torch.int32)
        self.et_ntiles = e(1, dt=torch.int32)
        self.key_end = e(B, dt=torch.int32)
        self.att_planes = precision == "f16" and (L % 16 == 0) and (64 <= L <= 256)
        can_pj = 64 <= L <= 128 and ((precision == "fp32" and L % 4 == 0 and not self.att_planes) or
                                     (precision == "f16" and self.att_planes and self.fused_pair))
        can_pj = bool(can_pj and self.lib.pf_ipa_proj_inside_ok(L, int(precision == "f16")))
        self.fused_proj = can_pj and opt.get("fused_proj", True)
        self.o_premul = bool(opt.get("o_premul", self.O_PREMUL and precision == "fp32"))
        self.k_fold = bool(self.fused_proj and opt.get("k_fold", self.K_FOLD and precision == "fp32"))
        self.att_qk = self.att_vt = None
        if self.att_planes and not self.fused_proj:
            self.att_qk = torch.zeros(rows * 2048, dtype=torch.float16, device=device)
            self.att_vt = torch.zeros(B * 8 * 11 * ((L + 31) // 32) * 512, dtype=torch.float16, device=device)
        self.att_vt32 = None
        if self.fused_proj and not self.att_planes:
            self.att_vt32 = torch.zeros(B * 8 * 512 * ((L + 31) // 32 * 32), dtype=torch.float16, device=device)
        self.k_frag = None
        if (not self.fused_proj and precision == "fp32" and L % 16 == 0 and self.pair_dz is not None and
                opt.get("k_frag", True)):
            self.k_frag = e(rows, 1024)
        self.logits, self.ang_raw = e(rows, 20), e(rows, 5)
        self.row_on = torch.ones(max(1, rows // 16), dtype=torch.int32, device=device) if L % 16 == 0 else None
        self._keep = []
        self.plan = None
        self.plan_version = 0
        self.active_rows = rows
        self._edge_in = None
        self._samplers = OrderedDict()
        self._warm = False
        self._side = None

    def edge_buffer(self):
        if self._edge_in is None:
            self._edge_in = torch.zeros(self.B, self.L, self.L, 64, dtype=torch.float32, device=self.device)
        return self._edge_in

    SAMPLER_CACHE = 2

    def sampler(self, num_steps, flags=(True, True, True), cond=False, guide=False):
        from .sampler import DeviceSampler
        key = (int(num_steps), tuple(bool(f) for f in flags)) + ((True,) if cond else ()) + (("guide",) if guide else ())
        smp = self._samplers.get(key)
        if smp is None:
            try:
                smp = DeviceSampler(self, num_steps, flags, cond=cond, guide=guide)
            except torch.cuda.OutOfMemoryError:
                self._samplers.clear()
                if self._owner is not None:
                    self._owner._make_room(self)
                torch.cuda.empty_cache()
                smp = DeviceSampler(self, num_steps, flags, cond=cond, guide=guide)
            self._samplers[key] = smp
            while len(self._samplers) > self.SAMPLER_CACHE:
                self._samplers.popitem(last=False)
        else:
            self._samplers.move_to_end(key)
        return smp

    RANGE_WARN = 0.5 * F16_MAX

    def operand_range(self):
        bufs = {"node_state": self.s, "pair_tensor": self.zbuf, "et_residue_terms": self.pre, "ipa_features": self.feats,
                "ipa_projection": self.proj}
        vals = torch.stack([torch.nan_to_num(b.detach().abs().amax().float(), nan=float("inf")) if b.numel() else torch.zeros((), device=self.device)
                            for b in bufs.values()]).tolist()
        rep = dict(zip(bufs, vals))
        rep["limit"] = F16_MAX
        rep["ok"] = all(v <= self.RANGE_WARN for v in vals)
        return rep

    def nbytes(self):
        seen, total = set(), 0
        holders = [self] + list(self._samplers.values())
        for h in holders:
            for v in vars(h).values():
                if torch.is_tensor(v) and v.device.type != "cpu":
                    st = v.untyped_storage()
                    if st.data_ptr() not in seen:
                        seen.add(st.data_ptr())
                        total += st.nbytes()
        return total

    def _linear(self, x, w, b, y, N, K, relu=False, mask_pre=False, mask_post=False, residual=None, ln=None, w16=None):
        a = _capi.LinearArgs()
        a.x, a.ldx = x.data_ptr(), x.shape[1]
        a.w, a.ldw = w.data_ptr(), w.shape[1]
        if w16 is not None:
            a.w_f16 = w16.data_ptr()
        a.bias = b.data_ptr() if b is not None else None
        a.y, a.ldy = y.data_ptr(), y.shape[1]
        a.M, a.N, a.K = self.rows, N, K
        a.relu = int(relu)
        a.row_mask = self.mask.data_ptr() if (mask_pre or mask_post) else None
        a.mask_pre, a.mask_post = int(mask_pre), int(mask_post)
        if residual is not None:
            a.residual, a.ldr = residual.data_ptr(), residual.shape[1]
        if ln is not None:
            a.ln_gamma, a.ln_beta, a.ln_eps = ln[0].data_ptr(), ln[1].data_ptr(), 1e-5
        self._keep.append(a)
        return (self.lib.pf_linear_fwd, C.byref(a), "pf_linear_fwd")

    def bind_context(self, node_embed, edge_embed, res_mask):
        B, L = self.B, self.L
        self.want_rows(None)
        self.node_embed.copy_(node_embed.reshape(B * L, 128))
        self.mask.copy_(res_mask.reshape(B * L).to(torch.float32))
        self._refresh_work_lists(res_mask.reshape(B, L))
        ee = edge_embed
        if ee.dtype != torch.float32 or not ee.is_contiguous():
            ee = ee.to(torch.float32).contiguous()
        _capi.dptr(ee, name="edge_embed")
        rebuild = self.plan is None or self.edge_embed is None or self.edge_embed.data_ptr() != ee.data_ptr()
        self.edge_embed = ee
        if self.z16:
            self.edge16.copy_(ee.reshape(B, L, L, 64))
        if self.z_frag:
            if self.et_v5h:
                z16_to_frag64(self.edge16, out=self.edge_frag)
            elif self.z16:
                z16_to_frag(self.edge16, out=self.edge_frag)
            else:
                z_to_frag(ee.reshape(B, L, L, 64), out=self.edge_frag)
        _capi.check(self.lib.pf_pair_bias_fwd(ee.data_ptr(), self.w["0.linear_b.w"].data_ptr(), self.w["0.linear_b.b"].data_ptr(),
                                              self.pair_bias0.data_ptr(), B, L, _capi.stream_ptr()), "pf_pair_bias_fwd")
        if self.pair_dz0 is not None:
            la = _capi.LinearArgs()
            la.x, la.ldx, la.w, la.ldw = ee.data_ptr(), 64, self.w["0.down_z.w"].data_ptr(), 64
            y = self._dz0_f32 if self.z16 else self.pair_dz0
            la.y, la.ldy, la.M, la.N, la.K = y.data_ptr(), 16, B * L * L, 16, 64
            _capi.check(self.lib.pf_linear_fwd(C.byref(la), _capi.stream_ptr()), "pf_linear_fwd (down_z of edge_embed)")
            if self.z16:
                self.pair_dz0.copy_(y)
        if rebuild:
            self._build_plan()

    def _refresh_work_lists(self, mask):
        B, L, R, nib, njb = self.B, self.L, self.et_rows, self.et_nib, self.et_njb
        m = mask.to(torch.bool)
        rows = torch.nn.functional.pad(m, (0, nib * R - L)).view(B, nib, R).any(-1)
        cols = torch.nn.functional.pad(m, (0, njb * 16 - L)).view(B, njb, 16).any(-1)
        active = (rows[:, :, None] & cols[:, None, :]).reshape(-1)
        order = torch.sort((~active).to(torch.int8), stable=True).indices
        self.et_tiles.copy_(order.to(torch.int32))
        self.et_ntiles.copy_(active.sum().to(torch.int32).reshape(1))
        self.key_end.copy_((m.to(torch.int32) * torch.arange(1, L + 1, device=m.device, dtype=torch.int32)).amax(-1))
        ke_sum, m_sum = torch.stack([self.key_end.sum().to(torch.int64), m.sum().to(torch.int64)]).tolist()
        self.active_rows = int(ke_sum)
        for la in getattr(self, "_proj_args", []):
            la.active_rows = self.active_rows
        for ta in getattr(self, "_tfmr_args", []):
            ta.key_end = self.key_end.data_ptr() if self.active_rows < B * L else None
        self.padded = int(m_sum) < B * L
        if self.padded:
            self.zbuf.zero_()
            self.pair_bias.zero_()
            if self.pair_dz is not None:
                self.pair_dz.zero_()

    def _build_plan(self):
        w, lib = self.w, self.lib
        self._keep = []
        self._proj_args = []
        self._tfmr_args = []
        plan = []
        B, L, rows = self.B, self.L, self.rows
        lin = self._linear

        ma = _capi.InputMixerArgs()
        ma.node_embed, ma.seq_table, ma.seqs = self.node_embed.data_ptr(), w["seq_table"].data_ptr(), self.seq_t.data_ptr()
        ma.t, ma.time_freq, ma.ang_freq, ma.angles = self.t.data_ptr(), w["time_freq"].data_ptr(), w["ang_freq"].data_ptr(), self.ang_t.data_ptr()
        ma.w0_f16, ma.b0, ma.w2_f16, ma.b2 = w["mix0.w16"].data_ptr(), w["mix0.b"].data_ptr(), w["mix2.w16"].data_ptr(), w["mix2.b"].data_ptr()
        ma.mask, ma.rot, ma.quat, ma.s_out, ma.B, ma.L = self.mask.data_ptr(), self.rot_t.data_ptr(), self.quat.data_ptr(), self.s.data_ptr(), B, L
        ma.single_pass = int(self.precision == "f16")
        self._keep.append(ma)
        plan.append((lib.pf_input_mixer_fwd, C.byref(ma), "pf_input_mixer_fwd"))

        def emit_proj(b, lane):
            rot = self.rot_t if b == 0 else self.rot
            trans = self.trans_t if b == 0 else self.trans
            pk = "projpm" if self.o_premul else "projp"
            e = lin(self.s, w[f"{b}.projm.w" if self.o_premul else f"{b}.proj.w"], w[f"{b}.{pk}.b"], self.proj, 3968, 128, w16=w[f"{b}.{pk}.w16"])
            la = self._keep[-1]
            la.single_pass = int(self.precision == "f16")
            la.pt_rot, la.pt_trans, la.pt_col0 = rot.data_ptr(), trans.data_ptr(), 3072
            la.pt_qp, la.pt_kp, la.pt_vp = self.qp.data_ptr(), self.kp.data_ptr(), self.vp.data_ptr()
            la.key_end, la.key_L, la.active_rows = self.key_end.data_ptr(), L, self.active_rows
            self._proj_args.append(la)
            if self.att_qk is not None:
                la.att_qk, la.att_vt, la.att_L = self.att_qk.data_ptr(), self.att_vt.data_ptr(), L
            if self.k_frag is not None:
                la.k_frag, la.att_L = self.k_frag.data_ptr(), L
            plan.append(e + (lane,))

        if not self.fused_proj:
            emit_proj(0, 0)
        for b in range(N_BLOCKS):
            rot = self.rot_t if b == 0 else self.rot
            trans = self.trans_t if b == 0 else self.trans
            z_in = (self.edge16 if self.z16 else self.edge_embed) if b == 0 else self.zbuf
            ia = _capi.IpaAttnArgs()
            ia.proj, ia.ldp = self.proj.data_ptr(), 3744
            ia.qp, ia.kp, ia.vp = self.qp.data_ptr(), self.kp.data_ptr(), self.vp.data_ptr()
            ia.z, ia.rot, ia.trans, ia.mask = z_in.data_ptr(), rot.data_ptr(), trans.data_ptr(), self.mask.data_ptr()
            ia.w_b, ia.b_b = w[f"{b}.linear_b.w"].data_ptr(), w[f"{b}.linear_b.b"].data_ptr()
            ia.w_dz, ia.b_dz = w[f"{b}.down_z.w"].data_ptr(), w[f"{b}.down_z.b"].data_ptr()
            ia.head_w, ia.feats, ia.B, ia.L = w[f"{b}.head_w"].data_ptr(), self.feats.data_ptr(), B, L
            ia.bias = (self.pair_bias if b > 0 else self.pair_bias0).data_ptr()
            ia.p_out = None if self.fused_pair else self.attn_p.data_ptr()
            ia.fused_pair = int(self.fused_pair)
            ia.key_end = self.key_end.data_ptr()
            ia.z_f16 = int(self.z16)
            if self.pair_dz is not None:
                ia.dz = (self.pair_dz if b > 0 else self.pair_dz0).data_ptr()
                ia.dz_f16 = int(self.z16)
            if self.att_planes:
                ia.att_mode = 2
                if self.att_qk is not None:
                    ia.att_qk, ia.att_vt = self.att_qk.data_ptr(), self.att_vt.data_ptr()
            if self.k_frag is not None:
                ia.k_frag = self.k_frag.data_ptr()
            if self.fused_proj:
                pk = ("projpm" if self.o_premul else "projp") + ("k" if self.k_fold else "")
                ia.s_in, ia.proj_w_f16, ia.proj_bias = self.s.data_ptr(), w[f"{b}.{pk}.w16"].data_ptr(), w[f"{b}.{pk}.b"].data_ptr()
                ia.k_from_s = int(self.k_fold)
                if self.att_vt32 is not None:
                    ia.att_vt = self.att_vt32.data_ptr()
            self._keep.append(ia)
            plan.append((lib.pf_ipa_attn_fwd, C.byref(ia), "pf_ipa_attn_fwd"))
            ha = _capi.NodeHeadArgs()
            ha.feats, ha.s_in, ha.mask = self.feats.data_ptr(), self.s.data_ptr(), self.mask.data_ptr()
            ha.w_out_f16, ha.b_out = w[f"{b}.linear_out.w16m" if self.o_premul else f"{b}.linear_out.w16"].data_ptr(), w[f"{b}.linear_out.b"].data_ptr()
            ha.o_premul = int(self.o_premul)
            ha.ln_g, ha.ln_b = w[f"{b}.ipa_ln.w"].data_ptr(), w[f"{b}.ipa_ln.b"].data_ptr()
            ha.w_in_f16, ha.b_in = w[f"{b}.0.in.w16"].data_ptr(), w[f"{b}.0.in.b"].data_ptr()
            ha.s_ipa, ha.qkv, ha.rows = self.s.data_ptr(), self.qkv.data_ptr(), rows
            ha.single_pass = int(self.precision == "f16")
            ha.key_end, ha.key_L = self.key_end.data_ptr(), L
            self._keep.append(ha)
            plan.append((lib.pf_node_head_fwd, C.byref(ha), "pf_node_head_fwd"))
            for l in range(2):
                ta = _capi.NodeTfmrArgs()
                ta.qkv = (self.qkv if l == 0 else self.qkv2).data_ptr()
                ta.resid = (self.s if l == 0 else self.v).data_ptr()
                ta.mask = self.mask.data_ptr()
                ta.key_end = self.key_end.data_ptr() if self.active_rows < rows else None
                self._tfmr_args.append(ta)
                ta.w_o_f16, ta.b_o = w[f"{b}.{l}.out.w16"].data_ptr(), w[f"{b}.{l}.out.b"].data_ptr()
                ta.n1_g, ta.n1_b = w[f"{b}.{l}.norm1.w"].data_ptr(), w[f"{b}.{l}.norm1.b"].data_ptr()
                ta.w_1_f16, ta.b_1 = w[f"{b}.{l}.linear1.w16"].data_ptr(), w[f"{b}.{l}.linear1.b"].data_ptr()
                ta.w_2_f16, ta.b_2 = w[f"{b}.{l}.linear2.w16"].data_ptr(), w[f"{b}.{l}.linear2.b"].data_ptr()
                ta.n2_g, ta.n2_b = w[f"{b}.{l}.norm2.w"].data_ptr(), w[f"{b}.{l}.norm2.b"].data_ptr()
                ta.B, ta.L = B, L
                ta.single_pass = int(self.precision == "f16")
                if l == 0:
                    ta.last = 0
                    ta.w_in_next_f16, ta.b_in_next = w[f"{b}.1.in.w16"].data_ptr(), w[f"{b}.1.in.b"].data_ptr()
                    ta.qkv_out, ta.v_out = self.qkv2.data_ptr(), self.v.data_ptr()
                else:
                    ta.last = 1
                    ta.s_ipa, ta.s_out = self.s.data_ptr(), self.s.data_ptr()
                    ta.w_post_f16, ta.b_post = w[f"{b}.post.w16"].data_ptr(), w[f"{b}.post.b"].data_ptr()
                    ta.w_t1_f16, ta.b_t1 = w[f"{b}.nt.linear_1.w16"].data_ptr(), w[f"{b}.nt.linear_1.b"].data_ptr()
                    ta.w_t2_f16, ta.b_t2 = w[f"{b}.nt.linear_2.w16"].data_ptr(), w[f"{b}.nt.linear_2.b"].data_ptr()
                    ta.w_t3_f16, ta.b_t3 = w[f"{b}.nt.linear_3.w16"].data_ptr(), w[f"{b}.nt.linear_3.b"].data_ptr()
                    ta.nt_g, ta.nt_b = w[f"{b}.nt.ln.w"].data_ptr(), w[f"{b}.nt.ln.b"].data_ptr()
                    ta.w_bb_f16, ta.b_bb = w[f"{b}.bb.w16"].data_ptr(), w[f"{b}.bb.b8"].data_ptr()
                    ta.quat_in, ta.rot_in, ta.trans_in = self.quat.data_ptr(), rot.data_ptr(), trans.data_ptr()
                    ta.quat_out, ta.rot_out, ta.trans_out = self.quat.data_ptr(), self.rot.data_ptr(), self.trans.data_ptr()
                    ta.has_et = int(b < N_BLOCKS - 1)
                    if not ta.has_et and self.row_on is not None:
                        ta.row_on = self.row_on.data_ptr()
                    if not ta.has_et:
                        for ni, net in enumerate(("seq_net", "angle_net")):
                            for li, layer in enumerate((0, 2, 4)):
                                ta.h_w[ni][li] = w[f"{net}.{layer}.w16"].data_ptr()
                                ta.h_b[ni][li] = w[f"{net}.{layer}.b"].data_ptr()
                        ta.logits_out, ta.ang_out = self.logits.data_ptr(), self.ang_raw.data_ptr()
                    if ta.has_et:
                        ta.w_init_f16, ta.b_init = w[f"{b}.et.init.w16"].data_ptr(), w[f"{b}.et.init.b"].data_ptr()
                        ta.w_pre_f16, ta.b_pre = w[f"{b}.et.pre.w16"].data_ptr(), w[f"{b}.et.pre.b"].data_ptr()
                        ta.pre = self.pre.data_ptr()
                self._keep.append(ta)
                plan.append((lib.pf_node_tfmr_fwd, C.byref(ta), "pf_node_tfmr_fwd"))
            if b < N_BLOCKS - 1:
                plan.append((None, None, "fork", 0))
                if not self.fused_proj:
                    emit_proj(b + 1, 1)
                et = _capi.EdgeTransitionArgs()
                drop_z = (b == N_BLOCKS - 2 and self.pair_dz is not None and not self.options.get("et_last_store", False))
                et.z_in, et.z_out, et.pre = z_in.data_ptr(), (None if drop_z else self.zbuf.data_ptr()), self.pre.data_ptr()
                if self.z_frag:
                    et.z_in_frag = et.z_out_frag = 1
                    if b == 0:
                        et.z_in = self.edge_frag.data_ptr()
                et.b2, et.ln_g, et.ln_b = w[f"{b}.et.b2"].data_ptr(), w[f"{b}.et.ln.w"].data_ptr(), w[f"{b}.et.ln.b"].data_ptr()
                et.w_stream = w[f"{b}.et.streamf" if (self.z_frag and self.z16) else f"{b}.et.stream"].data_ptr()
                et.bias_out, et.wb_frags = self.pair_bias.data_ptr(), w[f"{b}.et.wbfrags"].data_ptr()
                if self.et_v4:
                    et.w_stream32, et.wb_frags32 = w[f"{b}.et.stream32f" if self.z_frag else f"{b}.et.stream32"].data_ptr(), w[f"{b}.et.wbfrags32"].data_ptr()
                if self.et_v5:
                    et.w_stream64 = w[f"{b}.et.stream64f"].data_ptr()
                if self.et_v5h:
                    et.w_stream64, et.wb_frags32 = w[f"{b}.et.stream64h"].data_ptr(), w[f"{b}.et.wbfrags32"].data_ptr()
                et.bb = w[f"{b + 1}.linear_b.b"].data_ptr()
                et.mask, et.B, et.L = self.mask.data_ptr(), B, L
                et.single_pass = int(self.precision == "f16")
                et.tile_list, et.n_tiles = self.et_tiles.data_ptr(), self.et_ntiles.data_ptr()
                et.z_in_f16, et.z_out_f16 = int(self.z16), int(self.z16)
                if self.pair_dz is not None:
                    et.dz_out, et.dz_out_f16 = self.pair_dz.data_ptr(), int(self.z16)
                self._keep.append(et)
                plan.append((lib.pf_edge_transition_fwd, C.byref(et), "pf_edge_transition_fwd"))
                plan.append((None, None, "join", 0))
        self.plan = plan
        self.plan_version += 1
        self._warm = False

    def want_rows(self, want=None):
        if self.row_on is None:
            return
        if want is None:
            self.row_on.fill_(1)
        else:
            self.row_on.copy_((want.reshape(-1, 16).to(torch.float32).amax(1) > 0).to(torch.int32))

    def set_state(self, t, rotmats_t, trans_t, angles_t, seqs_t):
        rows = self.rows
        self.t.copy_(t.reshape(self.B).to(torch.float32))
        self.rot_t.copy_(rotmats_t.reshape(rows, 9).to(torch.float32))
        self.trans_t.copy_(trans_t.reshape(rows, 3))
        self.ang_t.copy_(angles_t.reshape(rows, 5))
        self.seq_t.copy_(seqs_t.reshape(rows))

    def run(self, stream=None, concurrent=False):
        if stream is not None or not concurrent:
            st = stream if stream is not None else _capi.stream_ptr()
            for entry in self.plan:
                fn, args, name = entry[0], entry[1], entry[2]
                if fn is None:
                    continue
                rc = fn(*args, st) if isinstance(args, tuple) else fn(args, st)
                if rc != 0:
                    _capi.check(rc, name)
            self._warm = True
            return
        main = torch.cuda.current_stream()
        if self._side is None:
            self._side = torch.cuda.Stream(device=self.device)
        side = self._side
        for entry in self.plan:
            fn, args, name = entry[0], entry[1], entry[2]
            lane = entry[3] if len(entry) > 3 else 0
            if fn is None:
                ev = torch.cuda.Event()
                if name == "fork":
                    ev.record(main)
                    side.wait_event(ev)
                else:
                    ev.record(side)
                    main.wait_event(ev)
                continue
            st = (side if lane else main).cuda_stream
            rc = fn(*args, st) if isinstance(args, tuple) else fn(args, st)
            if rc != 0:
                _capi.check(rc, name)

    @property
    def n_launches(self):
        return sum(1 for e in self.plan if e[0] is not None)
```

Baseline: 2.995 million res*step/s.

## Produce split-f16 K fragments in producer epilogues instead of inside IPA scores kernel

Moves the hi/lo f16 split of the node state into K-fragment layout out of the IPA projection/scores kernel. The input mixer and the node transformer's final LayerNorm epilogue now write a dedicated k_frag_s buffer, and the scores kernel reads it per batch. A fallback kfrag kernel fills the buffer when no producer pointer is set. This removes redundant per-head conversion work from the attention kernel, at the cost of an extra buffer, extra stores in producer kernels and ABI changes.

```diff
diff --git a/include/pepflow_hip.h b/include/pepflow_hip.h
--- a/include/pepflow_hip.h
+++ b/include/pepflow_hip.h
@@ -79,6 +79,7 @@
     float* s_out;
     int B, L;
     int single_pass;
+    void* k_frag_s;
 } pf_input_mixer_args;
 int pf_input_mixer_fwd(const pf_input_mixer_args* a, pf_stream_t stream);
 
@@ -117,6 +118,7 @@
     const float* s_in; const void* proj_w_f16; const float* proj_bias;
     const float* k_frag;
     int k_from_s;
+    const void* k_frag_s;
 } pf_ipa_attn_args;
 int pf_ipa_attn_fwd(const pf_ipa_attn_args* a, pf_stream_t stream);
 int pf_ipa_proj_inside_ok(int L, int f16_mode);
@@ -173,6 +175,7 @@
     const int* key_end;
     float* dump[11];
     const int* row_on;
+    void* k_frag_s;
 } pf_node_tfmr_args;
 int pf_node_tfmr_fwd(const pf_node_tfmr_args* a, pf_stream_t stream);
 
diff --git a/pepflowww_amd/_capi.py b/pepflowww_amd/_capi.py
--- a/pepflowww_amd/_capi.py
+++ b/pepflowww_amd/_capi.py
@@ -37,13 +37,13 @@
                 ("trans", _fp), ("mask", _fp), ("w_b", _fp), ("b_b", _fp), ("w_dz", _fp), ("b_dz", _fp),
                 ("head_w", _fp), ("feats", _fp), ("B", _i), ("L", _i), ("bias", _fp), ("p_out", _fp),
                 ("variant", _i), ("att_qk", _fp), ("att_vt", _fp), ("att_mode", _i), ("head_group", _i), ("key_end", _fp), ("z_f16", _i), ("dz", _fp), ("dz_f16", _i), ("fused_pair", _i),
-                ("s_in", _fp), ("proj_w_f16", _fp), ("proj_bias", _fp), ("k_frag", _fp), ("k_from_s", _i)]
+                ("s_in", _fp), ("proj_w_f16", _fp), ("proj_bias", _fp), ("k_frag", _fp), ("k_from_s", _i), ("k_frag_s", _fp)]
 
 
 class InputMixerArgs(C.Structure):
     _fields_ = [("node_embed", _fp), ("seq_table", _fp), ("seqs", _fp), ("t", _fp), ("time_freq", _fp), ("ang_freq", _fp),
                 ("angles", _fp), ("w0_f16", _fp), ("b0", _fp), ("w2_f16", _fp), ("b2", _fp), ("mask", _fp), ("rot", _fp),
-                ("quat", _fp), ("s_out", _fp), ("B", _i), ("L", _i), ("single_pass", _i)]
+                ("quat", _fp), ("s_out", _fp), ("B", _i), ("L", _i), ("single_pass", _i), ("k_frag_s", _fp)]
 
 
 class SeqAttnArgs(C.Structure):
@@ -170,7 +170,7 @@
                 ("b_bb", _fp), ("s_out", _fp), ("quat_in", _fp), ("rot_in", _fp), ("trans_in", _fp),
                 ("quat_out", _fp), ("rot_out", _fp), ("trans_out", _fp), ("has_et", _i),
                 ("w_init_f16", _fp), ("b_init", _fp), ("w_pre_f16", _fp), ("b_pre", _fp), ("pre", _fp), ("B", _i), ("L", _i),
-                ("h_w", (_fp * 3) * 2), ("h_b", (_fp * 3) * 2), ("logits_out", _fp), ("ang_out", _fp), ("single_pass", _i), ("key_end", _fp), ("dump", _fp * 11), ("row_on", _fp)]
+                ("h_w", (_fp * 3) * 2), ("h_b", (_fp * 3) * 2), ("logits_out", _fp), ("ang_out", _fp), ("single_pass", _i), ("key_end", _fp), ("dump", _fp * 11), ("row_on", _fp), ("k_frag_s", _fp)]
 
 
 class SuperposeArgs(C.Structure):
diff --git a/pepflowww_amd/csrc/common.h b/pepflowww_amd/csrc/common.h
--- a/pepflowww_amd/csrc/common.h
+++ b/pepflowww_amd/csrc/common.h
@@ -190,6 +190,21 @@
     }
 }
 __device__ __forceinline__ float join(f32x4 m, f32x4 c, int e) { return m[e] + c[e] * PF_LO_INV; }
+
+template <class V> __device__ __forceinline__ void pf_pin(V& v) { asm("" : "+v"(v)); }
+
+__device__ __forceinline__ void pf_kfrag_put(_Float16* kf, int i, int t8, int g, const float (&v)[4]) {
+    half4 hi, lo;
+#pragma unroll
+    for (int e = 0; e < 4; ++e) hi[e] = (_Float16)v[e];
+    pf_pin(hi);
+#pragma unroll
+    for (int e = 0; e < 4; ++e) lo[e] = (_Float16)(v[e] - (float)hi[e]);
+    _Float16* d = kf + (size_t)(i >> 4) * 4096 + (t8 >> 1) * 1024 + ((i & 15) + 16 * g) * 8 + (t8 & 1) * 4;
+    *reinterpret_cast<half4*>(d) = hi;
+    *reinterpret_cast<half4*>(d + 512) = lo;
+}
+constexpr int PF_KFRAG_TILE_B = 8192;
 
 template <int WT, int D, bool SP = false>
 struct WSplit {
diff --git a/pepflowww_amd/csrc/ipa_split.hip b/pepflowww_amd/csrc/ipa_split.hip
--- a/pepflowww_amd/csrc/ipa_split.hip
+++ b/pepflowww_amd/csrc/ipa_split.hip
@@ -152,7 +152,6 @@
     lds_addr = __builtin_amdgcn_readfirstlane(lds_addr);
     asm volatile("s_mov_b32 m0, %2\n\ts_nop 4\n\tglobal_load_lds_dwordx4 %0, %1" : : "v"(voff), "s"(sb), "s"(lds_addr) : "memory", "m0");
 }
-template <class V> __device__ __forceinline__ void pf_pin(V& v) { asm("" : "+v"(v)); }
 template <int N> __device__ __forceinline__ void pj_wait_vm() { asm volatile("s_waitcnt vmcnt(%0)" : : "n"(N) : "memory"); }
 __device__ __forceinline__ void pj_wait_vm_dyn(int n) {
     n = __builtin_amdgcn_readfirstlane(n);
@@ -225,8 +224,8 @@
         }
     }
     PROFS(31);
-    if constexpr (KF) {
-        _Float16* kfrag = VTH + (size_t)8 * (VTG >> 5) * 1024 + (size_t)tile * 4096 + lane * 8;
+    if constexpr (KF && !KS) {
+        float* kfrag32 = reinterpret_cast<float*>(VTH + (size_t)8 * (VTG >> 5) * 1024 + (size_t)tile * 4096);
         if (wave_on && role != 1) {
             const float* krow = a.s_in + (rowb + iq) * 128 + 4 * g;
 #pragma unroll
@@ -235,23 +234,7 @@
 #pragma unroll
                 for (int u = 0; u < 4; ++u) kt[u] = *reinterpret_cast<const float4*>(krow + 16 * (4 * hb + u));
 #pragma unroll
-                for (int u = 0; u < 4; ++u) {
-                    const int t8 = 4 * hb + u;
-                    const float v[4] = {kt[u].x, kt[u].y, kt[u].z, kt[u].w};
-                    if constexpr (KS) {
-                        half4 hi, lo;
-#pragma unroll
-                        for (int e = 0; e < 4; ++e) hi[e] = (_Float16)v[e];
-                        pf_pin(hi);
-#pragma unroll
-                        for (int e = 0; e < 4; ++e) lo[e] = (_Float16)(v[e] - (float)hi[e]);
-                        _Float16* d = kfrag + (t8 >> 1) * 1024 + (t8 & 1) * 4;
-                        *reinterpret_cast<half4*>(d) = hi;
-                        *reinterpret_cast<half4*>(d + 512) = lo;
-                    } else {
-                        *reinterpret_cast<float4*>(reinterpret_cast<float*>(kfrag - lane * 8) + t8 * 256 + lane * 4) = kt[u];
-                    }
-                }
+                for (int u = 0; u < 4; ++u) *reinterpret_cast<float4*>(kfrag32 + (4 * hb + u) * 256 + lane * 4) = kt[u];
             }
         }
     }
@@ -534,7 +517,7 @@
 }
 
 template <bool VEC4, bool FUSE = false, bool PROJ = false, bool KFRAG = false, bool KF = false, bool HELP = true>
-__global__ __launch_bounds__(512) void ipa_scores_kernel(pf_ipa_attn_args a, int nrb, int rows_per_block, int LP, int SLD) {
+__global__ __launch_bounds__(512) void ipa_scores_kernel(pf_ipa_attn_args a, int nrb, int rows_per_block, int LP, int SLD, unsigned kfs_b ) {
     extern __shared__ __attribute__((aligned(16))) float smem[];
     constexpr bool KSPLIT = PROJ && !FUSE;
     const int L = a.L;
@@ -574,7 +557,9 @@
     const float gamma = softplusf2(a.head_w[h]) * 0.09622504486493763f;
     const float* kbase = a.proj + rowb * a.ldp + OFF_KV + h * 2 * C + 4 * g;
     const char* kfr_u = nullptr;
-    if constexpr (PROJ) {
+    if constexpr (KSPLIT && KF) {
+        kfr_u = reinterpret_cast<const char*>(a.k_frag_s) + (size_t)b * kfs_b;
+    } else if constexpr (PROJ) {
         const int VTG = (L + 31) & ~31;
         kfr_u = reinterpret_cast<const char*>(a.att_vt) + (((size_t)b * H + h) * 512 * VTG + (size_t)8 * (VTG >> 5) * 1024) * sizeof(_Float16);
     }
@@ -1480,6 +1465,17 @@
     *reinterpret_cast<float2*>(a.feats + (size_t)row * PF_IPA_FEATS + 1408 + h * 16 + c) = make_float2(z2[0] + bd.x, z2[1] + bd.y);
 }
 
+__global__ __launch_bounds__(512) void ipa_kfrag_kernel(pf_ipa_attn_args a, _Float16* kf, unsigned kfs_b) {
+    const int tiles = (a.L + 15) >> 4;
+    const int b = blockIdx.x / tiles, tile = blockIdx.x - b * tiles;
+    const int Le = a.key_end ? min(__builtin_amdgcn_readfirstlane(a.key_end[b]), a.L) : a.L;
+    if (16 * tile >= Le) return;
+    const int t8 = threadIdx.x >> 6, lane = threadIdx.x & 63, r = lane & 15, g = lane >> 4;
+    const float4 x = *reinterpret_cast<const float4*>(a.s_in + ((size_t)b * a.L + min(16 * tile + r, Le - 1)) * 128 + 16 * t8 + 4 * g);
+    const float v[4] = {x.x, x.y, x.z, x.w};
+    pf_kfrag_put(reinterpret_cast<_Float16*>(reinterpret_cast<char*>(kf) + (size_t)b * kfs_b), 16 * tile + r, t8, g, v);
+}
+
 }
 
 extern "C" int pf_ipa_proj_inside_ok(int L, int f16_mode) {
@@ -1528,6 +1524,7 @@
         const int nrb = (tiles + wmax - 1) / wmax;
         const int wpb = (tiles + nrb - 1) / nrb;
         const size_t lds = fixed + wpb * per_wave;
+        unsigned kfs_b = 0;
         static PfOncePerDevice attr_set;
         if (attr_set.first()) {
             (void)hipFuncSetAttribute((const void*)ipa_scores_kernel<true>, hipFuncAttributeMaxDynamicSharedMemorySize, 160 * 1024);
@@ -1572,9 +1569,21 @@
             const size_t ldsp = lds > need ? lds : need;
             if (ldsp > 160 * 1024) return PF_E_TOOLARGE;
             const int nwv = wpb <= 4 ? 2 * wpb : wpb;
+            pf_ipa_attn_args ak = *a;
+            if (a->k_from_s && !fuse) {
+                kfs_b = (unsigned)tiles * PF_KFRAG_TILE_B;
+                if (!a->k_frag_s) {
+                    const int VTG = (L + 31) & ~31;
+                    kfs_b = (unsigned)((size_t)H * 512 * VTG * sizeof(_Float16));
+                    _Float16* kf = reinterpret_cast<_Float16*>(const_cast<void*>(a->att_vt)) + (size_t)8 * (VTG >> 5) * 1024;
+                    ak.k_frag_s = kf;
+                    hipLaunchKernelGGL(ipa_kfrag_kernel, dim3((unsigned)(a->B * tiles)), dim3(512), 0, s, ak, kf, kfs_b);
+                    PF_CHECK_LAUNCH();
+                }
+            }
 #define PF_SCORES_PJ(FUSEv, KFv) do { \
-                if (nwv != wpb) hipLaunchKernelGGL((ipa_scores_kernel<true, FUSEv, true, false, KFv, true>), dim3((unsigned)(a->B * H * nrb)), dim3(64 * nwv), ldsp, s, *a, nrb, 16 * wpb, LP, SLD); \
-                else hipLaunchKernelGGL((ipa_scores_kernel<true, FUSEv, true, false, KFv, false>), dim3((unsigned)(a->B * H * nrb)), dim3(64 * nwv), ldsp, s, *a, nrb, 16 * wpb, LP, SLD); } while (0)
+                if (nwv != wpb) hipLaunchKernelGGL((ipa_scores_kernel<true, FUSEv, true, false, KFv, true>), dim3((unsigned)(a->B * H * nrb)), dim3(64 * nwv), ldsp, s, ak, nrb, 16 * wpb, LP, SLD, kfs_b); \
+                else hipLaunchKernelGGL((ipa_scores_kernel<true, FUSEv, true, false, KFv, false>), dim3((unsigned)(a->B * H * nrb)), dim3(64 * nwv), ldsp, s, ak, nrb, 16 * wpb, LP, SLD, kfs_b); } while (0)
             if (a->k_from_s) {
                 if (fuse) PF_SCORES_PJ(true, true);
                 else PF_SCORES_PJ(false, true);
@@ -1600,15 +1609,15 @@
             if (fuse) hipLaunchKernelGGL((ipa_scores16_kernel<true>), g16, b16, lds16, s, *a, nrb16, 16 * wpb16, SLD16);
             else hipLaunchKernelGGL(ipa_scores16_kernel<false>, g16, b16, lds16, s, *a, nrb16, 16 * wpb16, SLD16);
         } else if (a->k_frag) {
-            if (fuse) hipLaunchKernelGGL((ipa_scores_kernel<true, true, false, true>), dim3((unsigned)(a->B * H * nrb)), dim3(64 * wpb), lds, s, *a, nrb, 16 * wpb, LP, SLD);
-            else hipLaunchKernelGGL((ipa_scores_kernel<true, false, false, true>), dim3((unsigned)(a->B * H * nrb)), dim3(64 * wpb), lds, s, *a, nrb, 16 * wpb, LP, SLD);
+            if (fuse) hipLaunchKernelGGL((ipa_scores_kernel<true, true, false, true>), dim3((unsigned)(a->B * H * nrb)), dim3(64 * wpb), lds, s, *a, nrb, 16 * wpb, LP, SLD, kfs_b);
+            else hipLaunchKernelGGL((ipa_scores_kernel<true, false, false, true>), dim3((unsigned)(a->B * H * nrb)), dim3(64 * wpb), lds, s, *a, nrb, 16 * wpb, LP, SLD, kfs_b);
         } else if (fuse) {
-            if ((L & 3) == 0) hipLaunchKernelGGL((ipa_scores_kernel<true, true>), dim3((unsigned)(a->B * H * nrb)), dim3(64 * wpb), lds, s, *a, nrb, 16 * wpb, LP, SLD);
-            else hipLaunchKernelGGL((ipa_scores_kernel<false, true>), dim3((unsigned)(a->B * H * nrb)), dim3(64 * wpb), lds, s, *a, nrb, 16 * wpb, LP, SLD);
+            if ((L & 3) == 0) hipLaunchKernelGGL((ipa_scores_kernel<true, true>), dim3((unsigned)(a->B * H * nrb)), dim3(64 * wpb), lds, s, *a, nrb, 16 * wpb, LP, SLD, kfs_b);
+            else hipLaunchKernelGGL((ipa_scores_kernel<false, true>), dim3((unsigned)(a->B * H * nrb)), dim3(64 * wpb), lds, s, *a, nrb, 16 * wpb, LP, SLD, kfs_b);
         } else if ((L & 3) == 0)
-            hipLaunchKernelGGL(ipa_scores_kernel<true>, dim3((unsigned)(a->B * H * nrb)), dim3(64 * wpb), lds, s, *a, nrb, 16 * wpb, LP, SLD);
+            hipLaunchKernelGGL(ipa_scores_kernel<true>, dim3((unsigned)(a->B * H * nrb)), dim3(64 * wpb), lds, s, *a, nrb, 16 * wpb, LP, SLD, kfs_b);
         else
-            hipLaunchKernelGGL(ipa_scores_kernel<false>, dim3((unsigned)(a->B * H * nrb)), dim3(64 * wpb), lds, s, *a, nrb, 16 * wpb, LP, SLD);
+            hipLaunchKernelGGL(ipa_scores_kernel<false>, dim3((unsigned)(a->B * H * nrb)), dim3(64 * wpb), lds, s, *a, nrb, 16 * wpb, LP, SLD, kfs_b);
         PF_CHECK_LAUNCH();
     }
     if (rc) return rc;
diff --git a/pepflowww_amd/csrc/node_track.hip b/pepflowww_amd/csrc/node_track.hip
--- a/pepflowww_amd/csrc/node_track.hip
+++ b/pepflowww_amd/csrc/node_track.hip
@@ -35,8 +35,8 @@
     p.g[0] = g0.x; p.g[1] = g0.y; p.g[2] = g0.z; p.g[3] = g0.w; p.g[4] = g1.x; p.g[5] = g1.y; p.g[6] = g1.z; p.g[7] = g1.w;
     p.b[0] = b0.x; p.b[1] = b0.y; p.b[2] = b0.z; p.b[3] = b0.w; p.b[4] = b1.x; p.b[5] = b1.y; p.b[6] = b1.z; p.b[7] = b1.w;
 }
-template <int ROWS = 16>
-__device__ __forceinline__ void ln_tile(float* T, const LnParams& p, float mk, Planes out, int m0, int M, float* gout) {
+template <int ROWS = 16, bool KFR = false>
+__device__ __forceinline__ void ln_tile(float* T, const LnParams& p, float mk, Planes out, int m0, int M, float* gout, _Float16* kf = nullptr, int i0 = 0) {
     const int tid = threadIdx.x;
     if (tid < 16 * ROWS) {
         const int row = tid >> 4, sub = tid & 15, m = m0 + row;
@@ -70,6 +70,12 @@
         if (gout && m < M) {
             *reinterpret_cast<float4*>(gout + (size_t)m * 128 + 8 * sub) = make_float4(y[0], y[1], y[2], y[3]);
             *reinterpret_cast<float4*>(gout + (size_t)m * 128 + 8 * sub + 4) = make_float4(y[4], y[5], y[6], y[7]);
+        }
+        if constexpr (KFR) {
+            if (kf && m < M) {
+                pf_kfrag_put(kf, i0 + row, sub >> 1, 2 * (sub & 1), y0);
+                pf_kfrag_put(kf, i0 + row, sub >> 1, 2 * (sub & 1) + 1, y1);
+            }
         }
     }
 }
@@ -718,7 +724,8 @@
             dump4(a.dump[9], rt, v[0] + s0.x, v[1] + s0.y, v[2] + s0.z, v[3] + s0.w);
         }
         __syncthreads();
-        ln_tile<TR>(T0, ln3, lnmask_ld * (lnrow < M ? 1.f : 0.f), Xb, m0, M, a.s_out);
+        _Float16* kfs = DUMP || !a.k_frag_s ? nullptr : reinterpret_cast<_Float16*>(a.k_frag_s) + (size_t)b * ((L + 15) >> 4) * (PF_KFRAG_TILE_B / 2);
+        ln_tile<TR, !DUMP>(T0, ln3, lnmask_ld * (lnrow < M ? 1.f : 0.f), Xb, m0, M, a.s_out, kfs, i0);
         __syncthreads();
         PROF(9);
         if (do_bb || do_init) {
@@ -914,6 +921,11 @@
         y.x = (join(am[0], ac[0], 0) + b2.x) * rmask; y.y = (join(am[0], ac[0], 1) + b2.y) * rmask;
         y.z = (join(am[0], ac[0], 2) + b2.z) * rmask; y.w = (join(am[0], ac[0], 3) + b2.w) * rmask;
         *reinterpret_cast<float4*>(a.s_out + (size_t)mr * 128 + n) = y;
+        if (a.k_frag_s) {
+            const int b = mr / a.L;
+            const float v[4] = {y.x, y.y, y.z, y.w};
+            pf_kfrag_put(reinterpret_cast<_Float16*>(a.k_frag_s) + (size_t)b * ((a.L + 15) >> 4) * (PF_KFRAG_TILE_B / 2), mr - b * a.L, wave, g, v);
+        }
     }
 }
 
diff --git a/pepflowww_amd/engine.py b/pepflowww_amd/engine.py
--- a/pepflowww_amd/engine.py
+++ b/pepflowww_amd/engine.py
@@ -541,6 +541,9 @@
         self.att_vt32 = None
         if self.fused_proj and not self.att_planes:
             self.att_vt32 = torch.zeros(B * 8 * 512 * ((L + 31) // 32 * 32), dtype=torch.float16, device=device)
+        self.k_frag_s = None
+        if self.att_vt32 is not None and self.k_fold and not self.fused_pair:
+            self.k_frag_s = torch.zeros(B * ((L + 15) // 16) * 4096, dtype=torch.float16, device=device)
         self.k_frag = None
         if (not self.fused_proj and precision == "fp32" and L % 16 == 0 and self.pair_dz is not None and
                 opt.get("k_frag", True)):
@@ -698,6 +701,8 @@
         ma.w0_f16, ma.b0, ma.w2_f16, ma.b2 = w["mix0.w16"].data_ptr(), w["mix0.b"].data_ptr(), w["mix2.w16"].data_ptr(), w["mix2.b"].data_ptr()
         ma.mask, ma.rot, ma.quat, ma.s_out, ma.B, ma.L = self.mask.data_ptr(), self.rot_t.data_ptr(), self.quat.data_ptr(), self.s.data_ptr(), B, L
         ma.single_pass = int(self.precision == "f16")
+        kfs = self.k_frag_s.data_ptr() if self.k_frag_s is not None else None
+        ma.k_frag_s = kfs
         self._keep.append(ma)
         plan.append((lib.pf_input_mixer_fwd, C.byref(ma), "pf_input_mixer_fwd"))
 
@@ -749,6 +754,7 @@
                 pk = ("projpm" if self.o_premul else "projp") + ("k" if self.k_fold else "")
                 ia.s_in, ia.proj_w_f16, ia.proj_bias = self.s.data_ptr(), w[f"{b}.{pk}.w16"].data_ptr(), w[f"{b}.{pk}.b"].data_ptr()
                 ia.k_from_s = int(self.k_fold)
+                ia.k_frag_s = kfs
                 if self.att_vt32 is not None:
                     ia.att_vt = self.att_vt32.data_ptr()
             self._keep.append(ia)
@@ -794,6 +800,7 @@
                     ta.quat_in, ta.rot_in, ta.trans_in = self.quat.data_ptr(), rot.data_ptr(), trans.data_ptr()
                     ta.quat_out, ta.rot_out, ta.trans_out = self.quat.data_ptr(), self.rot.data_ptr(), self.trans.data_ptr()
                     ta.has_et = int(b < N_BLOCKS - 1)
+                    ta.k_frag_s = kfs if ta.has_et else None
                     if not ta.has_et and self.row_on is not None:
                         ta.row_on = self.row_on.data_ptr()
                     if not ta.has_et:
```

Result: faster. 3.051 million res*step/s, median of 6 (+1.9%).
